# AdrienC21/CCSD

Hardware: AMD Instinct MI355X
Metric: sampled complexes/sec at 1000 PC steps, QM9_CC batch=1024, 1/2/4/8 GPU (higher is better)
Workload: dtype f32; 1 GPU; qm9_CC N=9 F=4 E=36 K=466, B=1024 per GPU, VE x3, Reverse+Langevin snr=0.2 scale_eps=0.7 n_steps=1, 1000 scales; global_batch=1024, parallelism=batch-sharded x1, per-shard Langevin norms, all-gather at end, finite=True

## Files before the change

### ccsd_amd/_lib.py

```python
from __future__ import annotations

import ctypes as C
import os
from typing import Optional

HERE = os.path.dirname(os.path.abspath(__file__))
HIP_LIB_PATH = os.path.join(HERE, "libccsd_hip.so")

ABI_VERSION = 5
OK, ERR_INVALID, ERR_UNSUPPORTED, ERR_WEIGHTS, ERR_RUNTIME, ERR_WORKSPACE, ERR_CALLBACK = range(7)
SDE_VP, SDE_VE, SDE_SUBVP = 0, 1, 2
PRED_EULER, PRED_REVERSE, PRED_S4 = 0, 1, 2
CORR_NONE, CORR_LANGEVIN = 0, 1
TARGET_X, TARGET_ADJ, TARGET_RANK2 = 0, 1, 2

EXPORTS = [
    "ccsd_plan_create", "ccsd_plan_destroy", "ccsd_weight_count", "ccsd_rank2_dims", "ccsd_workspace_bytes",
    "ccsd_last_error", "ccsd_score", "ccsd_init_state", "ccsd_corrector_norms", "ccsd_corrector_apply",
    "ccsd_predictor", "ccsd_s4_apply", "ccsd_sampler_run", "ccsd_quantize", "ccsd_rank2_cells", "ccsd_profile_kernel", "ccsd_profile_stride", "ccsd_profile_read", "ccsd_profile_launches", "ccsd_debug_stamps",
    "ccsd_noise_draws", "ccsd_noise_draws_at", "ccsd_plan_query", "ccsd_sampler_run_ex", "ccsd_finish",
    "ccsd_cluster_hist", "ccsd_orbit_counts", "ccsd_mmd_workspace_bytes", "ccsd_mmd",
    "ccsd_eig_workspace_bytes", "ccsd_eigvalsh", "ccsd_spectral_workspace_bytes", "ccsd_spectral_hist",
    "ccsd_hodge_workspace_bytes", "ccsd_hodge_spectrum",
    "ccsd_nspdk_row_capacity", "ccsd_nspdk_workspace_bytes", "ccsd_nspdk_features", "ccsd_nspdk_mmd_workspace_bytes", "ccsd_nspdk_mmd",
]
QUERIES = {"fused_r2": 0, "xa_variant": 1, "r2_lds_bytes": 2, "xa_lds_bytes": 3, "fused_loop": 4, "merged_r2": 5, "ew1": 6, "large_graph": 7,
           "r2_family": 8, "r2_instance": 9, "loop_form": 10, "h_full": 11, "hp_full": 12, "p0_narrow": 13, "tiled_fuse": 14, "ew1_fuse": 15,
           "h_general": 16, "geo_ek": 17, "h_wide": 18, "mlp_forms": 19}
KERNEL_IDS = {"k_xa": 0, "k_gemm_p": 1, "k_hf_score": 2, "k_gemm_h": 3, "k_langevin_apply": 4, "k_r2": 5, "k_s4_apply": 6, "k_ew1": 7}


class StepCoef(C.Structure):
    _fields_ = [(n, C.c_float) for n in ("sscale", "alpha", "pa", "pb", "pc", "m1", "s1", "d", "m2", "s2")]


class Config(C.Structure):
    _fields_ = (
        [(n, C.c_int32) for n in (
            "abi_version", "N", "F", "is_cc", "d_min", "d_max",
            "x_depth", "x_nhid",
            "a_num_layers", "a_num_linears", "a_c_init", "a_c_hid", "a_c_final", "a_nhid", "a_adim", "a_num_heads",
            "a_is_cc_net", "h_num_layers", "h_num_linears", "h_nhid", "h_adim", "h_c_hid", "h_c_final", "h_num_heads",
            "f_num_layers", "f_num_linears", "f_nhid", "f_c_hid", "f_c_final", "f_cnum", "f_num_layers_mlp",
            "f_use_hodge_mask",
            "predictor", "corrector", "n_corr_steps", "probability_flow", "denoise")]
        + [("snr", C.c_float), ("scale_eps", C.c_float), ("diff_steps", C.c_int32), ("batch_hint", C.c_int32)]
        + [(n, C.c_int32) for n in ("x_gmh", "x_num_linears", "x_c_init", "x_c_hid", "x_c_final", "x_adim", "x_num_heads",
                                    "a_conv_mlp", "x_conv_mlp")]
    )


class State(C.Structure):
    _fields_ = [("x", C.c_void_p), ("adj", C.c_void_p), ("rank2", C.c_void_p)]


class Noise(C.Structure):
    _fields_ = [("zx", C.c_void_p), ("zadj", C.c_void_p), ("zrank2", C.c_void_p)]


FINISH_ADJ_QUANTIZE, FINISH_ADJ_MOL = 0, 1
MMD_EMD, MMD_TV, MMD_L2 = 0, 1, 2
MMD_INT32, MMD_FP64 = 0, 1
MMD_IS_HIST, MMD_DEGREE, MMD_F32_PMF = 1, 2, 4
CLUSTER_MAX_BINS, MMD_MAX_ROWS, MMD_MAX_BINS = 1024, 1 << 20, 1 << 16
ORBITS = 15
NSPDK_MAX_NODES, NSPDK_FEATURES = 64, 65537
EIG_MAXN, EIG_MAX_SWEEPS = 512, 30


class FinishDims(C.Structure):
    _fields_ = [("B", C.c_int32), ("N", C.c_int32), ("F", C.c_int32), ("E", C.c_int32), ("K", C.c_int64),
                ("d_min", C.c_int32), ("d_max", C.c_int32), ("adj_mode", C.c_int32), ("thr", C.c_float)]


FINISH_OUTPUTS = ("adj_int", "degree", "degree_hist", "edge_hist", "n_nodes", "x_hist", "rank2_u8", "rank2_cell_bits",
                  "rank2_cell_count", "rank2_cell_hist", "rank2_nnz")


class FinishOut(C.Structure):
    _fields_ = [(n, C.c_void_p) for n in FINISH_OUTPUTS]


REDUCE_FN = C.CFUNCTYPE(C.c_int, C.c_void_p, C.c_int32, C.c_void_p, C.c_void_p)


class RunOptions(C.Structure):
    _fields_ = [("reduce", REDUCE_FN), ("user", C.c_void_p)]


class CcsdError(RuntimeError):
    pass


def raise_status(lib, status: int):
    if status == OK:
        return
    msg = lib.ccsd_last_error().decode("utf-8", "replace")
    if status == ERR_UNSUPPORTED:
        raise NotImplementedError(msg)
    if status in (ERR_INVALID, ERR_WEIGHTS, ERR_WORKSPACE):
        raise ValueError(msg)
    raise CcsdError(msg)


class Library:

    def __init__(self, path: str, is_hip: bool):
        if not os.path.exists(path):
            raise FileNotFoundError(path)
        self.path = path
        self.is_hip = is_hip
        L = self.c = C.CDLL(path)
        vp, i32, i64, u64, f32, sz = C.c_void_p, C.c_int32, C.c_int64, C.c_uint64, C.c_float, C.c_size_t
        P = C.POINTER
        L.ccsd_plan_create.argtypes = [P(Config), P(C.c_float), sz, P(StepCoef), P(vp)]
        L.ccsd_plan_create.restype = C.c_int
        L.ccsd_plan_destroy.argtypes = [vp]
        L.ccsd_plan_destroy.restype = None
        L.ccsd_weight_count.argtypes = [P(Config)]
        L.ccsd_weight_count.restype = sz
        L.ccsd_rank2_dims.argtypes = [P(Config), P(i32), P(i64)]
        L.ccsd_rank2_dims.restype = None
        L.ccsd_workspace_bytes.argtypes = [vp, i32]
        L.ccsd_workspace_bytes.restype = sz
        L.ccsd_last_error.argtypes = []
        L.ccsd_last_error.restype = C.c_char_p
        L.ccsd_score.argtypes = [vp, i32, i32, P(State), vp, f32, vp, vp, sz, vp]
        L.ccsd_score.restype = C.c_int
        L.ccsd_init_state.argtypes = [vp, i32, vp, P(Noise), u64, i64, P(State), vp]
        L.ccsd_init_state.restype = C.c_int
        L.ccsd_corrector_norms.argtypes = [vp, i32, i32, i32, P(State), P(State), vp, P(Noise), u64, i64, vp, vp, sz, vp]
        L.ccsd_corrector_norms.restype = C.c_int
        L.ccsd_corrector_apply.argtypes = [vp, i32, i32, i32, P(State), vp, P(Noise), u64, i64, vp, P(State), vp, sz, vp]
        L.ccsd_corrector_apply.restype = C.c_int
        L.ccsd_predictor.argtypes = [vp, i32, i32, P(State), vp, P(Noise), u64, i64, P(State), P(State), vp, sz, vp]
        L.ccsd_predictor.restype = C.c_int
        L.ccsd_s4_apply.argtypes = [vp, i32, i32, P(State), vp, P(Noise), P(Noise), P(Noise), u64, i64, vp, P(State), P(State), vp, sz, vp]
        L.ccsd_s4_apply.restype = C.c_int
        L.ccsd_sampler_run.argtypes = [vp, i32, vp, u64, i64, i32, i32, P(State), P(State), P(State), vp, vp, sz, vp]
        L.ccsd_sampler_run.restype = C.c_int
        L.ccsd_sampler_run_ex.argtypes = L.ccsd_sampler_run.argtypes + [P(RunOptions)]
        L.ccsd_sampler_run_ex.restype = C.c_int
        L.ccsd_quantize.argtypes = [vp, i64, f32, vp, vp]
        L.ccsd_quantize.restype = C.c_int
        L.ccsd_rank2_cells.argtypes = [vp, i32, i32, i64, f32, vp, vp, vp]
        L.ccsd_rank2_cells.restype = C.c_int
        L.ccsd_profile_kernel.argtypes = [vp, i32]
        L.ccsd_profile_kernel.restype = C.c_int
        L.ccsd_profile_stride.argtypes = [vp, i32]
        L.ccsd_profile_stride.restype = C.c_int
        L.ccsd_profile_read.argtypes = [vp, i32, P(i64), P(C.c_double)]
        L.ccsd_profile_read.restype = C.c_int
        L.ccsd_profile_launches.argtypes = [vp, i32, P(i64)]
        L.ccsd_profile_launches.restype = C.c_int
        L.ccsd_debug_stamps.argtypes = [vp, vp]
        L.ccsd_debug_stamps.restype = C.c_int
        L.ccsd_noise_draws.argtypes = [vp, i32, vp, u64, i64, i32, i32, P(State), vp]
        L.ccsd_noise_draws.restype = C.c_int
        L.ccsd_noise_draws_at.argtypes = [vp, i32, vp, u64, i64, C.c_uint32, i32, P(State), vp]
        L.ccsd_noise_draws_at.restype = C.c_int
        L.ccsd_plan_query.argtypes = [vp, i32, P(i64)]
        L.ccsd_plan_query.restype = C.c_int
        L.ccsd_finish.argtypes = [P(FinishDims), P(State), vp, P(FinishOut), vp]
        L.ccsd_finish.restype = C.c_int
        L.ccsd_cluster_hist.argtypes = [vp, i32, i32, i32, f32, vp, i32, vp, vp, vp]
        L.ccsd_cluster_hist.restype = C.c_int
        L.ccsd_orbit_counts.argtypes = [vp, i32, i32, i32, f32, vp, vp, vp, vp]
        L.ccsd_orbit_counts.restype = C.c_int
        L.ccsd_mmd_workspace_bytes.argtypes = [i32, i32, i32]
        L.ccsd_mmd_workspace_bytes.restype = sz
        L.ccsd_mmd.argtypes = [vp, i32, vp, vp, i32, vp, i32, i32, i32, i32, C.c_double, C.c_double, vp, sz, vp, vp]
        L.ccsd_mmd.restype = C.c_int
        L.ccsd_eig_workspace_bytes.argtypes = [i32, i32]
        L.ccsd_eig_workspace_bytes.restype = sz
        L.ccsd_eigvalsh.argtypes = [vp, i32, i32, vp, vp, vp, sz, vp]
        L.ccsd_eigvalsh.restype = C.c_int
        L.ccsd_spectral_workspace_bytes.argtypes = [i32, i32]
        L.ccsd_spectral_workspace_bytes.restype = sz
        L.ccsd_spectral_hist.argtypes = [vp, i32, i32, i32, f32, vp, i32, vp, vp, vp, vp, sz, vp]
        L.ccsd_spectral_hist.restype = C.c_int
        L.ccsd_hodge_workspace_bytes.argtypes = [i32, i32]
        L.ccsd_hodge_workspace_bytes.restype = sz
        L.ccsd_hodge_spectrum.argtypes = [vp, vp, i32, i32, i32, i32, i32, f32, vp, vp, vp, sz, vp]
        L.ccsd_hodge_spectrum.restype = C.c_int
        L.ccsd_nspdk_row_capacity.argtypes = [i32]
        L.ccsd_nspdk_row_capacity.restype = i32
        L.ccsd_nspdk_workspace_bytes.argtypes = [i32, i32]
        L.ccsd_nspdk_workspace_bytes.restype = sz
        L.ccsd_nspdk_features.argtypes = [vp, vp, i32, i32, i32, f32, vp, vp, vp, vp, sz, vp]
        L.ccsd_nspdk_features.restype = C.c_int
        L.ccsd_nspdk_mmd_workspace_bytes.argtypes = [i32, i32]
        L.ccsd_nspdk_mmd_workspace_bytes.restype = sz
        L.ccsd_nspdk_mmd.argtypes = [vp, vp, vp, i32, vp, vp, vp, i32, vp, sz, vp, vp]
        L.ccsd_nspdk_mmd.restype = C.c_int

    def __getattr__(self, name):
        return getattr(self.c, name)

    def check(self, status: int):
        raise_status(self.c, status)


_hip: Optional[Library] = None


def get_library() -> Library:
    global _hip
    if _hip is None:
        import torch

        path = os.environ.get("CCSD_LIB_PATH") or HIP_LIB_PATH
        if not os.path.exists(path):
            raise CcsdError(
                f"{path} is missing: build it with `python -c 'import __graft_entry__ as g; g.build()'` "
                "(hipcc --offload-arch=gfx950).  ccsd_amd has no CPU fallback."
            )
        _hip = Library(path, is_hip=True)
    return _hip
```

### ccsd_amd/csrc/ccsd_api.h

```cpp
#pragma once
#include "ccsd_kernels.h"
#define CCSD_INST_TABLES
#include "ccsd_instances.h"
#include <stdio.h>
#include <stdlib.h>
#include <memory>
#include <string>
#include <vector>

static thread_local std::string g_last_error;
static int set_err(int st, const std::string& m) { g_last_error = m; return st; }

static inline int fnet_width(const PlanD& p) {
    int fw = p.f_fdim > p.f_cnum ? p.f_fdim : p.f_cnum;
    for (int l = 0; l < p.f_L; ++l) {
        const MlpD& m = p.fl[l];
        const int wd = m.n > 1 && m.hid > m.in ? (m.hid > m.out ? m.hid : m.out) : (m.in > m.out ? m.in : m.out);
        if (wd > fw) fw = wd;
    }
    if (p.f_fin.n > 1 && p.f_fin.hid > fw) fw = p.f_fin.hid;
    return fw;
}

struct Knobs {
    int no_fused_r2 = 0, hodge_general = 0, geo_off = 0, no_fused_apply = 0, no_h_full = 0, no_hp_full = 0, hp_full_norms = 0, split_bf16 = 0;
    int xa_threads = 0, xa_prio = 0, lg_force = 0, xa_pass = -1, xa_gch = 0, no_mlp_wt = 0, verbose = 0;
    const char *dump_plan = nullptr, *dump_plan_name = nullptr;
};
static Knobs read_knobs() {
    Knobs k;
    auto on = [](const char* name) { return getenv(name) != nullptr; };
    k.no_fused_r2 = on("CCSD_NO_FUSED_R2"); k.hodge_general = on("CCSD_HODGE_GENERAL");
    k.geo_off = on("CCSD_NO_GEO") ? 1 : on("CCSD_NO_BAKE") ? 2 : 0;
    k.no_fused_apply = on("CCSD_NO_FUSED_APPLY"); k.no_h_full = on("CCSD_NO_H_FULL"); k.no_hp_full = on("CCSD_NO_HP_FULL");
    k.hp_full_norms = on("CCSD_HP_FULL_NORMS");
    if (const char* v = getenv("CCSD_SPLIT_BF16")) k.split_bf16 = atoi(v) == 3 ? 3 : 0;
    if (const char* v = getenv("CCSD_XA_THREADS")) { const int t = atoi(v); if (t >= 64 && t <= 1024 && t % 64 == 0) k.xa_threads = t; }
    if (const char* v = getenv("CCSD_XA_PRIO")) k.xa_prio = atoi(v);
    if (const char* v = getenv("CCSD_LARGE_GRAPH")) { const int f = atoi(v); k.lg_force = (f == 1 || f == 2) ? f : 0; }
    if (const char* v = getenv("CCSD_XA_PASS")) k.xa_pass = atoi(v);
    k.xa_gch = on("CCSD_XA_GCH"); k.no_mlp_wt = on("CCSD_NO_MLP_WT"); k.verbose = on("CCSD_VERBOSE");
    k.dump_plan = getenv("CCSD_DUMP_PLAN"); k.dump_plan_name = getenv("CCSD_DUMP_PLAN_NAME");
    return k;
}

enum { R2_NONE = 0, R2_FUSED = 1, R2_EW1 = 2, R2_TILED = 3 };
enum { LOOP_PRED_ONLY = 0, LOOP_LANGEVIN = 1, LOOP_LANGEVIN_FUSED = 2, LOOP_S4 = 3, LOOP_LANGEVIN_MULTI = 4 };
struct Route {
    int lg = 0;
    int xa_variant = 0;
    const XaEntry* xa = nullptr;
    const XaEntry* xa_twin = nullptr;
    int xa_threads = 0;
    int r2_family = R2_NONE;
    const R2Entry* r2 = nullptr;
    int r2_ldk = 0, r2_ldh = 0;
    size_t r2_lds = 0;
    int h_general = 0;
    int h_wide = 0;
    int geo = 0;
    int p0 = -1;
    int h_full = 0;
    unsigned hp_full_modes = 0;
    int loop = LOOP_PRED_ONLY;
    int merged = 0;
    int tiled_fuse = 0;
    int ew1_fuse = 0;
    int corrector_flat = 0, predictor_flat = 0;
};

struct ccsd_plan {
    ccsd_config_t cfg;
    PlanD h;
    HodgeBaseD hbx[CCSD_LG_MAXHB];
    MlpD hdm[CCSD_MAXHL + CCSD_MAXHLX];
    MlpD afin_lg;
    PlanD* d = nullptr;
    float* w = nullptr;
    float* wp = nullptr;
    unsigned char* hpairs = nullptr;
    size_t npacked = 0;
    unsigned char* edges = nullptr;
    unsigned long long* cells = nullptr;
    std::vector<ccsd_step_coef_t> coef;
    size_t nweights = 0;
    long long* dbg = nullptr;
    unsigned long long* init_off = nullptr;
    size_t init_off_cap = 0;
    Knobs knobs;
    Route rt;
    mutable unsigned prof_mask = 0;
    mutable size_t prof_used[8] = {0, 0, 0, 0, 0, 0, 0, 0};
    mutable int prof_stride = 1;
    mutable size_t prof_calls[8] = {0, 0, 0, 0, 0, 0, 0, 0};
#ifndef CCSD_EMU
    mutable std::vector<hipEvent_t> prof_ev[8];
#endif
};

enum { KID_XA = 0, KID_GEMM_P = 1, KID_HF = 2, KID_GEMM_H = 3, KID_LANGEVIN = 4, KID_R2 = 5, KID_S4 = 6, KID_EW1 = 7 };
static void prof_mark(const ccsd_plan* pl, int kid, void* stream) {
#ifndef CCSD_EMU
    if (!(pl->prof_mask & (1u << kid))) return;
    const size_t call = pl->prof_calls[kid]++;
    if (pl->prof_stride > 1 && (call >> 1) % (size_t)pl->prof_stride != 0) return;
    std::vector<hipEvent_t>& ev = pl->prof_ev[kid];
    if (pl->prof_used[kid] == ev.size()) {
        hipEvent_t e;
        if (hipEventCreate(&e) != hipSuccess) return;
        ev.push_back(e);
    }
    (void)hipEventRecord(ev[pl->prof_used[kid]++], (hipStream_t)stream);
#else
    (void)pl; (void)kid; (void)stream;
#endif
}
#define RT_CHECK(expr)                                                                    \
    do {                                                                                  \
        rtError_t _e = (expr);                                                            \
        if (_e != RT_OK) return set_err(CCSD_ERR_RUNTIME, std::string(#expr) + ": " + rt_error_string(_e)); \
    } while (0)
#define LAUNCH_CHECK()                                                                    \
    do {                                                                                  \
        rtError_t _e = rt_last_error();                                                   \
        if (_e != RT_OK) return set_err(CCSD_ERR_RUNTIME, std::string("kernel launch: ") + rt_error_string(_e)); \
    } while (0)

static int resolve_route(ccsd_plan* pl) {
    const PlanD& p = pl->h;
    const ccsd_config_t& c = pl->cfg;
    const Knobs& k = pl->knobs;
    Route& r = pl->rt;
    const int E = p.E, K = p.K;
    const bool s4 = c.predictor == CCSD_PRED_S4, langevin = c.corrector == CCSD_CORR_LANGEVIN;
    unsigned char arch[sizeof(PlanD)];
    ccsd_plan_arch_bytes(p, arch);
    auto baked = [&](const unsigned char* plan, size_t size) { return size == sizeof(PlanD) && p.geo_off == 0 && memcmp(arch, plan, size) == 0; };

    bool conv_mlp = false;
    for (int l = 0; l < p.a_L; ++l) conv_mlp = conv_mlp || p.al[l].conv_mlp;
    if (p.x_gmh) for (int l = 0; l < p.x_depth; ++l) conv_mlp = conv_mlp || p.gl[l].conv_mlp;
    int v = p.hb_L ? XA_HB : p.x_gmh ? XA_GMH : XA_PLAIN;
    if (conv_mlp || (p.hb_L && p.x_gmh) || p.h_L > 2 || (!p.chan_global && !p.hb_L && p.a_fin.chain >= 5)) v = XA_GEN;
    if (v == XA_PLAIN && !p.chan_global && baked(CCSD_BAKED_QM9_PLAN, CCSD_BAKED_QM9_SIZE)) v = XA_BAKED9;
    else if (v == XA_PLAIN && p.chan_global && baked(CCSD_BAKED_CS_PLAN, CCSD_BAKED_CS_SIZE)) v = XA_BAKED20;
    else if (v == XA_PLAIN && p.chan_global && baked(CCSD_BAKED_Z_PLAN, CCSD_BAKED_Z_SIZE)) v = XA_BAKED38;
    else if (v == XA_GEN && !p.chan_global && baked(CCSD_BAKED_ENZ_PLAN, CCSD_BAKED_ENZ_SIZE)) v = XA_BAKEDENZ;
    else if (v == XA_PLAIN && p.geo_off != 1)
        for (const auto& g : XA_GEO_TABLE)
            if ((p.chan_global != 0) == (g.gch != 0) && p.N == g.N && (!g.F || p.F == g.F) && E == g.E && p.ldn == g.ldn) v = g.var;
    r.xa_variant = v;
    r.xa_threads = k.xa_threads;
    for (const XaEntry& e : XA_TABLE) {
        if ((e.gch != 0) != (p.chan_global != 0)) continue;
        if (e.var == v) r.xa = &e;
        if (e.var == XA_PLAIN) r.xa_twin = &e;
    }
    if (!r.xa || !r.xa_twin) return set_err(CCSD_ERR_RUNTIME, "k_xa variant " + std::to_string(v) + " has no instance in CCSD_XA_LIST");
    if (!r.xa->fixed256) r.xa_twin = nullptr;

    const bool aff = p.f_affine != 0, gen1 = p.h_L > 1 && p.hl[0].mval.n > 1;
    const int mt = (E + 15) / 16, rem = E & 15, rs = (!aff || rem == 0 || rem > 12) ? 0 : (rem + 3) / 4;
    auto r2_find = [&](int qm9) -> const R2Entry* {
        for (const R2Entry& e : R2_TABLE)
            if (e.mt == mt && e.rs == rs && (e.affine != 0) == aff && (e.gen1 != 0) == gen1 && e.qm9 == qm9) return &e;
        return nullptr;
    };
    bool fused = false;
    if (c.is_cc && E <= 64 && !k.no_fused_r2 && !r.h_wide) {
        const int Kp4 = (K + 31) & ~31, Ep4 = (E + 3) & ~3;
        int ldk = Kp4; while ((ldk & 31) != 8 && (ldk & 31) != 24) ldk += 4;
        const int ldh = Ep4;
        const size_t fl = (size_t)E * ldk + (size_t)E * ldh + 64 * 2 + (size_t)p.a_cinit * E + 3 * c.N * c.N + 64 + (Kp4 + 3) / 4 + 4;
        if (fl * 4 + 64 <= 160 * 1024 && fnet_width(p) <= CCSD_FW && r2_find(0) && p.f_cnum <= 2) {
            fused = true; r.r2_ldk = ldk; r.r2_ldh = ldh; r.r2_lds = fl * 4;
            const bool qm9 = p.geo_off != 1 && !gen1 && E == CCSD_R2_QM9_E && K == CCSD_R2_QM9_K && p.N == CCSD_R2_QM9_N &&
                             ldk == CCSD_R2_QM9_LDK && ldh == CCSD_R2_QM9_LDH;
            r.r2 = r2_find(!qm9 ? 0 : aff && baked(CCSD_BAKED_QM9_PLAN, CCSD_BAKED_QM9_SIZE) ? 2 : 1);
            if (!r.r2) return set_err(CCSD_ERR_RUNTIME, "k_r2: the qm9-geometry instance is missing from CCSD_R2_LIST_*");
        }
    }
    if (p.h_L > 2) {
        bool affine_values = true;
        for (int l = 0; l + 1 < p.h_L; ++l) affine_values = affine_values && ccsd_hl(p, l).mval.n == 1;
        if (!affine_values || !fused || p.h_L > 4 || k.hodge_general || r.lg) { r.h_general = 1; fused = false; r.r2 = nullptr; }
    }
    const bool ew1 = c.is_cc && !fused && aff && p.f_cnum == 1 && !s4 && !r.h_wide;
    r.r2_family = !c.is_cc ? R2_NONE : fused ? R2_FUSED : ew1 ? R2_EW1 : R2_TILED;
    if (p.geo_off != 1) for (const GeoEntry& g : GEO_TABLE) if (E == g.E && K == g.K) r.geo = g.idx;
    if (p.h_L >= 1) {
        auto p0_find = [&](int kc) {
            for (int i = 0; i < (int)(sizeof(P0_TABLE) / sizeof(P0_TABLE[0])); ++i)
                if (P0_TABLE[i].nt == (p.hl[0].wc + 15) / 16 && P0_TABLE[i].kc == kc) return i;
            return -1;
        };
        if (p.geo_off != 1) r.p0 = p0_find(K);
        if (r.p0 < 0) r.p0 = p0_find(0);
    }
    r.tiled_fuse = !r.lg && r.r2_family == R2_TILED && p.h_L == 1 && (K & 3) == 0 && !s4 && langevin;
    r.ew1_fuse = !r.lg && ew1 && p.h_L == 1 && (K & 3) == 0 && langevin;
    const bool full_geo = c.is_cc && E == CCSD_FULL_E && K == CCSD_FULL_K && p.geo_off != 1 && !k.no_h_full;
    r.h_full = full_geo && r.r2_family == R2_TILED && p.f_cnum >= 2;

    const bool fused_apply = !r.lg && (fused || (ew1 && p.h_L <= 1) || r.tiled_fuse) && !k.no_fused_apply;
    r.loop = s4 ? LOOP_S4 : !langevin ? LOOP_PRED_ONLY : c.n_corr_steps != 1 ? LOOP_LANGEVIN_MULTI : fused_apply ? LOOP_LANGEVIN_FUSED : LOOP_LANGEVIN;
    if (full_geo && r.tiled_fuse && p.hl[0].wc <= 16 && p.f_cnum == 2 && !k.no_hp_full)
        r.hp_full_modes = (r.loop == LOOP_LANGEVIN_FUSED ? 1u << 2 : 0u) | (k.hp_full_norms ? 1u << 1 : 0u);
    r.merged = r.loop == LOOP_LANGEVIN_FUSED && fused && mt == 3 && rs == 1 && aff && !gen1 && (K & 1) == 0 && ((E * K) & 3) == 0;
    r.corrector_flat = !s4;
    r.predictor_flat = ew1;
    return CCSD_OK;
}
static inline bool use_h_full(const Route& r, int B) { return r.h_full && B >= 256; }
static inline bool use_hp_full(const Route& r, int B, int mode) { return B >= 256 && ((r.hp_full_modes >> mode) & 1u); }
#define HP_FULL_LDS ((size_t)(2 * 192 * H_LD + 2 * 16 * H_LD) * 4)
static inline int hodge_value_cw(int E) { return E > 128 ? 32 : 64; }
static inline size_t hodge_value_lds(int E) { return (size_t)E * hodge_value_cw(E) * 4; }
static inline const XaEntry* xa_launch(const Route& r, int B, int* threads) {
    const XaEntry* e = r.xa;
    int t = r.xa_threads;
    if (t == 0) t = e->max_threads == 256 ? 256 : B <= 256 ? 1024 : B <= 512 ? 512 : 256;
    if (e->fixed256 && t != 256) e = r.xa_twin;
    *threads = t > e->max_threads ? e->max_threads : t;
    return e;
}
static inline int normsum_threads(int B) { return B > 512 ? 1024 : B > 256 ? 512 : 256; }

extern "C" const char* ccsd_last_error(void) { return g_last_error.c_str(); }

extern "C" void ccsd_rank2_dims(const ccsd_config_t* cfg, int32_t* E, int64_t* K) {
    int e = 0; int64_t k = 0;
    if (cfg) ccsd_dims(cfg, &e, &k);
    if (E) *E = e;
    if (K) *K = k;
}

extern "C" size_t ccsd_weight_count(const ccsd_config_t* cfg) {
    PlanD p; PlanBuilder pb;
    size_t n = ccsd_build_plan(cfg, &p, pb);
    if (pb.status != CCSD_OK) { set_err(pb.status, pb.err); return 0; }
    return n;
}

extern "C" int ccsd_debug_stamps(ccsd_plan_t* plan, void* dev_buffer) {
    if (!plan) return set_err(CCSD_ERR_INVALID, "NULL plan");
    plan->dbg = (long long*)dev_buffer;
    return CCSD_OK;
}
extern "C" int ccsd_profile_kernel(ccsd_plan_t* plan, int32_t kernel_id) {
    if (!plan) return set_err(CCSD_ERR_INVALID, "NULL plan");
    if (kernel_id < 0) plan->prof_mask = 0;
    else if (kernel_id < 8) plan->prof_mask |= 1u << kernel_id;
    for (int k = 0; k < 8; ++k) { plan->prof_used[k] = 0; plan->prof_calls[k] = 0; }
    return CCSD_OK;
}
extern "C" int ccsd_profile_stride(ccsd_plan_t* plan, int32_t stride) {
    if (!plan || stride < 1) return set_err(CCSD_ERR_INVALID, "bad argument");
    plan->prof_stride = stride;
    for (int k = 0; k < 8; ++k) plan->prof_calls[k] = 0;
    return CCSD_OK;
}
extern "C" int ccsd_profile_launches(ccsd_plan_t* plan, int32_t kernel_id, int64_t* launches) {
    if (!plan || !launches || kernel_id < 0 || kernel_id >= 8) return set_err(CCSD_ERR_INVALID, "bad argument");
    *launches = (int64_t)(plan->prof_calls[kernel_id] >> 1);
    return CCSD_OK;
}
extern "C" int ccsd_profile_read(ccsd_plan_t* plan, int32_t kernel_id, int64_t* launches, double* total_ms) {
    if (!plan || !launches || !total_ms || kernel_id < 0 || kernel_id >= 8) return set_err(CCSD_ERR_INVALID, "bad argument");
    *launches = 0; *total_ms = 0.0;
#ifndef CCSD_EMU
    for (size_t i = 0; i + 1 < plan->prof_used[kernel_id]; i += 2) {
        float ms = 0.f;
        RT_CHECK(hipEventSynchronize(plan->prof_ev[kernel_id][i + 1]));
        RT_CHECK(hipEventElapsedTime(&ms, plan->prof_ev[kernel_id][i], plan->prof_ev[kernel_id][i + 1]));
        *total_ms += ms; *launches += 1;
    }
#endif
    plan->prof_used[kernel_id] = 0;
    return CCSD_OK;
}

extern "C" void ccsd_plan_destroy(ccsd_plan_t* plan) {
    if (!plan) return;
#ifndef CCSD_EMU
    for (int k = 0; k < 8; ++k) for (hipEvent_t e : plan->prof_ev[k]) (void)hipEventDestroy(e);
#endif
    if (plan->d) (void)rt_free(plan->d);
    if (plan->w) (void)rt_free(plan->w);
    if (plan->wp) (void)rt_free(plan->wp);
    if (plan->hpairs) (void)rt_free(plan->hpairs);
    if (plan->edges) (void)rt_free(plan->edges);
    if (plan->cells) (void)rt_free(plan->cells);
    if (plan->init_off) (void)rt_free(plan->init_off);
    delete plan;
}

extern "C" int ccsd_plan_create(const ccsd_config_t* cfg, const float* weights, size_t n_weights,
                                const ccsd_step_coef_t* step_coef, ccsd_plan_t** out) {
    if (!cfg || !weights || !step_coef || !out) return set_err(CCSD_ERR_INVALID, "NULL argument");
    *out = nullptr;
    std::unique_ptr<ccsd_plan, void (*)(ccsd_plan_t*)> guard(new ccsd_plan(), ccsd_plan_destroy);
    ccsd_plan* pl = guard.get();
    pl->cfg = *cfg;
    const Knobs& k = pl->knobs = read_knobs();
    PlanBuilder pb;
    pb.lg_force = k.lg_force; pb.xa_pass = k.xa_pass; pb.xa_gch = k.xa_gch; pb.no_mlp_wt = k.no_mlp_wt; pb.verbose = k.verbose;
    pl->nweights = ccsd_build_plan(cfg, &pl->h, pb);
    if (pb.status != CCSD_OK) return set_err(pb.status, pb.err);
    pl->rt.lg = pb.lg; pl->rt.h_wide = pb.h_wide;
    memcpy(pl->hbx, pb.hbx, sizeof(pl->hbx));
    memcpy(pl->hdm, pb.hdm, sizeof(pl->hdm));
    pl->afin_lg = pb.afin_lg;
    pl->h.geo_off = k.geo_off;
    pl->npacked = (size_t)pb.pcur;
    if (pl->nweights != n_weights)
        return set_err(CCSD_ERR_WEIGHTS, "weight blob has " + std::to_string(n_weights) + " floats, config needs " +
                                             std::to_string(pl->nweights));
    if (cfg->predictor != CCSD_PRED_EULER && cfg->predictor != CCSD_PRED_REVERSE && cfg->predictor != CCSD_PRED_S4) return set_err(CCSD_ERR_UNSUPPORTED, "unknown predictor");
    if (cfg->corrector != CCSD_CORR_NONE && cfg->corrector != CCSD_CORR_LANGEVIN) return set_err(CCSD_ERR_UNSUPPORTED, "unknown corrector");
    if (cfg->diff_steps < 1 || cfg->n_corr_steps < 0) return set_err(CCSD_ERR_INVALID, "bad step counts");
    ccsd_fold_fnet(&pl->h, weights);
    pl->coef.assign(step_coef, step_coef + (size_t)cfg->diff_steps * 3);
    const int N = cfg->N, E = pl->h.E, K = pl->h.K;
    std::vector<unsigned char> edges((size_t)2 * E + 2);
    {
        int e = 0;
        for (int i = 0; i < N; ++i)
            for (int j = i + 1; j < N; ++j) { edges[2 * e] = (unsigned char)i; edges[2 * e + 1] = (unsigned char)j; ++e; }
    }
    std::vector<unsigned long long> cells((size_t)K + 1);
    if (cfg->is_cc) {
        size_t c = 0;
        std::vector<int> idx;
        for (int k = cfg->d_min; k <= cfg->d_max; ++k) {
            idx.resize(k);
            for (int i = 0; i < k; ++i) idx[i] = i;
            while (true) {
                unsigned long long m = 0;
                for (int i = 0; i < k; ++i) m |= 1ull << idx[i];
                cells[c++] = m;
                int i = k - 1;
                while (i >= 0 && idx[i] == N - k + i) --i;
                if (i < 0) break;
                ++idx[i];
                for (int j = i + 1; j < k; ++j) idx[j] = idx[j - 1] + 1;
            }
        }
        if ((int)c != K) return set_err(CCSD_ERR_INVALID, "cell enumeration mismatch");
    }
    RT_CHECK(rt_malloc((void**)&pl->d, sizeof(PlanD)));
    RT_CHECK(rt_h2d(pl->d, &pl->h, sizeof(PlanD)));
    {
        const size_t wtotal = pl->h.f_blk >= 0 ? (size_t)pl->h.f_blk + CCSD_FBLK_FLOATS : n_weights;
        RT_CHECK(rt_malloc((void**)&pl->w, wtotal * sizeof(float)));
        RT_CHECK(rt_h2d(pl->w, weights, n_weights * sizeof(float)));
        if (pl->h.f_blk >= 0) {
            std::vector<float> blk(CCSD_FBLK_FLOATS);
            ccsd_pack_fnet_blocks(&pl->h, weights, blk.data());
            RT_CHECK(rt_h2d(pl->w + pl->h.f_blk, blk.data(), blk.size() * sizeof(float)));
        }
    }
    {
        std::vector<float> packed(pl->npacked + 4, 0.f);
        ccsd_pack_mlp(pl->h.x_fin, weights, packed.data());
        for (int l = 0; l < pl->h.a_L; ++l) {
            ccsd_pack_mlp(pl->h.al[l].mlp, weights, packed.data()); ccsd_pack_mlp(pl->h.al[l].mc, weights, packed.data());
            ccsd_pack_qkv(pl->h.al[l], weights, packed.data()); ccsd_pack_mc(pl->h.al[l], weights, packed.data());
        }
        if (pl->h.x_gmh) for (int l = 0; l < pl->h.x_depth; ++l) {
            ccsd_pack_mlp(pl->h.gl[l].mlp, weights, packed.data()); ccsd_pack_mlp(pl->h.gl[l].mc, weights, packed.data());
            ccsd_pack_qkv(pl->h.gl[l], weights, packed.data()); ccsd_pack_mc(pl->h.gl[l], weights, packed.data());
        }
        for (int l = 0; l < pl->h.hb_L; ++l) {
            const HodgeBaseD& h = pl->hbx[l];
            ccsd_pack_mlp(h.mh, weights, packed.data());
            for (int c = 0; c < h.cin; ++c) {
                const float* blk = weights + h.blk_base + (size_t)c * h.blk_stride;
                const float* w2 = blk + h.hid * E + h.hid;
                for (int e = 0; e < E; ++e)
                    for (int hh = 0; hh < h.hid; ++hh) {
                        packed[(size_t)h.w2t + ((size_t)c * h.hid + hh) * E + e] = w2[e * h.hid + hh];
                        packed[(size_t)h.w1t + ((size_t)c * E + e) * h.hid + hh] = blk[hh * E + e];
                    }
            }
        }
        ccsd_pack_mlp(pl->h.a_fin, weights, packed.data());
        if (pl->rt.lg) {
            for (int l = 0; l < pl->h.h_L; ++l) ccsd_pack_mlp(pl->hdm[l], weights, packed.data());
            if (pl->afin_lg.chain) ccsd_pack_mlp(pl->afin_lg, weights, packed.data());
        }
        for (int l = 0; l < pl->h.h_L; ++l) {
            const HodgeLayerD& h = ccsd_hl(pl->h, l);
            const int Kp = (K + 31) & ~31;
            for (int k = 0; k < K; ++k)
                for (int n = 0; n < h.wc; ++n) packed[(size_t)h.wcatT + (size_t)n * Kp + k] = weights[(size_t)h.wcat + (size_t)k * h.wc + n];
        }
        RT_CHECK(rt_malloc((void**)&pl->wp, packed.size() * sizeof(float)));
        RT_CHECK(rt_h2d(pl->wp, packed.data(), packed.size() * sizeof(float)));
    }
    if (pl->h.h_L > 1 && !pl->rt.lg) {
        if (E > 255) return set_err(CCSD_ERR_UNSUPPORTED, "dense hodge layer needs E <= 255");
        std::vector<unsigned char> hp;
        for (int e = 0; e < E; ++e)
            for (int e2 = e; e2 < E; ++e2) { hp.push_back((unsigned char)e); hp.push_back((unsigned char)e2); }
        RT_CHECK(rt_malloc((void**)&pl->hpairs, hp.size()));
        RT_CHECK(rt_h2d(pl->hpairs, hp.data(), hp.size()));
    }
    RT_CHECK(rt_malloc((void**)&pl->edges, edges.size()));
    RT_CHECK(rt_h2d(pl->edges, edges.data(), edges.size()));
    RT_CHECK(rt_malloc((void**)&pl->cells, cells.size() * sizeof(unsigned long long)));
    RT_CHECK(rt_h2d(pl->cells, cells.data(), cells.size() * sizeof(unsigned long long)));
    if (int st = resolve_route(pl)) return st;
    {
        const Route& r = pl->rt;
        const size_t xlds = (size_t)pl->h.xa_lds_floats * 4;
        if (xlds > 64 * 1024) {
            RT_CHECK(rt_set_max_dyn_smem((const void*)r.xa->fn, xlds));
            if (r.xa_twin) RT_CHECK(rt_set_max_dyn_smem((const void*)r.xa_twin->fn, xlds));
        }
        if (r.r2 && r.r2_lds > 64 * 1024) RT_CHECK(rt_set_max_dyn_smem((const void*)r.r2->fn, r.r2_lds));
        if (r.lg && lg_nmlp_lds(pl->h) > 64 * 1024) RT_CHECK(rt_set_max_dyn_smem((const void*)k_lg_nmlp, lg_nmlp_lds(pl->h)));
        if (r.lg && pl->h.hb_L > 1) {
            size_t v = 0;
            for (int l = 0; l + 1 < pl->h.hb_L; ++l) if (lg_hb_dense_lds(pl->hbx[l]) > v) v = lg_hb_dense_lds(pl->hbx[l]);
            if (v > 64 * 1024) RT_CHECK(rt_set_max_dyn_smem((const void*)k_lg_hb_dense, v));
        }
        if (r.lg && r.h_general && hodge_value_lds(E) > 64 * 1024)
            RT_CHECK(rt_set_max_dyn_smem(r.h_wide ? (const void*)k_hodge_value_w : (const void*)k_hodge_value, hodge_value_lds(E)));
#ifndef CCSD_EMU
        if (r.hp_full_modes) {
            RT_CHECK(rt_set_max_dyn_smem((const void*)k_hp_full<CCSD_FULL_E, CCSD_FULL_K, 1>, HP_FULL_LDS));
            RT_CHECK(rt_set_max_dyn_smem((const void*)k_hp_full<CCSD_FULL_E, CCSD_FULL_K, 2>, HP_FULL_LDS));
        }
#endif
    }
    if (const char* path = k.dump_plan) {
        const char* nm = k.dump_plan_name ? k.dump_plan_name : "QM9";
        std::vector<unsigned char> bytes(sizeof(PlanD));
        ccsd_plan_arch_bytes(pl->h, bytes.data());
        if (FILE* f = fopen(path, "w")) {
            fprintf(f, "// GENERATED by tools/bake_plan.py (do not edit): the PlanD of a shipped configuration at its bench batch as a compile-time\n"
                       "// constant (architecture bytes: ccsd_plan_arch_bytes, the weight-derived affine fold zeroed).  The baked kernel instances read\n"
                       "// their plan from it instead of from memory; the host selects them only for plans whose architecture bytes are equal.\n"
                       "#pragma once\n#define CCSD_BAKED_%s_SIZE %zu\n#define CCSD_BAKED_%s_A_L %d      /* AttentionLayers of ScoreNetworkA: unroll count */\n"
                       "alignas(16) static constexpr unsigned char CCSD_BAKED_%s_PLAN[CCSD_BAKED_%s_SIZE] = {", nm, sizeof(PlanD), nm, pl->h.a_L, nm, nm);
            for (size_t i = 0; i < bytes.size(); ++i) fprintf(f, "%s%u,", (i % 40) ? "" : "\n    ", (unsigned)bytes[i]);
            fprintf(f, "\n};\n");
            fclose(f);
        }
    }
    *out = guard.release();
    return CCSD_OK;
}

#define CCSD_P_SPLITS 8

struct Workspace {
    unsigned long long* offbits;
    unsigned char *mfr, *mfl;
    int Kp, Ep;
    float *H, *P0, *P1, *U1, *acoef, *net_x, *net_adj, *net_r, *norm2, *part, *sums, *chan, *zpart, *part2;
    float* psplit; size_t psplit_floats;
    float *P0b, *P1b, *U1b;
    int ntiles, nchunk;
    float *hgH, *hgR[2], *hgP[CCSD_MAXHL + CCSD_MAXHLX - 1];
    size_t hg_hstride;
    float *lg_S, *lg_att, *lg_dis, *lg_Y, *lg_QKV, *lg_x[2], *lg_xcat, *lg_xY, *lg_xnet, *lg_part;
    int lg_tiles;
    float *lg_hbg, *lg_hbH;
    size_t lg_hbg_stride, lg_hbH_stride;
    float *lg_hdq, *lg_hdd, *lg_hdpc, *lg_hdH;
    size_t lg_hdq_stride, lg_hdH_stride;
    ccsd_state_t third;
    size_t bytes;
    MaskTab masks() const { return MaskTab{mfr, mfl, Kp, Ep}; }
};
struct Pass {
    const float* h_src = nullptr;
    int p1_raw = 0;
};
static inline int r2_p1_raw(const PlanD& p) { return p.h_L > 1 && p.hl[0].mval.n == 1; }
static Workspace carve_ws(const ccsd_plan* pl, int B, void* base) {
    const PlanD& p = pl->h;
    Workspace w{};
    size_t o = 0;
    auto take = [&](size_t nbytes) { size_t r = o; o += (nbytes + 255) / 256 * 256; return base ? (char*)base + r : (char*)nullptr; };
    w.offbits = (unsigned long long*)take((size_t)B * 8);
    const size_t E = p.E, K = p.K;
    w.Kp = p.is_cc ? (p.K + 3) & ~3 : 0; w.Ep = p.is_cc ? (p.E + 3) & ~3 : 0;
    w.mfr = (unsigned char*)take((size_t)B * w.Kp);
    w.mfl = (unsigned char*)take((size_t)B * w.Ep);
    w.H = (float*)take(p.is_cc ? (size_t)B * E * h_ld((int)E) * 4 * (p.f_cnum > 2 ? p.f_cnum - 1 : 1) : 0);
    w.P0 = (float*)take(p.h_L > 0 ? (size_t)B * E * p.hl[0].wc * 4 : 0);
    w.P1 = (float*)take(p.h_L > 1 ? (size_t)B * E * p.h_pw * 4 : 0);
    w.U1 = (float*)take(p.h_L > 1 ? (size_t)B * p.h_pw * 4 : 0);
    w.psplit_floats = p.h_L > 1 ? (size_t)CCSD_P_SPLITS * B * E * p.h_pw : 0;
    w.psplit = (float*)take(w.psplit_floats * 4);
    const bool two = pl->rt.r2_family == R2_FUSED;
    w.P0b = (float*)take(two && p.h_L > 0 ? (size_t)B * E * p.hl[0].wc * 4 : 0);
    w.P1b = (float*)take(two && p.h_L > 1 ? (size_t)B * E * p.h_pw * 4 : 0);
    w.U1b = (float*)take(two && p.h_L > 1 ? (size_t)B * p.h_pw * 4 : 0);
    w.acoef = (float*)take(p.h_L > 1 ? (size_t)B * p.a_cinit * E * 4 : 0);
    if (pl->rt.h_general) {
        int cmax = 1;
        for (int l = 0; l + 1 < p.h_L; ++l) cmax = ccsd_hl(p, l).cout > cmax ? ccsd_hl(p, l).cout : cmax;
        w.hg_hstride = (size_t)cmax * E * E;
        w.hgH = (float*)take((size_t)B * w.hg_hstride * 4);
        w.hgR[0] = (float*)take((size_t)B * E * K * 4);
        w.hgR[1] = (float*)take((size_t)B * E * K * 4);
        for (int l = 1; l < p.h_L; ++l) w.hgP[l - 1] = (float*)take((size_t)B * E * ccsd_hl(p, l).wc * 4);
    }
    w.net_x = (float*)take((size_t)B * p.N * p.F * 4);
    w.net_adj = (float*)take((size_t)B * p.N * p.N * 4);
    w.net_r = (float*)take(p.is_cc ? (size_t)B * E * K * 4 : 0);
    w.norm2 = (float*)take((size_t)B * 4 * 4);
    w.ntiles = p.is_cc ? ((p.K + T_BN - 1) / T_BN) * ((p.E + T_BM - 1) / T_BM) : 0;
    w.nchunk = p.is_cc ? (int)((((size_t)p.E * p.K + 3) / 4 + CCSD_NN_CH - 1) / CCSD_NN_CH) : 0;
    { int np = w.ntiles > w.nchunk ? w.ntiles : w.nchunk; if ((int)E > np) np = (int)E;
      w.part = (float*)take((size_t)B * (np ? np : 1) * 2 * 4); }
    w.zpart = (float*)take((size_t)B * ((size_t)w.nchunk > E ? (size_t)w.nchunk : E ? E : 1) * 4);
    w.part2 = (float*)take((size_t)B * 2 * 4);
    w.sums = (float*)take(64);
    w.chan = (float*)take(p.chan_global ? (size_t)B * p.chan_rows * p.N * p.N * 4 : 0);
    if (pl->rt.lg) {
        const size_t N = p.N, NN = N * N;
        int cin = 1, cp = 1, fx = p.F > p.x_nhid ? p.F : p.x_nhid;
        for (int l = 0; l < p.a_L; ++l) {
            if (p.al[l].cin > cin) cin = p.al[l].cin;
            if (p.al[l].cp > cp) cp = p.al[l].cp;
            if (p.al[l].fout > fx) fx = p.al[l].fout;
        }
        w.lg_tiles = (int)((NN + CCSD_LG_FIN_ROWS - 1) / CCSD_LG_FIN_ROWS);
        w.lg_S = (float*)take((size_t)B * p.a_fdim * NN * 4);
        w.lg_att = (float*)take((size_t)B * cin * NN * 4);
        w.lg_dis = (float*)take((size_t)B * cin * N * 4);
        w.lg_Y = (float*)take((size_t)B * cin * N * cp * 4);
        w.lg_QKV = (float*)take((size_t)B * cin * N * cp * 4);
        w.lg_x[0] = (float*)take((size_t)B * N * fx * 4);
        w.lg_x[1] = (float*)take((size_t)B * N * fx * 4);
        w.lg_xcat = (float*)take((size_t)B * N * p.x_fdim * 4);
        w.lg_xY = (float*)take((size_t)B * N * p.x_nhid * 4);
        w.lg_xnet = (float*)take((size_t)B * N * p.F * 4);
        w.lg_part = (float*)take((size_t)B * w.lg_tiles * 2 * 4);
        if (p.hb_L) {
            size_t g = 0, hd = 0;
            for (int l = 0; l < p.hb_L; ++l) {
                const HodgeBaseD& h = pl->hbx[l];
                if ((size_t)h.cin * E * h.hid > g) g = (size_t)h.cin * E * h.hid;
                if (l + 1 < p.hb_L && (size_t)h.cout * E * E > hd) hd = (size_t)h.cout * E * E;
            }
            w.lg_hbg_stride = g; w.lg_hbH_stride = hd;
            w.lg_hbg = (float*)take((size_t)B * g * 4);
            w.lg_hbH = (float*)take((size_t)B * hd * 4);
        }
        if (p.h_L > 1) {
            size_t q = 0, d = 0, hd = 0;
            for (int l = 0; l < p.h_L; ++l) {
                const HodgeLayerD& h = ccsd_hl(p, l);
                if ((size_t)h.cin * E * 2 * h.adim > q) q = (size_t)h.cin * E * 2 * h.adim;
                if (l > 0 && (size_t)h.cin * E > d) d = (size_t)h.cin * E;
                if (l + 1 < p.h_L && (size_t)h.cout * E * E > hd) hd = (size_t)h.cout * E * E;
            }
            w.lg_hdq_stride = q;
            w.lg_hdq = (float*)take((size_t)B * q * 4);
            w.lg_hdd = (float*)take((size_t)B * d * 4);
            w.lg_hdpc = (float*)take((size_t)B * 2 * E * 4);
            if (pl->rt.h_general) { w.lg_hdH = w.hgH; w.lg_hdH_stride = w.hg_hstride; }
            else { w.lg_hdH_stride = hd; w.lg_hdH = (float*)take((size_t)B * hd * 4); }
        }
    }
    if (pl->rt.loop == LOOP_LANGEVIN_MULTI && pl->cfg.n_corr_steps > 1) {
        w.third.x = (float*)take((size_t)B * p.N * p.F * 4);
        w.third.adj = (float*)take((size_t)B * p.N * p.N * 4);
        w.third.rank2 = p.is_cc ? (float*)take((size_t)B * E * K * 4) : nullptr;
    }
    w.bytes = o;
    return w;
}
extern "C" size_t ccsd_workspace_bytes(const ccsd_plan_t* plan, int32_t B) {
    if (!plan || B < 1) return 0;
    return carve_ws(plan, B, nullptr).bytes;
}

static int grid_for(long long n, int block) {
    long long g = (n + block - 1) / block;
    if (g > 2048) g = 2048;
    if (g < 1) g = 1;
    return (int)g;
}

static int check_common(const ccsd_plan* pl, int B, const void* flags, void* ws, size_t ws_bytes, Workspace& w) {
    if (!pl) return set_err(CCSD_ERR_INVALID, "NULL plan");
    if (B < 1) return set_err(CCSD_ERR_INVALID, "B must be >= 1");
    if (!flags) return set_err(CCSD_ERR_INVALID, "NULL flags");
    if (ws) w = carve_ws(pl, B, ws);
    if (!ws || ws_bytes < w.bytes) return set_err(CCSD_ERR_WORKSPACE, "workspace too small");
    return CCSD_OK;
}
static int check_state(const ccsd_plan* pl, const ccsd_state_t* s, const char* what) {
    if (!s || !s->x || !s->adj || (pl->h.is_cc && !s->rank2)) return set_err(CCSD_ERR_INVALID, std::string("NULL tensor in ") + what);
    return CCSD_OK;
}

static int launch_flagbits(const ccsd_plan* pl, int B, const float* flags, Workspace& w, void* stream) {
    if (pl->rt.lg && !pl->h.is_cc) return CCSD_OK;
    CCSD_LAUNCH(k_flagbits, dim3(grid_for(B, 256)), dim3(CCSD_NTHREADS), 0, stream, flags, w.offbits, B, pl->h.N);
    LAUNCH_CHECK();
    if (pl->h.is_cc) {
        CCSD_LAUNCH(k_masktab, dim3(grid_for((long long)B * (w.Kp + w.Ep), 256)), dim3(CCSD_NTHREADS), 0, stream,
                    (const unsigned long long*)w.offbits, (const unsigned char*)pl->edges, (const unsigned long long*)pl->cells, w.mfr, w.mfl,
                    B, pl->h.E, pl->h.K, w.Kp, w.Ep);
        LAUNCH_CHECK();
    }
    return CCSD_OK;
}

static int launch_h(const ccsd_plan* pl, int B, const float* rank2, Pass& ps, Workspace& w, void* stream) {
    const PlanD& p = pl->h;
    if (!p.is_cc || p.f_cnum < 2) return CCSD_OK;
    if (ps.h_src == rank2) return CCSD_OK;
    const bool full = use_h_full(pl->rt, B);
    const int nth_ = (p.E + T_BM - 1) / T_BM;
    dim3 g(xcd_grid(B, nth_ * (nth_ + 1) / 2));
    prof_mark(pl, KID_GEMM_H, stream);
#ifndef CCSD_EMU
    if (full && pl->knobs.split_bf16 == 3) hipLaunchKernelGGL((k_gemm_h_full<CCSD_FULL_E, CCSD_FULL_K, 2>), dim3(B), dim3(256), 0, (hipStream_t)stream, rank2, w.H, p.f_hmask);
    else if (full) hipLaunchKernelGGL((k_gemm_h_full<CCSD_FULL_E, CCSD_FULL_K>), dim3(B), dim3(256), 0, (hipStream_t)stream, rank2, w.H, p.f_hmask);
    else
#endif
    {
        (void)full;
#define H_GO(EC_, KC_) CCSD_LAUNCH((k_gemm_h<EC_, KC_>), g, dim3(CCSD_NTHREADS), 0, stream, rank2, w.H, p.E, p.K, p.f_hmask, B)
        GEO_EK(pl->rt.geo, H_GO);
#undef H_GO
    }
    prof_mark(pl, KID_GEMM_H, stream);
    LAUNCH_CHECK();
    for (int j = 2; j < p.f_cnum; ++j) {
        const size_t slab = (size_t)B * p.E * h_ld(p.E);
        const int nt = (p.E + 15) / 16, per = CCSD_NTHREADS >= 64 ? CCSD_NTHREADS / 64 : 1;
        CCSD_LAUNCH(k_gemm_pow, dim3((nt * nt + per - 1) / per, 1, B), dim3(CCSD_NTHREADS), 0, stream,
                    (const float*)(w.H + (size_t)(j - 2) * slab), (const float*)w.H, w.H + (size_t)(j - 1) * slab, p.E);
        LAUNCH_CHECK();
    }
    return CCSD_OK;
}
static void launch_gemm_p_whole(const ccsd_plan* pl, int B, const float* R, const HodgeLayerD& h, float* out, const Workspace& w, void* stream) {
    const PlanD& p = pl->h;
    const int rows = B * p.E;
    CCSD_LAUNCH(k_gemm_p, dim3((h.wc + T_BN - 1) / T_BN, (rows + T_BM - 1) / T_BM, 1), dim3(CCSD_NTHREADS), 0, stream, R, (const float*)pl->w, out,
                rows, p.E, p.K, h.wc, h.wcat, 0, h.mval, h.cin, (const float*)nullptr, (const unsigned long long*)w.offbits,
                (const unsigned char*)pl->edges, (const unsigned long long*)pl->cells, p.K);
}
static void launch_hodge_value(const ccsd_plan* pl, int B, const float* Rin, const float* H, size_t h_stride, const float* acoef,
                              const HodgeLayerD& h, float* Rout, const Workspace& w, void* stream) {
    const PlanD& p = pl->h;
    const int cw = hodge_value_cw(p.E);
    CCSD_LAUNCH(pl->rt.h_wide ? k_hodge_value_w : k_hodge_value, dim3((p.K + cw - 1) / cw, B), dim3(CCSD_NTHREADS), hodge_value_lds(p.E), stream, Rin, H,
                (int)h_stride, acoef, (const float*)pl->w, h.mval, h.cin, Rout, p.E, p.K, cw,
                (const unsigned long long*)w.offbits, (const unsigned char*)pl->edges, (const unsigned long long*)pl->cells);
}
static int hodge_stack_layer(const ccsd_plan* pl, int B, int l, Workspace& w, void* stream) {
    float* Rl = w.hgR[(l - 1) & 1];
    launch_hodge_value(pl, B, w.hgR[(l - 2) & 1], w.hgH, w.hg_hstride, nullptr, ccsd_hl(pl->h, l - 1), Rl, w, stream);
    LAUNCH_CHECK();
    launch_gemm_p_whole(pl, B, Rl, ccsd_hl(pl->h, l), w.hgP[l - 1], w, stream);
    LAUNCH_CHECK();
    return CCSD_OK;
}
static int launch_r2(const ccsd_plan* pl, int B, const float* rank2, const float* adj, const float* flags, int want_p,
                     RankEpi& ep, NoiseArgs& na, Pass& ps, Workspace& w, void* stream, const CorrFuse* cf, int merge_draw);
static int launch_p(const ccsd_plan* pl, int B, const float* adj, const float* rank2, Pass& ps, Workspace& w, void* stream, const P0Fuse* fuse = nullptr) {
    const PlanD& p = pl->h;
    const Route& rt = pl->rt;
    if (p.h_L < 1) return CCSD_OK;
    if (p.h_L > 2 && !rt.h_general) {
        RankEpi ep{};
        ep.mode = MODE_SCORE; ep.sscale = 0.f; ep.out = w.net_r;
        NoiseArgs na0{};
        return launch_r2(pl, B, rank2, adj, nullptr, 1, ep, na0, ps, w, stream, nullptr, -1);
    }
    ps.p1_raw = 0;
    const int rows = B * p.E;
    const bool hp_full = fuse && use_hp_full(rt, B, fuse->mode);
#ifndef CCSD_EMU
    if (hp_full) {
        const HodgeLayerD& h = p.hl[0];
        const float* WT = (const float*)pl->wp + h.wcatT;
        prof_mark(pl, KID_GEMM_H, stream);
        if (fuse->mode == 1)
            hipLaunchKernelGGL((k_hp_full<CCSD_FULL_E, CCSD_FULL_K, 1>), dim3(B), dim3(512), HP_FULL_LDS, (hipStream_t)stream, rank2, WT, w.H, w.P0, h.wc, p.f_hmask, *fuse);
        else
            hipLaunchKernelGGL((k_hp_full<CCSD_FULL_E, CCSD_FULL_K, 2>), dim3(B), dim3(512), HP_FULL_LDS, (hipStream_t)stream, rank2, WT, w.H, w.P0, h.wc, p.f_hmask, *fuse);
        prof_mark(pl, KID_GEMM_H, stream);
        LAUNCH_CHECK();
        ps.h_src = fuse->mode == 2 ? fuse->f1 : rank2;
        return CCSD_OK;
    }
#endif
    (void)hp_full;
    {
        const HodgeLayerD& h = p.hl[0];
        prof_mark(pl, KID_GEMM_P, stream);
        P0Fuse pf{};
        if (fuse) pf = *fuse;
#ifndef CCSD_EMU
        if (rt.p0 >= 0)
            hipLaunchKernelGGL(P0_TABLE[rt.p0].fn[pf.mode], dim3((rows + T_BM - 1) / T_BM), dim3(256), 0, (hipStream_t)stream, rank2,
                               (const float*)pl->wp + h.wcatT, w.P0, rows, p.K, (p.K + 31) & ~31, h.wc, pf);
        else
#endif
        {
            const float* src = rank2;
            if (pf.mode) {
                CCSD_LAUNCH(k_p0_fuse_ew, dim3(grid_for(rows, 256)), dim3(CCSD_NTHREADS), 0, stream, rank2, pf, rows, p.K);
                LAUNCH_CHECK();
                if (pf.mode == 2 || pf.mode == 4) src = pf.f1;
            }
            launch_gemm_p_whole(pl, B, src, h, w.P0, w, stream);
        }
        prof_mark(pl, KID_GEMM_P, stream);
        LAUNCH_CHECK();
    }
    if (p.h_L > 1) {
        CCSD_LAUNCH(k_edgecoef, dim3(B), dim3(CCSD_NTHREADS), (size_t)3 * p.N * p.N * 4, stream, adj, w.acoef, p.N, p.E,
                    p.a_cinit, (const unsigned char*)pl->edges);
        LAUNCH_CHECK();
        const HodgeLayerD& h0 = p.hl[0];
        const HodgeLayerD& h = p.hl[1];
        dim3 g((h.wc + T_BN - 1) / T_BN, (rows + T_BM - 1) / T_BM, 1);
        const int nslab = (p.K + T_BK - 1) / T_BK;
        int S = CCSD_P_SPLITS < nslab ? CCSD_P_SPLITS : nslab;
        if ((size_t)S * rows * h.wc > w.psplit_floats) S = 1;
        const int kchunk = ((nslab + S - 1) / S) * T_BK;
        S = (p.K + kchunk - 1) / kchunk;
        g.z = S;
        float* P1 = rt.h_general ? w.hgP[0] : w.P1;
        CCSD_LAUNCH(rt.h_wide ? k_gemm_p_w : k_gemm_p, g, dim3(CCSD_NTHREADS), 0, stream, rank2, (const float*)pl->w, S > 1 ? w.psplit : P1, rows, p.E, p.K, h.wc,
                    h.wcat, 1, h0.mval, h0.cin, (const float*)w.acoef, (const unsigned long long*)w.offbits,
                    (const unsigned char*)pl->edges, (const unsigned long long*)pl->cells, kchunk);
        LAUNCH_CHECK();
        if (S > 1) {
            const long long n = (long long)rows * h.wc;
            CCSD_LAUNCH(k_sum_splits, dim3(grid_for(n, 256)), dim3(CCSD_NTHREADS), 0, stream, (const float*)w.psplit, P1, n, S);
            LAUNCH_CHECK();
        }
        if (rt.h_general) {
            launch_hodge_value(pl, B, rank2, nullptr, 0, w.acoef, h0, w.hgR[0], w, stream);
            LAUNCH_CHECK();
        }
    }
    return CCSD_OK;
}
static int launch_lg(const ccsd_plan* pl, int B, XaArgs& xa, NoiseArgs& na, Workspace& w, void* stream);
static int launch_xa(const ccsd_plan* pl, int B, XaArgs& xa, NoiseArgs& na, const Pass& ps, Workspace& w, void* stream, bool set_b = false) {
    const Route& rt = pl->rt;
    xa.P0 = set_b ? w.P0b : w.P0;
    xa.P1 = set_b ? w.P1b : w.P1; xa.U1 = set_b ? w.U1b : w.U1; xa.p1_raw = ps.p1_raw;
    if (rt.lg) return launch_lg(pl, B, xa, na, w, stream);
    xa.chan_ws = w.chan;
    xa.dbg = pl->dbg ? pl->dbg + 32 : nullptr;
    int xa_threads;
    const XaEntry* inst = xa_launch(rt, B, &xa_threads);
    prof_mark(pl, KID_XA, stream);
    xa.wp = pl->wp; xa.hpairs = pl->hpairs;
    xa.prio_mode = pl->knobs.xa_prio;
    const dim3 xblk(CCSD_NTHREADS == 1 ? 1 : xa_threads);
    const size_t xlds = (size_t)pl->h.xa_lds_floats * 4;
#define XA_LAUNCH(XA_) CCSD_LAUNCH(inst->fn, dim3(B), xblk, xlds, stream, (const PlanD*)pl->d, (const float*)pl->w, (const unsigned char*)pl->edges, XA_, na)
    if (rt.h_general) {
        const PlanD& p = pl->h;
        if (rt.xa_variant != XA_GEN) return set_err(CCSD_ERR_RUNTIME, "general hodge stack needs k_xa<., XA_GEN>");
        xa.pdirect = 1;
        for (int l = 1; l < p.h_L; ++l) xa.Pd[l - 1] = w.hgP[l - 1];
        for (int l = 2; l < p.h_L; ++l) {
            XaArgs pre = xa;
            pre.hdump_layer = l - 1; pre.hdump = w.hgH; pre.hdump_stride = (int)w.hg_hstride;
            XA_LAUNCH(pre);
            LAUNCH_CHECK();
            if (int st = hodge_stack_layer(pl, B, l, w, stream)) return st;
        }
    }
    XA_LAUNCH(xa);
#undef XA_LAUNCH
    prof_mark(pl, KID_XA, stream);
    LAUNCH_CHECK();
    return CCSD_OK;
}
static int launch_lg(const ccsd_plan* pl, int B, XaArgs& xa, NoiseArgs& na, Workspace& w, void* stream) {
    const PlanD& p = pl->h;
    if (xa.cf.on) return set_err(CCSD_ERR_RUNTIME, "tiled graph-network route: no fused corrector apply");
    const int N = p.N, F = p.F, NN = N * N, H = p.x_nhid, XF = p.x_fdim;
    const int rt = (N + 15) / 16, gt = (N + CCSD_LG_GT - 1) / CCSD_LG_GT, at = (N + CCSD_LG_AT - 1) / CCSD_LG_AT;
    const dim3 blk(CCSD_NTHREADS);
    auto cdiv = [](int a, int b_) { return (a + b_ - 1) / b_; };
    prof_mark(pl, KID_XA, stream);
    if (xa.do_x) {
        CCSD_LAUNCH(k_lg_dis, dim3(grid_for(N, 256), B), blk, 0, stream, xa.adjX, (long long)NN, 0, 1, N, w.lg_dis);
        CCSD_LAUNCH(k_lg_put, dim3(grid_for((long long)B * N * F, 256)), blk, 0, stream, xa.xX, F, w.lg_xcat, XF, B * N);
        for (int l = 0; l < p.x_depth; ++l) {
            const int fin = l ? H : F;
            const float* src = l ? w.lg_xcat + F + (l - 1) * H : xa.xX;
            CCSD_LAUNCH(k_lg_xw, dim3(grid_for((long long)N * H, 256), B), blk, 0, stream, src, (long long)N * (l ? XF : F), l ? XF : F, fin,
                        (const float*)pl->w + p.x_gw[l], 0, H, 1, N, (const float*)w.lg_dis, w.lg_xY);
            CCSD_LAUNCH(k_lg_gcn, dim3(gt * cdiv(H, CCSD_LG_GT), 1, B), blk, 0, stream, xa.adjX, (long long)NN, 0, (const float*)w.lg_xY,
                        (const float*)w.lg_dis, (const float*)pl->w + p.x_gb[l], 0, H, H, 1, N, w.lg_xcat, (long long)N * XF, 0, XF, F + l * H, 1);
        }
        CCSD_LAUNCH(k_lg_nmlp, dim3(rt, B), blk, lg_nmlp_lds_of(p.x_fin), stream, p.x_fin, (const float*)pl->w,
                    (LgGather{w.lg_xcat, (long long)N * XF, 0, XF, 0, XF}), N, xa.flags, 0, w.lg_xnet);
        LAUNCH_CHECK();
    }
    if (xa.do_a) {
        const long long ss = (long long)p.a_fdim * NN;
        for (int c = 0; c < p.a_cinit; ++c)
            CCSD_LAUNCH(k_lg_pow, dim3(grid_for(NN, 256), B), blk, 0, stream, xa.adjA, w.lg_S, ss, N, c);
        if (p.h_L == 1) {
            if (!xa.P0) return set_err(CCSD_ERR_RUNTIME, "tiled graph-network route: no hodge projections");
            if (pl->rt.h_wide) {
                CCSD_LAUNCH(k_lg_hodge1_w, dim3(grid_for(p.E, 256), B), blk, 0, stream, p.hl[0], pl->hdm[0], 1.0f / (float)sqrt((double)p.K), (const float*)pl->w,
                            (const float*)pl->wp, (const unsigned char*)pl->edges, xa.P0, w.lg_S, ss, p.a_nch_graph, N, p.E, xa.flags);
            } else {
                CCSD_LAUNCH(k_lg_hodge1, dim3(grid_for(p.E + N, 256), B), blk, 0, stream, p.hl[0], 1.0f / (float)sqrt((double)p.K), (const float*)pl->w,
                            (const unsigned char*)pl->edges, xa.P0, w.lg_S, ss, p.a_nch_graph, N, p.E, xa.flags);
            }
        }
        if (p.h_L > 1) {
            const Route& rtp = pl->rt;
            if (!xa.P0 || (!rtp.h_general && !xa.P1)) return set_err(CCSD_ERR_RUNTIME, "tiled graph-network route: no hodge projections");
            if (p.h_L > 2 && !rtp.h_general) return set_err(CCSD_ERR_RUNTIME, "tiled graph-network route: more than two hodge layers need the general hodge stack");
            const int E = p.E, et = (E + 15) / 16;
            const unsigned char* edges = (const unsigned char*)pl->edges;
            const float* wts = (const float*)pl->w;
            const float rks = 1.0f / (float)sqrt((double)p.K);
            const long long qs = (long long)w.lg_hdq_stride, hs = (long long)w.lg_hdH_stride;
            int ch = p.a_nch_graph + p.a_cinit;
            CCSD_LAUNCH(k_lg_hd_qk0, dim3(grid_for(E + N, 256), B), blk, 0, stream, p.hl[0], p.a_nch_hodge, wts, edges, xa.P0, w.lg_S, ss, p.a_nch_graph, N, E,
                        w.lg_hdq, qs);
            for (int j = 1; j < p.h_L; ++j) {
                const HodgeLayerD& hp = ccsd_hl(p, j - 1);
                const HodgeLayerD& h = ccsd_hl(p, j);
                CCSD_LAUNCH(k_lg_hd_dense, dim3(et * (et + 1) / 2, B), blk, lg_hd_dense_lds(hp), stream, hp, pl->hdm[j - 1], rks, (const float*)pl->wp, edges,
                            (const float*)w.lg_hdq, qs, w.lg_hdH, hs, w.lg_S, ss, ch, N, E, xa.flags);
                ch += hp.cout;
                LAUNCH_CHECK();
                if (rtp.h_general && j + 1 < p.h_L)
                    if (int st = hodge_stack_layer(pl, B, j + 1, w, stream)) return st;
                const bool raw = j == 1 && !rtp.h_general && xa.p1_raw;
                LgHdRaw rw{};
                if (raw) {
                    if (!xa.U1) return set_err(CCSD_ERR_RUNTIME, "tiled graph-network route: raw hodge projections without their u_1");
                    rw = LgHdRaw{wts, (const float*)w.lg_S, xa.flags, edges, w.lg_hdpc, ss, N, p.hl[0].cin, p.hl[0].mval.w[0], p.hl[0].mval.b[0]};
                }
                const float* Pj = rtp.h_general ? (const float*)w.hgP[j - 1] : xa.P1;
                CCSD_LAUNCH(k_lg_hd_dis, dim3(grid_for((long long)h.cin * E, 256), B), blk, 0, stream, (const float*)w.lg_hdH, hs, h.cin, E, w.lg_hdd, rw);
                CCSD_LAUNCH(k_lg_hd_conv, dim3((et + 3) / 4, h.cin, B), blk, 0, stream, h, wts, (const float*)w.lg_hdH, hs, (const float*)w.lg_hdd, Pj, h.wc,
                            raw ? (const float*)w.lg_hdpc : (const float*)nullptr, raw ? xa.U1 : (const float*)nullptr, E, w.lg_hdq, qs);
                LAUNCH_CHECK();
            }
            if (rtp.h_wide) {
                CCSD_LAUNCH(k_lg_hd_diag_w, dim3(grid_for(E, 256), B), blk, 0, stream, ccsd_hl(p, p.h_L - 1), pl->hdm[p.h_L - 1], rks, (const float*)pl->wp, edges,
                            (const float*)w.lg_hdq, qs, w.lg_S, ss, ch, N, E, xa.flags);
            } else {
                CCSD_LAUNCH(k_lg_hd_diag, dim3(grid_for(E, 256), B), blk, 0, stream, ccsd_hl(p, p.h_L - 1), rks, wts, edges, (const float*)w.lg_hdq, qs, w.lg_S, ss,
                            ch, N, E, xa.flags);
            }
            LAUNCH_CHECK();
        }
        if (p.hb_L) {
            const int E = p.E, et = (E + 15) / 16;
            const unsigned char* edges = (const unsigned char*)pl->edges;
            const float* wts = (const float*)pl->w;
            const float* wpk = (const float*)pl->wp;
            int ch = p.a_nch_graph + p.a_cinit;
            CCSD_LAUNCH(k_lg_hb_in, dim3(grid_for(E + N, 256), B), blk, 0, stream, pl->hbx[0], p.a_nch_hodge, wts, edges, w.lg_S, ss, p.a_nch_graph, N, E,
                        w.lg_hbg, (long long)w.lg_hbg_stride);
            for (int l = 0; l + 1 < p.hb_L; ++l) {
                const HodgeBaseD& h = pl->hbx[l];
                const HodgeBaseD& hn = pl->hbx[l + 1];
                float* Hl = w.lg_hbH;
                CCSD_LAUNCH(k_lg_hb_dense, dim3(et * (et + 1) / 2, B), blk, lg_hb_dense_lds(h), stream, h, wts, wpk, edges, (const float*)w.lg_hbg,
                            (long long)w.lg_hbg_stride, Hl, (long long)w.lg_hbH_stride, w.lg_S, ss, ch, N, E, xa.flags);
                CCSD_LAUNCH(k_lg_hb_hid, dim3((et + 3) / 4, hn.cin, B), blk, 0, stream, hn, wts, wpk, (const float*)Hl, (long long)w.lg_hbH_stride, E,
                            w.lg_hbg, (long long)w.lg_hbg_stride);
                ch += h.cout;
            }
            CCSD_LAUNCH(k_lg_hb_diag, dim3(grid_for(E, 256), B), blk, 0, stream, pl->hbx[p.hb_L - 1], wts, edges, (const float*)w.lg_hbg,
                        (long long)w.lg_hbg_stride, w.lg_S, ss, ch, N, E, xa.flags);
            LAUNCH_CHECK();
        }
        for (int l = 0; l < p.a_L; ++l) {
            const AttnLayerD& L = p.al[l];
            const float* xin = l ? w.lg_x[(l - 1) & 1] : xa.xA;
            const float* wq = pl->wp + L.qkvp;
            const int wcs = L.fin * L.cp + L.cp;
            CCSD_LAUNCH(k_lg_dis, dim3(grid_for((long long)L.cin * N, 256), B), blk, 0, stream, (const float*)w.lg_S, ss, L.ci0, L.cin, N, w.lg_dis);
            CCSD_LAUNCH(k_lg_xw, dim3(grid_for((long long)L.cin * N * L.cp, 256), B), blk, 0, stream, xin, (long long)N * L.fin, L.fin, L.fin,
                        wq, wcs, L.cp, L.cin, N, (const float*)w.lg_dis, w.lg_Y);
            CCSD_LAUNCH(k_lg_gcn, dim3(gt * cdiv(L.cp, CCSD_LG_GT), L.cin, B), blk, 0, stream, (const float*)w.lg_S, ss, L.ci0, (const float*)w.lg_Y,
                        (const float*)w.lg_dis, wq + L.fin * L.cp, wcs, L.cp, L.cp, L.cin, N, w.lg_QKV, (long long)L.cin * N * L.cp, N * L.cp, L.cp, 0, 0);
            CCSD_LAUNCH(k_lg_nmlp, dim3(rt, B), blk, lg_nmlp_lds_of(L.mc), stream, L.mc, (const float*)pl->w,
                        (LgGather{w.lg_QKV, (long long)L.cin * N * L.cp, N * L.cp, L.cp, 2 * L.adim, L.fout}), N, xa.flags, 1, w.lg_x[l & 1]);
            const float inv_scale = (float)sqrt((double)L.fout);
            CCSD_LAUNCH(k_lg_att, dim3(at * at, L.cin, B), blk, 0, stream, (const float*)w.lg_QKV, L.cp, L.adim, L.nchunk, L.dsplit, 1.0f / inv_scale,
                        0.5f / (float)L.nchunk, L.cin, N, w.lg_att);
            CCSD_LAUNCH(k_lg_edge, dim3(w.lg_tiles, B), blk, 0, stream, L.mlp, (const float*)pl->wp, (const float*)w.lg_att, w.lg_S, ss, L.ci0, L.co0,
                        L.cin, N);
            CCSD_LAUNCH(k_lg_sym, dim3(grid_for((long long)L.cout * NN, 256), B), blk, 0, stream, w.lg_S, ss, L.co0, L.cout, N, xa.flags);
            LAUNCH_CHECK();
        }
        if (pl->afin_lg.chain) {
            CCSD_LAUNCH(k_lg_fin_w, dim3(w.lg_tiles, B), blk, 0, stream, pl->afin_lg, (const float*)pl->wp, (const float*)w.lg_S, ss, N, xa.flags, xa.adjA,
                        xa, na, w.lg_part);
        } else {
            CCSD_LAUNCH(k_lg_fin, dim3(w.lg_tiles, B), blk, 0, stream, p.a_fin, (const float*)pl->wp, (const float*)w.lg_S, ss, N, xa.flags, xa.adjA,
                        xa, na, w.lg_part);
        }
        LAUNCH_CHECK();
    }
    CCSD_LAUNCH(k_lg_epi, dim3(B), blk, 0, stream, (const float*)w.lg_xnet, xa.xX, xa.flags, xa, na, (const float*)w.lg_part, w.lg_tiles, N, F);
    prof_mark(pl, KID_XA, stream);
    LAUNCH_CHECK();
    return CCSD_OK;
}

static int launch_hf(const ccsd_plan* pl, int B, const float* rank2, RankEpi& ep, NoiseArgs& na, Workspace& w, void* stream) {
    const PlanD& p = pl->h;
    dim3 g(xcd_grid(B, ((p.K + T_BN - 1) / T_BN) * ((p.E + T_BM - 1) / T_BM)));
    prof_mark(pl, KID_HF, stream);
#define HF_ARGS (const PlanD*)pl->d, (const float*)pl->w, rank2, (const float*)w.H, (const unsigned long long*)w.offbits, \
                (const unsigned char*)pl->edges, (const unsigned long long*)pl->cells, ep, na, B, w.masks()
    const int fw = fnet_width(p);
#define HF_AFF1(EC_, KC_) CCSD_LAUNCH((k_hf_score<true, 8, 1, EC_, KC_>), g, dim3(CCSD_NTHREADS), 0, stream, HF_ARGS)
#define HF_GEN1(EC_, KC_) CCSD_LAUNCH((k_hf_score<false, 8, 1, EC_, KC_>), g, dim3(CCSD_NTHREADS), 0, stream, HF_ARGS)
#define HF_GO(NP_) \
    do { \
        if (p.f_affine && NP_ == 1) GEO_EK(pl->rt.geo, HF_AFF1); \
        else if (p.f_affine) CCSD_LAUNCH((k_hf_score<true, 8, NP_>), g, dim3(CCSD_NTHREADS), 0, stream, HF_ARGS); \
        else if (fw <= 8 && NP_ == 1) GEO_EK(pl->rt.geo, HF_GEN1); \
        else if (fw <= 8) CCSD_LAUNCH((k_hf_score<false, 8, NP_>), g, dim3(CCSD_NTHREADS), 0, stream, HF_ARGS); \
        else if (fw <= CCSD_FW) CCSD_LAUNCH((k_hf_score<false, CCSD_FW, NP_>), g, dim3(CCSD_NTHREADS), 0, stream, HF_ARGS); \
        else CCSD_LAUNCH((k_hf_score<false, CCSD_FWMAX, NP_>), g, dim3(CCSD_NTHREADS), 0, stream, HF_ARGS); \
    } while (0)
    if (p.f_cnum <= 2) HF_GO(1); else HF_GO(CCSD_MAXCN - 1);
#undef HF_GO
#undef HF_AFF1
#undef HF_GEN1
#undef HF_ARGS
    prof_mark(pl, KID_HF, stream);
    LAUNCH_CHECK();
    return CCSD_OK;
}

static int launch_ew1(const ccsd_plan* pl, int B, const float* rank2, RankEpi& ep, NoiseArgs& na, Workspace& w, void* stream,
                      float* net_out = nullptr, const CorrFuse* cf = nullptr, float* f1 = nullptr) {
    const PlanD& p = pl->h;
    Ew1Args a{};
    a.r = rank2; a.out = ep.out; a.mean = ep.mean; a.f1 = f1; a.net_out = net_out; a.part = ep.part;
    a.mode = ep.mode; a.apply = (cf && cf->on) ? 1 : 0;
    a.sscale = ep.sscale; a.pa = ep.pa; a.pb = ep.pb; a.pc = ep.pc; a.alpha = p.f_alpha; a.gamma = p.f_gamma;
    if (a.apply) {
        const LangCoef& lc = cf->lc;
        a.sums = lc.sums; a.ss = lc.ss[2]; a.sde_alpha = lc.alpha[2]; a.snr = lc.snr; a.seps = lc.seps; a.draw_corr = cf->draw_r;
    }
    a.E = p.E; a.K = p.K; a.mt = w.masks();
    prof_mark(pl, KID_EW1, stream);
#define EW1_GO(EC_, KC_) CCSD_LAUNCH((k_ew1<EC_, KC_>), dim3(w.nchunk, B), dim3(CCSD_NTHREADS), 0, stream, a, na)
    GEO_EK(pl->rt.geo, EW1_GO);
#undef EW1_GO
    prof_mark(pl, KID_EW1, stream);
    LAUNCH_CHECK();
    return CCSD_OK;
}

static int launch_r2(const ccsd_plan* pl, int B, const float* rank2, const float* adj, const float* flags, int want_p,
                     RankEpi& ep, NoiseArgs& na, Pass& ps, Workspace& w, void* stream, const CorrFuse* cf = nullptr, int merge_draw = -1) {
    const Route& rt = pl->rt;
    R2Args ra{};
    if (cf) ra.cf = *cf;
    ra.masked = (cf && cf->on) ? 1 : 0;
    if (merge_draw >= 0) {
        ra.merge = 1; ra.draw_r2 = (unsigned)merge_draw;
        ra.P0b = w.P0b; ra.P1b = w.P1b; ra.U1b = w.U1b; ra.net2 = w.net_r; ra.part2 = w.part;
    }
    ra.rank2 = rank2; ra.adj = adj; ra.flags = flags; ra.offbits = w.offbits; ra.P0 = w.P0; ra.P1 = w.P1; ra.U1 = w.U1; ra.want_p = want_p;
    ra.ldk = rt.r2_ldk; ra.ldh = rt.r2_ldh; ra.dbg = pl->dbg; ra.wp = pl->wp;
    if (want_p && pl->h.h_L > 1) ps.p1_raw = r2_p1_raw(pl->h);
    prof_mark(pl, KID_R2, stream);
    CCSD_LAUNCH(rt.r2->fn, dim3(B), dim3(CCSD_NTHREADS == 1 ? 1 : 512), rt.r2_lds, stream, (const PlanD*)pl->d, (const float*)pl->w,
                (const unsigned char*)pl->edges, (const unsigned long long*)pl->cells, ra, ep, na);
    prof_mark(pl, KID_R2, stream);
    LAUNCH_CHECK();
    return CCSD_OK;
}

static inline int draws_per_step(const ccsd_config_t& cfg) { return cfg.predictor == CCSD_PRED_S4 ? 3 : cfg.n_corr_steps + 1; }
static unsigned int draw_base(const ccsd_plan* pl, int step, int phase) { return 3u + (unsigned)((step * draws_per_step(pl->cfg) + phase) * 3); }
static inline long long state_items(const PlanD& p, int B, int flat_r) {
    const long long r4 = flat_r ? ((long long)p.E * p.K + 3) / 4 : (long long)((p.E + 3) / 4) * p.K;
    return (long long)B * (p.N * p.F + p.N * p.N) + (p.is_cc ? (long long)B * r4 : 0);
}
static NoiseArgs make_noise(const ccsd_noise_t* n, uint64_t seed, int64_t off, unsigned int base, int flat_r = 0) {
    NoiseArgs na{};
    if (n) { na.zx = n->zx; na.zadj = n->zadj; na.zr = n->zrank2; }
    na.seed = seed; na.b_off = off;
    na.draw_x = base; na.draw_adj = base + 1; na.draw_r = base + 2;
    na.flat_r = flat_r;
    return na;
}

static LangCoef lang_coef(const ccsd_plan* pl, int step, const float* sums) {
    LangCoef lc{};
    lc.sums = sums;
    for (int t = 0; t < 3; ++t) {
        const ccsd_step_coef_t& c = pl->coef[(size_t)step * 3 + t];
        lc.ss[t] = c.sscale; lc.alpha[t] = c.alpha;
    }
    lc.snr = pl->h.snr; lc.seps = pl->h.seps;
    return lc;
}
static LangArgs lang_args(const ccsd_plan* pl, int B, int step, const ccsd_state_t* cur, const float* flags, const float* sums,
                          ccsd_state_t* out, const Workspace& w) {
    const PlanD& p = pl->h;
    LangArgs a{};
    a.x = cur->x; a.adj = cur->adj; a.r = cur->rank2;
    a.nx = w.net_x; a.nadj = w.net_adj; a.nr = w.net_r;
    a.ox = out->x; a.oadj = out->adj; a.orr = out->rank2;
    a.flags = flags; a.lc = lang_coef(pl, step, sums);
    a.B = B; a.N = p.N; a.F = p.F; a.E = p.E; a.K = p.K; a.is_cc = p.is_cc;
    return a;
}
static P0Fuse p0_fuse(const ccsd_plan* pl, int mode, const NoiseArgs& na, unsigned int draw, const Workspace& w) {
    P0Fuse pf{};
    pf.mode = mode; pf.seed = na.seed; pf.b_off = na.b_off; pf.draw = draw;
    pf.mt = w.masks(); pf.E = pl->h.E;
    return pf;
}
static RankEpi pred_epi(const ccsd_plan* pl, int step, ccsd_state_t* out, ccsd_state_t* mean) {
    const ccsd_step_coef_t& c = pl->coef[(size_t)step * 3 + 2];
    RankEpi ep{};
    ep.mode = MODE_PRED; ep.pa = c.pa; ep.pb = c.pb; ep.pc = c.pc;
    ep.out = out->rank2; ep.mean = mean ? mean->rank2 : nullptr;
    return ep;
}
static RankEpi norms_epi(const Workspace& w) {
    RankEpi ep{};
    ep.mode = MODE_NORMS; ep.out = w.net_r; ep.part = w.part;
    return ep;
}
static int copy_state(const ccsd_state_t& dst, const ccsd_state_t& src, const PlanD& p, size_t n, void* stream) {
    RT_CHECK(rt_d2d_async(dst.x, src.x, n * p.N * p.F * 4, stream));
    RT_CHECK(rt_d2d_async(dst.adj, src.adj, n * p.N * p.N * 4, stream));
    if (p.is_cc && p.E && p.K) RT_CHECK(rt_d2d_async(dst.rank2, src.rank2, n * p.E * p.K * 4, stream));
    return CCSD_OK;
}

extern "C" int ccsd_score(ccsd_plan_t* pl, int32_t target, int32_t B, const ccsd_state_t* in, const float* flags,
                          float sscale, float* out, void* workspace, size_t ws_bytes, void* stream) {
    Workspace w{};
    int st = check_common(pl, B, flags, workspace, ws_bytes, w);
    if (st) return st;
    if ((st = check_state(pl, in, "in"))) return st;
    if (!out) return set_err(CCSD_ERR_INVALID, "NULL out");
    if ((st = launch_flagbits(pl, B, flags, w, stream))) return st;
    NoiseArgs na{};
    Pass ps;
    if (target == CCSD_TARGET_X || target == CCSD_TARGET_ADJ) {
        XaArgs xa{};
        xa.xX = xa.xA = in->x; xa.adjX = xa.adjA = in->adj; xa.flags = flags;
        xa.do_x = target == CCSD_TARGET_X; xa.do_a = !xa.do_x; xa.mode = MODE_SCORE;
        xa.ss_x = xa.ss_a = sscale; xa.out_x = xa.out_a = out;
        if (xa.do_a && (st = launch_p(pl, B, in->adj, in->rank2, ps, w, stream))) return st;
        return launch_xa(pl, B, xa, na, ps, w, stream);
    }
    if (target == CCSD_TARGET_RANK2) {
        if (!pl->h.is_cc) return set_err(CCSD_ERR_INVALID, "rank2 score requested from a graph-only plan");
        RankEpi ep{};
        ep.mode = MODE_SCORE; ep.sscale = sscale; ep.out = out;
        if (pl->rt.r2_family == R2_FUSED) return launch_r2(pl, B, in->rank2, in->adj, flags, 0, ep, na, ps, w, stream);
        if (pl->rt.r2_family == R2_EW1) return launch_ew1(pl, B, in->rank2, ep, na, w, stream);
        if ((st = launch_h(pl, B, in->rank2, ps, w, stream))) return st;
        return launch_hf(pl, B, in->rank2, ep, na, w, stream);
    }
    return set_err(CCSD_ERR_UNSUPPORTED, "Object not yet supported. Select from [x, adj, rank2].");
}

static int draws_to_state(ccsd_plan* pl, int32_t B, const float* flags, const ccsd_noise_t* raw, uint64_t seed, int64_t sample_offset,
                          unsigned int base, ccsd_state_t* state, void* stream, int flat_r = 0) {
    if (!pl || B < 1 || !flags) return set_err(CCSD_ERR_INVALID, "bad argument");
    int st = check_state(pl, state, "state");
    if (st) return st;
    const PlanD& p = pl->h;
    if (pl->init_off_cap < (size_t)B) {
        if (pl->init_off) {
#ifndef CCSD_EMU
            (void)hipDeviceSynchronize();
#endif
            (void)rt_free(pl->init_off);
            pl->init_off = nullptr; pl->init_off_cap = 0;
        }
        RT_CHECK(rt_malloc((void**)&pl->init_off, (size_t)B * 8));
        pl->init_off_cap = (size_t)B;
    }
    unsigned long long* offbits = pl->init_off;
    if (!pl->rt.lg || p.is_cc) CCSD_LAUNCH(k_flagbits, dim3(grid_for(B, 256)), dim3(CCSD_NTHREADS), 0, stream, flags, offbits, B, p.N);
    NoiseArgs na = make_noise(raw, seed, sample_offset, base, flat_r);
    CCSD_LAUNCH(k_init_state, dim3(grid_for(state_items(p, B, flat_r), 256)), dim3(CCSD_NTHREADS), 0, stream, state->x, state->adj, state->rank2,
                flags, na, (const unsigned long long*)offbits, (const unsigned char*)pl->edges,
                (const unsigned long long*)pl->cells, B, p.N, p.F, p.E, p.K, p.is_cc);
    LAUNCH_CHECK();
    return CCSD_OK;
}

extern "C" int ccsd_init_state(ccsd_plan_t* pl, int32_t B, const float* flags, const ccsd_noise_t* prior, uint64_t seed,
                               int64_t sample_offset, ccsd_state_t* state, void* stream) {
    return draws_to_state(pl, B, flags, prior, seed, sample_offset, 0, state, stream);
}

extern "C" int ccsd_noise_draws(ccsd_plan_t* pl, int32_t B, const float* flags, uint64_t seed, int64_t sample_offset, int32_t step,
                                int32_t phase, ccsd_state_t* out, void* stream) {
    if (!pl) return set_err(CCSD_ERR_INVALID, "NULL plan");
    if (step < 0 || step >= pl->cfg.diff_steps || phase < 0 || phase >= draws_per_step(pl->cfg)) return set_err(CCSD_ERR_INVALID, "step / phase out of range");
    const bool corr = pl->cfg.predictor != CCSD_PRED_S4 && phase < pl->cfg.n_corr_steps && pl->cfg.corrector == CCSD_CORR_LANGEVIN;
    return draws_to_state(pl, B, flags, nullptr, seed, sample_offset, draw_base(pl, step, phase), out, stream,
                          corr ? pl->rt.corrector_flat : pl->rt.predictor_flat);
}

extern "C" int ccsd_noise_draws_at(ccsd_plan_t* pl, int32_t B, const float* flags, uint64_t seed, int64_t sample_offset, uint32_t draw,
                                   int32_t flat_rank2, ccsd_state_t* out, void* stream) {
    if (!pl) return set_err(CCSD_ERR_INVALID, "NULL plan");
    return draws_to_state(pl, B, flags, nullptr, seed, sample_offset, draw, out, stream, flat_rank2 ? 1 : 0);
}

extern "C" int ccsd_plan_query(const ccsd_plan_t* pl, int32_t what, int64_t* value) {
    if (!pl || !value) return set_err(CCSD_ERR_INVALID, "NULL argument");
    const Route& r = pl->rt;
    const int hint = pl->cfg.batch_hint;
    switch (what) {
        case CCSD_QUERY_FUSED_R2: *value = r.r2_family == R2_FUSED; break;
        case CCSD_QUERY_XA_VARIANT: *value = r.xa_variant; break;
        case CCSD_QUERY_R2_LDS_BYTES: *value = (int64_t)r.r2_lds; break;
        case CCSD_QUERY_XA_LDS_BYTES: *value = (int64_t)pl->h.xa_lds_floats * 4; break;
        case CCSD_QUERY_FUSED_LOOP: *value = r.loop == LOOP_LANGEVIN_FUSED; break;
        case CCSD_QUERY_MERGED_R2: *value = r.merged; break;
        case CCSD_QUERY_EW1: *value = r.r2_family == R2_EW1; break;
        case CCSD_QUERY_LARGE_GRAPH: *value = r.lg; break;
        case CCSD_QUERY_R2_FAMILY: *value = r.r2_family; break;
        case CCSD_QUERY_R2_INSTANCE: *value = r.r2 ? ((((int64_t)r.r2->mt * 10 + r.r2->rs) * 10 + r.r2->affine) * 10 + r.r2->gen1) * 10 + r.r2->qm9 : -1; break;
        case CCSD_QUERY_LOOP_FORM: *value = r.loop; break;
        case CCSD_QUERY_H_FULL: *value = use_h_full(r, hint); break;
        case CCSD_QUERY_HP_FULL: *value = (use_hp_full(r, hint, 2) ? 1 : 0) | (use_hp_full(r, hint, 1) ? 2 : 0); break;
        case CCSD_QUERY_P0_NARROW: *value = r.p0 >= 0 ? (int64_t)P0_TABLE[r.p0].nt * 100000 + P0_TABLE[r.p0].kc : 0; break;
        case CCSD_QUERY_TILED_FUSE: *value = r.tiled_fuse; break;
        case CCSD_QUERY_EW1_FUSE: *value = r.ew1_fuse; break;
        case CCSD_QUERY_H_GENERAL: *value = r.h_general; break;
        case CCSD_QUERY_GEO_EK: *value = r.geo; break;
        case CCSD_QUERY_H_WIDE: *value = r.h_wide; break;
        case CCSD_QUERY_MLP_FORMS: {
            int64_t edge = 0;
            for (int l = 0; l < pl->h.a_L; ++l) edge |= (int64_t)(pl->h.al[l].mlp.chain != 0) << l;
            const int afin = r.lg && pl->afin_lg.chain ? pl->afin_lg.chain : pl->h.a_fin.chain;
            *value = pl->h.x_fin.chain + 16 * afin + 256 * edge;
            break;
        }
        default: return set_err(CCSD_ERR_INVALID, "unknown query");
    }
    return CCSD_OK;
}

static int corrector_norms(ccsd_plan* pl, int B, int step, int it, const ccsd_state_t* base, const ccsd_state_t* cur,
                           const float* flags, const ccsd_noise_t* noise, uint64_t seed, int64_t off, float* sums,
                           Workspace& w, void* stream, bool keep_net = true, bool r2_done = false) {
    const PlanD& p = pl->h;
    int st = CCSD_OK;
    NoiseArgs na = make_noise(noise, seed, off, draw_base(pl, step, it), pl->rt.corrector_flat);
    const Route& rt = pl->rt;
    Pass ps;
    enum { NR_NONE, NR_R2, NR_EW1_RIDE, NR_EW1, NR_TILED };
    const bool same_r2 = cur->rank2 == base->rank2, own_draw = na.flat_r && !na.zr;
    const int form = !p.is_cc ? NR_NONE : rt.r2_family == R2_FUSED && same_r2 ? NR_R2 : rt.r2_family != R2_EW1 ? NR_TILED
                   : rt.ew1_fuse && own_draw && same_r2 ? NR_EW1_RIDE : NR_EW1;
    const bool z_rides = form == NR_TILED && rt.tiled_fuse && own_draw;
    RankEpi ep = norms_epi(w);
    P0Fuse pf{};
    int ntiles = w.ntiles;
    switch (form) {
    case NR_R2:
        if (r2_done) ps.p1_raw = r2_p1_raw(p);
        else if ((st = launch_r2(pl, B, cur->rank2, cur->adj, flags, 1, ep, na, ps, w, stream))) return st;
        ntiles = 1;
        break;
    case NR_EW1_RIDE:
        pf = p0_fuse(pl, 3, na, na.draw_r, w);
        pf.zrow = w.part; pf.alpha = p.f_alpha; pf.gamma = p.f_gamma;
        pf.net_out = keep_net ? w.net_r : nullptr;
        ntiles = p.E;
        break;
    case NR_TILED:
        if (z_rides) { pf = p0_fuse(pl, 1, na, na.draw_r, w); pf.zrow = w.zpart; }
        break;
    }
    if (form != NR_R2) st = launch_p(pl, B, cur->adj, base->rank2, ps, w, stream, pf.mode ? &pf : nullptr);
    if (st) return st;
    XaArgs xa{};
    xa.xX = cur->x; xa.adjX = base->adj;
    xa.xA = base->x; xa.adjA = cur->adj;
    xa.flags = flags; xa.do_x = xa.do_a = 1; xa.mode = MODE_NORMS;
    xa.out_x = w.net_x; xa.out_a = w.net_adj; xa.norm2 = w.norm2;
    if ((st = launch_xa(pl, B, xa, na, ps, w, stream, form == NR_R2 && r2_done))) return st;
    if (form == NR_EW1) {
        if ((st = launch_ew1(pl, B, cur->rank2, ep, na, w, stream, keep_net ? w.net_r : nullptr))) return st;
        ntiles = w.nchunk;
    } else if (form == NR_TILED) {
        if ((st = launch_h(pl, B, cur->rank2, ps, w, stream))) return st;
        if ((st = launch_hf(pl, B, cur->rank2, ep, na, w, stream))) return st;
    }
    const float* part = w.part;
    if (form != NR_NONE && form != NR_R2) {
        const bool zk = form == NR_TILED && own_draw;
        if (zk && !z_rides) {
#define NN_GO(EC_, KC_) CCSD_LAUNCH((k_noise_norm<EC_, KC_>), dim3(w.nchunk, B), dim3(CCSD_NTHREADS), 0, stream, na, w.masks(), p.E, p.K, w.zpart)
            GEO_EK(pl->rt.geo, NN_GO);
#undef NN_GO
            LAUNCH_CHECK();
        }
        if (zk || ntiles > 8) {
            CCSD_LAUNCH(k_normpart, dim3(B), dim3(CCSD_NTHREADS), 0, stream, (const float*)w.part, ntiles, zk ? (const float*)w.zpart : (const float*)nullptr,
                        z_rides ? p.E : w.nchunk, w.part2);
            LAUNCH_CHECK();
            part = w.part2; ntiles = 1;
        }
    }
    CCSD_LAUNCH(k_normsum, dim3(1), dim3(CCSD_NTHREADS == 1 ? 1 : normsum_threads(B)), 0, stream, (const float*)w.norm2, part, B, ntiles,
                p.is_cc, sums);
    LAUNCH_CHECK();
    return CCSD_OK;
}
static int corrector_apply(ccsd_plan* pl, int B, int step, int it, const ccsd_state_t* cur, const float* flags,
                           const ccsd_noise_t* noise, uint64_t seed, int64_t off, const float* sums, ccsd_state_t* out,
                           Workspace& w, void* stream) {
    const PlanD& p = pl->h;
    NoiseArgs na = make_noise(noise, seed, off, draw_base(pl, step, it), pl->rt.corrector_flat);
    LangArgs a = lang_args(pl, B, step, cur, flags, sums, out, w);
    const long long total = state_items(p, B, 1);
    prof_mark(pl, KID_LANGEVIN, stream);
#define LA_GO(EC_, KC_) CCSD_LAUNCH((k_langevin_apply<EC_, KC_>), dim3(grid_for(total, 256)), dim3(CCSD_NTHREADS), 0, stream, a, na, w.masks())
    GEO_EK(pl->rt.geo, LA_GO);
#undef LA_GO
    prof_mark(pl, KID_LANGEVIN, stream);
    LAUNCH_CHECK();
    return CCSD_OK;
}
static int predictor(ccsd_plan* pl, int B, int step, const ccsd_state_t* in, const float* flags, const ccsd_noise_t* noise,
                     uint64_t seed, int64_t off, ccsd_state_t* out, ccsd_state_t* mean, Workspace& w, void* stream,
                     const float* fuse_sums = nullptr, bool merge_next = false) {
    const PlanD& p = pl->h;
    int st = CCSD_OK;
    NoiseArgs na = make_noise(noise, seed, off, draw_base(pl, step, pl->cfg.n_corr_steps), pl->rt.predictor_flat);
    const ccsd_step_coef_t* c = &pl->coef[(size_t)step * 3];
    const Route& rt = pl->rt;
    Pass ps;
    enum { PR_NONE, PR_R2, PR_EW1_ONEPASS, PR_EW1, PR_TILED_APPLY, PR_TILED };
    const int form = !p.is_cc ? PR_NONE : rt.r2_family == R2_FUSED ? PR_R2
                   : rt.r2_family == R2_EW1 ? (fuse_sums && rt.ew1_fuse && !na.zr ? PR_EW1_ONEPASS : PR_EW1)
                   : fuse_sums && rt.tiled_fuse ? PR_TILED_APPLY : PR_TILED;
    CorrFuse cf{};
    if (fuse_sums) {
        cf.on = 1; cf.net_x = w.net_x; cf.net_adj = w.net_adj; cf.net_r = w.net_r; cf.lc = lang_coef(pl, step, fuse_sums);
        const unsigned int cb = draw_base(pl, step, 0);
        cf.draw_x = cb; cf.draw_adj = cb + 1; cf.draw_r = cb + 2;
    }
    RankEpi ep = pred_epi(pl, step, out, mean);
    P0Fuse pf{};
    const float* p_in = in->rank2;
    const float* r2_in = in->rank2;
    const int md = merge_next ? (int)draw_base(pl, step + 1, 0) + 2 : -1;
    switch (form) {
    case PR_R2:
        if ((st = launch_r2(pl, B, in->rank2, in->adj, flags, 1, ep, na, ps, w, stream, &cf, md))) return st;
        break;
    case PR_EW1_ONEPASS:
        pf = p0_fuse(pl, 4, na, cf.draw_r, w);
        pf.draw_pred = na.draw_r; pf.cf = cf;
        pf.alpha = p.f_alpha; pf.gamma = p.f_gamma; pf.pa = c[2].pa; pf.pb = c[2].pb; pf.pc = c[2].pc;
        pf.out = out->rank2; pf.mean = mean ? mean->rank2 : nullptr;
        pf.f1 = w.net_r;
        break;
    case PR_EW1:
        if ((st = launch_ew1(pl, B, in->rank2, ep, na, w, stream, nullptr, &cf, w.net_r))) return st;
        if (cf.on) p_in = w.net_r;
        break;
    case PR_TILED_APPLY:
        pf = p0_fuse(pl, 2, na, cf.draw_r, w);
        pf.net = w.net_r; pf.f1 = w.net_r; pf.cf = cf;
        r2_in = w.net_r;
        break;
    }
    if (form != PR_R2) st = launch_p(pl, B, in->adj, p_in, ps, w, stream, pf.mode ? &pf : nullptr);
    if (st) return st;
    XaArgs xa{};
    xa.xX = xa.xA = in->x; xa.adjX = xa.adjA = in->adj; xa.flags = flags;
    xa.do_x = xa.do_a = 1; xa.mode = MODE_PRED;
    xa.pa_x = c[0].pa; xa.pb_x = c[0].pb; xa.pc_x = c[0].pc;
    xa.pa_a = c[1].pa; xa.pb_a = c[1].pb; xa.pc_a = c[1].pc;
    xa.out_x = out->x; xa.out_a = out->adj;
    xa.mean_x = mean ? mean->x : nullptr; xa.mean_a = mean ? mean->adj : nullptr;
    xa.cf = cf;
    if ((st = launch_xa(pl, B, xa, na, ps, w, stream))) return st;
    if (form == PR_TILED_APPLY || form == PR_TILED) {
        if ((st = launch_h(pl, B, r2_in, ps, w, stream))) return st;
        if ((st = launch_hf(pl, B, r2_in, ep, na, w, stream))) return st;
    }
    return CCSD_OK;
}

static int s4_apply(ccsd_plan* pl, int B, int step, const ccsd_state_t* cur, const float* flags, const ccsd_noise_t* n1,
                    const ccsd_noise_t* n2, const ccsd_noise_t* n3, uint64_t seed, int64_t off, const float* sums,
                    ccsd_state_t* out, ccsd_state_t* mean, Workspace& w, void* stream) {
    const PlanD& p = pl->h;
    S4Args q{};
    q.a = lang_args(pl, B, step, cur, flags, sums, out, w);
    for (int t = 0; t < 3; ++t) {
        const ccsd_step_coef_t& c = pl->coef[(size_t)step * 3 + t];
        q.m1[t] = c.m1; q.s1[t] = c.s1; q.d[t] = c.d; q.m2[t] = c.m2; q.s2[t] = c.s2;
    }
    q.mx = mean ? mean->x : nullptr; q.madj = mean ? mean->adj : nullptr; q.mr = mean ? mean->rank2 : nullptr;
    NoiseArgs na1 = make_noise(n1, seed, off, draw_base(pl, step, 0));
    NoiseArgs na2 = make_noise(n2, seed, off, draw_base(pl, step, 1));
    NoiseArgs na3 = make_noise(n3, seed, off, draw_base(pl, step, 2));
    prof_mark(pl, KID_S4, stream);
    CCSD_LAUNCH(k_s4_apply, dim3(grid_for(state_items(p, B, 0), 256)), dim3(CCSD_NTHREADS), 0, stream, q, na1, na2, na3,
                (const unsigned long long*)w.offbits, (const unsigned char*)pl->edges, (const unsigned long long*)pl->cells);
    prof_mark(pl, KID_S4, stream);
    LAUNCH_CHECK();
    return CCSD_OK;
}

static int check_step(const ccsd_plan* pl, int step) {
    if (step < 0 || step >= pl->cfg.diff_steps) return set_err(CCSD_ERR_INVALID, "step out of range");
    return CCSD_OK;
}

extern "C" int ccsd_corrector_norms(ccsd_plan_t* pl, int32_t B, int32_t step, int32_t corr_iter, const ccsd_state_t* base,
                                    const ccsd_state_t* cur, const float* flags, const ccsd_noise_t* noise, uint64_t seed,
                                    int64_t sample_offset, float* norm_sums, void* workspace, size_t ws_bytes, void* stream) {
    Workspace w{};
    int st = check_common(pl, B, flags, workspace, ws_bytes, w);
    if (st || (st = check_step(pl, step)) || (st = check_state(pl, base, "base")) || (st = check_state(pl, cur, "cur"))) return st;
    if (!norm_sums) return set_err(CCSD_ERR_INVALID, "NULL norm_sums");
    if ((st = launch_flagbits(pl, B, flags, w, stream))) return st;
    return corrector_norms(pl, B, step, corr_iter, base, cur, flags, noise, seed, sample_offset, norm_sums, w, stream);
}
extern "C" int ccsd_corrector_apply(ccsd_plan_t* pl, int32_t B, int32_t step, int32_t corr_iter, const ccsd_state_t* cur,
                                    const float* flags, const ccsd_noise_t* noise, uint64_t seed, int64_t sample_offset,
                                    const float* norm_sums, ccsd_state_t* out, void* workspace, size_t ws_bytes, void* stream) {
    Workspace w{};
    int st = check_common(pl, B, flags, workspace, ws_bytes, w);
    if (st || (st = check_step(pl, step)) || (st = check_state(pl, cur, "cur")) || (st = check_state(pl, out, "out"))) return st;
    if (!norm_sums) return set_err(CCSD_ERR_INVALID, "NULL norm_sums");
    if ((st = launch_flagbits(pl, B, flags, w, stream))) return st;
    return corrector_apply(pl, B, step, corr_iter, cur, flags, noise, seed, sample_offset, norm_sums, out, w, stream);
}
extern "C" int ccsd_predictor(ccsd_plan_t* pl, int32_t B, int32_t step, const ccsd_state_t* in, const float* flags,
                              const ccsd_noise_t* noise, uint64_t seed, int64_t sample_offset, ccsd_state_t* out,
                              ccsd_state_t* mean, void* workspace, size_t ws_bytes, void* stream) {
    Workspace w{};
    int st = check_common(pl, B, flags, workspace, ws_bytes, w);
    if (!st && pl->cfg.predictor == CCSD_PRED_S4) return set_err(CCSD_ERR_INVALID, "S4 plans step with ccsd_corrector_norms + ccsd_s4_apply");
    if (st || (st = check_step(pl, step)) || (st = check_state(pl, in, "in")) || (st = check_state(pl, out, "out"))) return st;
    if (mean && (st = check_state(pl, mean, "mean"))) return st;
    if (in->x == out->x || in->adj == out->adj || (pl->h.is_cc && in->rank2 == out->rank2))
        return set_err(CCSD_ERR_INVALID, "predictor cannot run in place");
    if ((st = launch_flagbits(pl, B, flags, w, stream))) return st;
    return predictor(pl, B, step, in, flags, noise, seed, sample_offset, out, mean, w, stream);
}

extern "C" int ccsd_s4_apply(ccsd_plan_t* pl, int32_t B, int32_t step, const ccsd_state_t* cur, const float* flags,
                             const ccsd_noise_t* noise1, const ccsd_noise_t* noise2, const ccsd_noise_t* noise3, uint64_t seed,
                             int64_t sample_offset, const float* norm_sums, ccsd_state_t* out, ccsd_state_t* mean,
                             void* workspace, size_t ws_bytes, void* stream) {
    Workspace w{};
    int st = check_common(pl, B, flags, workspace, ws_bytes, w);
    if (st || (st = check_step(pl, step)) || (st = check_state(pl, cur, "cur")) || (st = check_state(pl, out, "out"))) return st;
    if (mean && (st = check_state(pl, mean, "mean"))) return st;
    if (pl->cfg.predictor != CCSD_PRED_S4) return set_err(CCSD_ERR_INVALID, "ccsd_s4_apply needs a plan created with CCSD_PRED_S4");
    if (!norm_sums) return set_err(CCSD_ERR_INVALID, "NULL norm_sums");
    if ((st = launch_flagbits(pl, B, flags, w, stream))) return st;
    return s4_apply(pl, B, step, cur, flags, noise1, noise2, noise3, seed, sample_offset, norm_sums, out, mean, w, stream);
}

extern "C" int ccsd_sampler_run_ex(ccsd_plan_t* pl, int32_t B, const float* flags, uint64_t seed, int64_t sample_offset,
                                   int32_t first_step, int32_t last_step, ccsd_state_t* state, ccsd_state_t* scratch,
                                   ccsd_state_t* result, float* traj, void* workspace, size_t ws_bytes, void* stream,
                                   const ccsd_run_options_t* options) {
    Workspace w{};
    int st = check_common(pl, B, flags, workspace, ws_bytes, w);
    if (st || (st = check_state(pl, state, "state")) || (st = check_state(pl, scratch, "scratch")) ||
        (st = check_state(pl, result, "result"))) return st;
    if (first_step < 0 || last_step > pl->cfg.diff_steps || first_step >= last_step) return set_err(CCSD_ERR_INVALID, "bad step range");
    const Route& rt = pl->rt;
    const PlanD& p = pl->h;
    if ((st = launch_flagbits(pl, B, flags, w, stream))) return st;
    const size_t nx = (size_t)p.N * p.F, na = (size_t)p.N * p.N, nr = p.is_cc ? (size_t)p.E * p.K : 0;
    ccsd_state_t a = *state, b = *scratch;
#define REDUCE_SUMS() do { if (options && options->reduce && options->reduce(w.sums, 6, stream, options->user)) \
                               return set_err(CCSD_ERR_CALLBACK, "the reduce hook of ccsd_sampler_run_ex failed"); } while (0)
    for (int step = first_step; step < last_step; ++step) {
        const bool lastone = step == last_step - 1;
        const bool want_mean = pl->cfg.denoise && (lastone || traj);
        if (rt.loop == LOOP_S4) {
            if ((st = corrector_norms(pl, B, step, 0, &a, &a, flags, nullptr, seed, sample_offset, w.sums, w, stream))) return st;
            REDUCE_SUMS();
            if ((st = s4_apply(pl, B, step, &a, flags, nullptr, nullptr, nullptr, seed, sample_offset, w.sums, &b,
                               want_mean ? result : nullptr, w, stream))) return st;
            ccsd_state_t t = a; a = b; b = t;
        } else if (rt.loop == LOOP_LANGEVIN_FUSED) {
            const bool r2_done = rt.merged && step > first_step;
            const bool merge_next = rt.merged && !lastone;
            if ((st = corrector_norms(pl, B, step, 0, &a, &a, flags, nullptr, seed, sample_offset, w.sums, w, stream, rt.r2_family == R2_FUSED, r2_done))) return st;
            REDUCE_SUMS();
            if (rt.merged && !r2_done && r2_p1_raw(p))
                RT_CHECK(rt_d2d_async(w.U1b, w.U1, (size_t)B * p.h_pw * 4, stream));
            if ((st = predictor(pl, B, step, &a, flags, nullptr, seed, sample_offset, &b, want_mean ? result : nullptr, w, stream, w.sums, merge_next))) return st;
            ccsd_state_t t = a; a = b; b = t;
        } else if (rt.loop == LOOP_LANGEVIN || (rt.loop == LOOP_LANGEVIN_MULTI && pl->cfg.n_corr_steps > 0)) {
            const ccsd_state_t* cur = &a;
            for (int it = 0; it < pl->cfg.n_corr_steps; ++it) {
                ccsd_state_t* out = (it & 1) ? &w.third : &b;
                if ((st = corrector_norms(pl, B, step, it, &a, cur, flags, nullptr, seed, sample_offset, w.sums, w, stream))) return st;
                REDUCE_SUMS();
                if ((st = corrector_apply(pl, B, step, it, cur, flags, nullptr, seed, sample_offset, w.sums, out, w, stream))) return st;
                cur = out;
            }
            if ((st = predictor(pl, B, step, cur, flags, nullptr, seed, sample_offset, &a, want_mean ? result : nullptr, w, stream))) return st;
        } else {
            if ((st = predictor(pl, B, step, &a, flags, nullptr, seed, sample_offset, &b, want_mean ? result : nullptr, w, stream))) return st;
            ccsd_state_t t = a; a = b; b = t;
        }
        if (traj) {
            const ccsd_state_t* src = pl->cfg.denoise ? result : &a;
            float* slot = traj + (size_t)step * (nx + na + nr);
            if ((st = copy_state(ccsd_state_t{slot, slot + nx, slot + nx + na}, *src, p, 1, stream))) return st;
        }
    }
#undef REDUCE_SUMS
    if (a.x != state->x) st = copy_state(*state, a, p, B, stream);
    if (!st && !pl->cfg.denoise) st = copy_state(*result, a, p, B, stream);
    return st;
}
extern "C" int ccsd_sampler_run(ccsd_plan_t* pl, int32_t B, const float* flags, uint64_t seed, int64_t sample_offset,
                                int32_t first_step, int32_t last_step, ccsd_state_t* state, ccsd_state_t* scratch,
                                ccsd_state_t* result, float* traj, void* workspace, size_t ws_bytes, void* stream) {
    return ccsd_sampler_run_ex(pl, B, flags, seed, sample_offset, first_step, last_step, state, scratch, result, traj, workspace, ws_bytes, stream, nullptr);
}

#include "ccsd_api_samples.h"
```

### ccsd_amd/csrc/ccsd_k_r2.h

```cpp
#pragma once
#include "ccsd_baked_qm9.h"
#include "ccsd_rank2_common.h"

#ifndef CCSD_R2_LB
#define CCSD_R2_LB 4
#endif
struct R2Args {
    const float* rank2; const float* adj; const float* flags;
    const unsigned long long* offbits;
    float* P0; float* P1;
    float* U1;
    int want_p;
    int masked;
    int merge;
    unsigned int draw_r2;
    float* P0b; float* P1b; float* U1b;
    float* net2; float* part2;
    int ldk, ldh;
    long long* dbg;
    const float* wp;
    CorrFuse cf;
};

template <int MT, int RS, bool AFFINE, bool GEN1, int QM9 = 0>
__global__ __launch_bounds__(512, 4) void k_r2(const PlanD* __restrict__ plan, const float* __restrict__ w,
                                            const unsigned char* __restrict__ edges,
                                            const unsigned long long* __restrict__ cells, R2Args ra, RankEpi ep,
                                            NoiseArgs na) {
    CCSD_DYN_SMEM(sm);
    constexpr bool BAKED = QM9 == 2 && CCSD_BAKED_QM9_SIZE == sizeof(PlanD);
    const PlanD& pw = *plan;
    const PlanD& p = BAKED ? *reinterpret_cast<const PlanD*>(CCSD_BAKED_QM9_PLAN) : *plan;
    const int E = QM9 ? 36 : p.E, K = QM9 ? 466 : p.K, N = QM9 ? 9 : p.N, NN = N * N, ldk = QM9 ? 488 : ra.ldk, ldh = QM9 ? 36 : ra.ldh;
    const int b = blockIdx.x, tid = threadIdx.x, nth = blockDim.x;
    const int Kp4 = (K + 31) & ~31, Ep4 = (E + 3) & ~3;
    float* sF = sm;
    float* sH = sF + E * ldk;
    float* sFl = sH + E * ldh;
    float* sRow = sFl + 64;
    float* sAco = sRow + 64;
    float* sAdj = sAco + p.a_cinit * E;
    float* sRed = sAdj + 3 * NN;
    unsigned char* sFrb = reinterpret_cast<unsigned char*>(sRed + 64);
#ifndef CCSD_EMU
    __shared__ int s_hdone;
#endif
    const float* Fg = ra.rank2 + (size_t)b * E * K;
    const FastDiv dK(K);
    constexpr bool ST = AFFINE && !GEN1 && MT == 3 && RS == 1;
    constexpr int MTF = ST ? MT - 1 : MT;
    constexpr int E0 = 16 * MTF;

    stamp(ra.dbg, 0);
#ifndef CCSD_EMU
    if (tid == 0) s_hdone = 0;
#endif
    const unsigned long long off = ra.offbits[b];
    const int hodge2 = (p.h_L > 1) && ra.want_p;
    const bool adjpow = hodge2 && p.hl[0].mval.n > 1;
    auto build_tables = [&](auto&& between) {
        unsigned long long cw[2];
        unsigned int ew = 0;
#pragma unroll
        for (int u = 0; u < 2; ++u) { const int k = tid + u * nth; cw[u] = cells[k < K ? k : K - 1]; }
        if (tid < 64) ew = *reinterpret_cast<const unsigned short*>(edges + 2 * (tid < E ? tid : E - 1));
        between();
#pragma unroll
        for (int u = 0; u < 2; ++u) { const int k = tid + u * nth; if (k < Kp4) sFrb[k] = (k < K && !(cw[u] & off)) ? 1 : 0; }
        for (int k = tid + 2 * nth; k < Kp4; k += nth) sFrb[k] = (k < K && !(cells[k] & off)) ? 1 : 0;
        if (tid < 64) sFl[tid] = (tid < E && !(((off >> (ew & 0xffu)) | (off >> (ew >> 8))) & 1ull)) ? 1.f : 0.f;
        for (int e = tid + nth; e < 64; e += nth) sFl[e] = e < E ? edge_on(off, edges, e) : 0.f;
        for (int t = tid; t < E * (Kp4 - K); t += nth) { const int e = t / (Kp4 - K), k = K + t % (Kp4 - K); sF[e * ldk + k] = 0.f; }
        if (adjpow) {
            float c1a = 0.f, c2a = 0.f;
            if (ra.cf.on) langevin_coef(ra.cf.lc, 1, &c1a, &c2a);
            for (int i = tid; i < NN; i += nth) {
                float v = ra.adj[(size_t)b * NN + i];
                if (ra.cf.on) {
                    NoiseArgs nc = na;
                    nc.zadj = nullptr; nc.draw_adj = ra.cf.draw_adj;
                    const int ii = i / N, jj = i % N;
                    const float z = raw_noise_adj(nc, b, ii, jj, N) * ra.flags[(size_t)b * N + ii] * ra.flags[(size_t)b * N + jj];
                    v = corr_apply(c1a, c2a, ra.cf.net_adj[(size_t)b * NN + i], v, z);
                }
                sAdj[i] = v; sAdj[NN + i] = v;
            }
        }
        __syncthreads();
        stamp(ra.dbg, 8);
    };
    float s_net = 0.f, s_z = 0.f;
    {
        float c1f = 0.f, c2f = 0.f;
        if (ra.cf.on) langevin_coef(ra.cf.lc, 2, &c1f, &c2f);
        NoiseArgs nc = na;
        if (ra.cf.on) { nc.zr = nullptr; nc.draw_r = ra.cf.draw_r; }
        const bool znorm = ep.mode == MODE_NORMS && na.flat_r, zuse = znorm || ra.cf.on;
        const float* Ng = ra.cf.on ? ra.cf.net_r + (size_t)b * E * K : Fg;
        const int EK = E * K;
        if ((EK & 3) == 0 && (K & 1) == 0) {
            const float4* F4 = reinterpret_cast<const float4*>(Fg);
            const float4* N4 = reinterpret_cast<const float4*>(Ng);
            const float4* Z4 = reinterpret_cast<const float4*>(nc.zr ? nc.zr + (size_t)b * EK : Fg);
            const int n4 = EK >> 2;
            const FastDiv dK2(K >> 1);
            auto phase0 = [&](auto LB_, auto CF_, auto ZN_) {
                constexpr int LB = decltype(LB_)::value;
                constexpr bool CF = decltype(CF_)::value;
                constexpr bool ZN = decltype(ZN_)::value;
                constexpr int LN = CF ? LB : 1;
                float4 va[LB], vb[LB], qa[LN], qb[LN];
                auto issue = [&](float4* v, float4* q, int base) {
#pragma unroll
                    for (int u = 0; u < LB; ++u) { const int i4 = base + u * nth; v[u] = F4[i4 < n4 ? i4 : n4 - 1]; }
                    if (CF) {
#pragma unroll
                        for (int u = 0; u < LB; ++u) { const int i4 = base + u * nth; q[CF ? u : 0] = N4[i4 < n4 ? i4 : n4 - 1]; }
                    }
                };
                auto consume = [&](const float4* v, const float4* q, int base) {
#pragma unroll
                    for (int u = 0; u < LB; ++u) {
                        const int i4 = base + u * nth;
                        if (i4 < n4) {
                            int e, kp;
                            dK2.divmod(2 * i4, e, kp);
                            const int k = 2 * kp;
                            const bool wrap = k + 2 == K;
                            const int e1 = wrap ? e + 1 : e, k1 = wrap ? 0 : k + 2;
                            float vv[4] = {v[u].x, v[u].y, v[u].z, v[u].w};
                            if (CF || ZN) {
                                float z[4];
                                if (nc.zr) { const float4 z4 = Z4[i4]; z[0] = z4.x; z[1] = z4.y; z[2] = z4.z; z[3] = z4.w; }
                                else philox_normal4(nc.seed, nc.draw_r, nc.b_off + b, (unsigned)i4, z);
                                const unsigned f0 = *reinterpret_cast<const unsigned short*>(sFrb + k), f1 = *reinterpret_cast<const unsigned short*>(sFrb + k1);
                                const float fl0 = sFl[e], fl1 = sFl[e1];
                                const float m[4] = {fl0 * (float)(f0 & 0xffu), fl0 * (float)(f0 >> 8), fl1 * (float)(f1 & 0xffu), fl1 * (float)(f1 >> 8)};
                                const float4 n4v = q[CF ? u : 0];
                                const float nn[4] = {n4v.x, n4v.y, n4v.z, n4v.w};
#pragma unroll
                                for (int j = 0; j < 4; ++j) {
                                    const float zz = z[j] * m[j];
                                    if (ZN && !CF) s_z = fmaf(zz, zz, s_z);
                                    if (CF) vv[j] = corr_apply(c1f, c2f, nn[j], vv[j], zz);
                                }
                                if (CF && ZN) {
                                    float z2[4];
                                    philox_normal4(na.seed, ra.draw_r2, na.b_off + b, (unsigned)i4, z2);
#pragma unroll
                                    for (int j = 0; j < 4; ++j) { const float zz = z2[j] * m[j]; s_z = fmaf(zz, zz, s_z); }
                                }
                            }
                            *reinterpret_cast<float2*>(sF + e * ldk + k) = make_float2(vv[0], vv[1]);
                            *reinterpret_cast<float2*>(sF + e1 * ldk + k1) = make_float2(vv[2], vv[3]);
                        }
                    }
                };
                const int step = LB * nth;
                int base = tid;
                build_tables([&]() { issue(va, qa, base); });
                while (true) {
                    const bool more_b = base - tid + step < n4;
                    if (more_b) issue(vb, qb, base + step);
                    consume(va, qa, base);
                    if (!more_b) break;
                    base += step;
                    const bool more_a = base - tid + step < n4;
                    if (more_a) issue(va, qa, base + step);
                    consume(vb, qb, base);
                    if (!more_a) break;
                    base += step;
                }
            };
            typedef std::integral_constant<bool, true> T_;
            typedef std::integral_constant<bool, false> F_;
            if (ra.cf.on && ra.merge) phase0(std::integral_constant<int, 3>{}, T_{}, T_{});
            else if (ra.cf.on) phase0(std::integral_constant<int, 3>{}, T_{}, F_{});
            else if (znorm) phase0(std::integral_constant<int, 3>{}, F_{}, T_{});
            else phase0(std::integral_constant<int, 3>{}, F_{}, F_{});
        } else {
            build_tables([]() {});
            for (int t = tid; t < EK; t += nth) {
                int e, k;
                dK.divmod(t, e, k);
                float v = Fg[t];
                if (zuse) {
                    const float z = nc.zr ? nc.zr[(size_t)b * EK + t] : philox_normal1(nc.seed, nc.draw_r, nc.b_off + b, (unsigned)t);
                    const float zz = z * sFl[e] * (float)sFrb[k];
                    if (znorm) s_z = fmaf(zz, zz, s_z);
                    if (ra.cf.on) v = corr_apply(c1f, c2f, Ng[t], v, zz);
                }
                sF[e * ldk + k] = v;
            }
        }
    }
    stamp(ra.dbg, 9);
    if (adjpow) {
        float* A = sAdj; float* P0_ = sAdj + NN; float* P1_ = sAdj + 2 * NN;
        for (int c = 0; c < p.a_cinit; ++c) {
            for (int e = tid; e < E; e += nth) sAco[c * E + e] = P0_[edges[2 * e] * N + edges[2 * e + 1]];
            if (c + 1 < p.a_cinit) {
                for (int i = tid; i < NN; i += nth) {
                    const int r = i / N, cc = i % N;
                    float acc = 0.f;
                    for (int kk = 0; kk < N; ++kk) acc = fmaf(P0_[r * N + kk], A[kk * N + cc], acc);
                    P1_[i] = acc;
                }
                __syncthreads();
                float* t2 = P0_; P0_ = P1_; P1_ = t2;
            }
            __syncthreads();
        }
    }
    __syncthreads();
    const int npass = ra.merge ? 2 : 1;
    for (int pass = 0; pass < npass; ++pass) {
    const bool wb = ra.merge && pass == 0;
    if (pass == 1) {
        __syncthreads();
        ep.mode = MODE_NORMS; ep.out = ra.net2; ep.mean = nullptr; ep.part = ra.part2;
        na.zr = nullptr; na.draw_r = ra.draw_r2; na.flat_r = 1;
        ra.P0 = ra.P0b; ra.P1 = ra.P1b; ra.U1 = ra.U1b;
#ifndef CCSD_EMU
        if (tid == 0) s_hdone = 0;
#endif
        __syncthreads();
    }
    stamp(ra.dbg, 1);
#ifdef CCSD_STOP_DIAG
    const int diag = ra.dbg ? (int)ra.dbg[((size_t)gridDim.x + 254) * 64 + 62] : 0;
#else
    constexpr int diag = 0;
#endif
    const HodgeLayerD& h0 = p.hl[0];
    const HodgeLayerD& h1 = p.hl[1];
    const bool doP0 = ra.want_p && p.h_L > 0, doP1 = hodge2;
    const bool lin1 = doP1 && h0.mval.n == 1;
    const bool pm = !GEN1 && lin1 && ra.masked;
    const int wc0 = doP0 ? h0.wc : 0, wc1 = doP1 ? p.h_pw : 0;

    stamp(ra.dbg, 2);
    const int ks = Kp4 >> 2;
    int nHtasks = 0;
    const int nHf = p.f_cnum == 2 ? MTF * (MTF + 1) / 2 : 0, nHs = (ST && p.f_cnum == 2) ? MT : 0;
    const int nH = nHf + nHs;
    const int nt0 = doP0 ? (wc0 + 15) >> 4 : 0, nt1 = doP1 ? (wc1 + 15) >> 4 : 0;
    const int nPf = MTF * (nt0 + nt1);
    const int ntask = nH + nPf + (ST ? nt0 + nt1 : 0);
#ifdef CCSD_EMU
    (void)ks; (void)ntask;
    for (int m = 0; m < E; ++m) {
        for (int n = 0; n < E; ++n) {
            float acc = 0.f;
            if (p.f_cnum == 2) for (int kk = 0; kk < K; ++kk) acc = fmaf(sF[m * ldk + kk], sF[n * ldk + kk], acc);
            sH[m * ldh + n] = (p.f_hmask && m == n) ? 0.f : acc;
        }
        for (int n = 0; n < wc0; ++n) {
            float acc = 0.f;
            for (int kk = 0; kk < K; ++kk) acc = fmaf(sF[m * ldk + kk], w[h0.wcat + (size_t)kk * wc0 + n], acc);
            ra.P0[((size_t)b * E + m) * wc0 + n] = acc;
        }
        for (int n = 0; n < wc1; ++n) {
            float acc = 0.f, un = 0.f;
            int ll = 1;
            while (ll + 1 < p.h_L && n >= p.h_poff[ll + 1]) ++ll;
            const HodgeLayerD& hn = ccsd_hl(p, ll);
            const int nl = n - p.h_poff[ll];
            for (int kk = 0; kk < K; ++kk) {
                const float frk = (float)sFrb[kk], wv = nl < hn.wc ? w[hn.wcat + (size_t)kk * hn.wc + nl] : 0.f;
                float a;
                if (lin1) a = sF[m * ldk + kk] * frk;
                else {
                    float in[CCSD_SMALLW], out[CCSD_SMALLW];
                    for (int c = 0; c < CCSD_SMALLW; ++c) in[c] = c < h0.cin ? sAco[c * E + m] * sF[m * ldk + kk] : 0.f;
                    small_mlp<CCSD_SMALLW>(h0.mval, w, in, out);
                    a = sFl[m] * out[0] * frk;
                }
                acc = fmaf(a, wv, acc);
                un = fmaf(frk, wv, un);
            }
            ra.P1[((size_t)b * E + m) * wc1 + n] = acc;
            if (lin1 && m == 0 && !pm) ra.U1[(size_t)b * wc1 + n] = un;
        }
    }
#endif
#ifndef CCSD_EMU
    typedef float r2_f32x4 __attribute__((ext_vector_type(4)));
    const int nblk = Kp4 >> 4;
    const float* WT0 = ra.wp + h0.wcatT;
    const float* WT1 = ra.wp + h1.wcatT;
    const bool hmask = p.f_hmask != 0;
    auto run_tile = [&](int t) {
        const int lane = tid & 63, l15 = lane & 15, kq = lane >> 4;
        int type, i, c;
        bool strip = false;
        if (t < nHf) {
            type = 0; i = 0;
            int rem = t;
            while (rem >= MTF - i) { rem -= MTF - i; ++i; }
            c = i + rem;
        } else if (t < nH) {
            type = 0; i = MTF; c = t - nHf; strip = true;
        } else if (t < nH + MTF * nt0) {
            type = 1; i = (t - nH) / nt0; c = (t - nH) % nt0;
        } else if (t < nH + nPf) {
            type = 2; i = (t - nH - MTF * nt0) / nt1; c = (t - nH - MTF * nt0) % nt1;
        } else if (t < nH + nPf + nt0) {
            type = 1; i = MTF; c = t - nH - nPf; strip = true;
        } else {
            type = 2; i = MTF; c = t - nH - nPf - nt0; strip = true;
        }
        const int ra_ = strip ? E0 + (l15 & 3) : 16 * i + l15;
        const int arow = ra_ < E ? ra_ : E - 1;
        const float* pa = sF + arow * ldk + 4 * kq;
        int offB = 0;
        const float* wtp = WT0;
        if (type == 0) {
            const int rb_ = 16 * c + l15;
            offB = (rb_ < E ? rb_ : E - 1) * ldk + 4 * kq;
        } else {
            const int wcn = type == 1 ? wc0 : wc1, n = 16 * c + l15;
            wtp = (type == 1 ? WT0 : WT1) + (size_t)(n < wcn ? n : wcn - 1) * Kp4 + 4 * kq;
        }
        r2_f32x4 acc0 = {0.f, 0.f, 0.f, 0.f}, acc1 = {0.f, 0.f, 0.f, 0.f};
        float upart = 0.f;
        auto kloop = [&](auto LB, auto K1, auto SR) {
            constexpr bool lb = decltype(LB)::v, k1 = decltype(K1)::v, sr = decltype(SR)::v;
            auto ldB = [&](int blk) -> float4 {
                if (lb) return *reinterpret_cast<const float4*>(sF + offB + 16 * blk);
                return *reinterpret_cast<const float4*>(wtp + 16 * blk);
            };
            constexpr int D = 4;
            float4 ab[D], bb[D];
            unsigned int fb[D];
#pragma unroll
            for (int u = 0; u < D; ++u) {
                const int bl = u < nblk ? u : nblk - 1;
                ab[u] = *reinterpret_cast<const float4*>(pa + 16 * bl);
                bb[u] = ldB(bl);
                fb[u] = k1 ? *reinterpret_cast<const unsigned int*>(sFrb + 16 * bl + 4 * kq) : 0u;
            }
            auto block = [&](int u, int blk, bool refill) {
                float4 a4 = ab[u];
                const float4 b4 = bb[u];
                if (k1) {
                    const unsigned int f4 = fb[u];
                    const float fr0 = (float)(f4 & 0xffu), fr1 = (float)((f4 >> 8) & 0xffu), fr2 = (float)((f4 >> 16) & 0xffu),
                                fr3 = (float)(f4 >> 24);
                    if (GEN1) {
                        const int e = arow;
                        float fv[4] = {a4.x, a4.y, a4.z, a4.w};
                        const float frv[4] = {fr0, fr1, fr2, fr3};
#pragma unroll
                        for (int j = 0; j < 4; ++j) {
                            float iin[CCSD_SMALLW], out[CCSD_SMALLW];
#pragma unroll
                            for (int cc = 0; cc < CCSD_SMALLW; ++cc) iin[cc] = cc < h0.cin ? sAco[cc * E + e] * fv[j] : 0.f;
                            small_mlp<CCSD_SMALLW>(h0.mval, w, iin, out);
                            fv[j] = sFl[e] * out[0] * frv[j];
                        }
                        a4 = make_float4(fv[0], fv[1], fv[2], fv[3]);
                    } else {
                        a4.x *= fr0; a4.y *= fr1; a4.z *= fr2; a4.w *= fr3;
                        if (!sr) upart = fmaf(fr0, b4.x, fmaf(fr1, b4.y, fmaf(fr2, b4.z, fmaf(fr3, b4.w, upart))));
                    }
                }
                r2_f32x4& acc = (u & 1) ? acc1 : acc0;
                if (sr) {
                    acc = __builtin_amdgcn_mfma_f32_4x4x1f32(a4.x, b4.x, acc, 0, 0, 0);
                    acc = __builtin_amdgcn_mfma_f32_4x4x1f32(a4.y, b4.y, acc, 0, 0, 0);
                    acc = __builtin_amdgcn_mfma_f32_4x4x1f32(a4.z, b4.z, acc, 0, 0, 0);
                    acc = __builtin_amdgcn_mfma_f32_4x4x1f32(a4.w, b4.w, acc, 0, 0, 0);
                } else {
                    acc = __builtin_amdgcn_mfma_f32_16x16x4f32(a4.x, b4.x, acc, 0, 0, 0);
                    acc = __builtin_amdgcn_mfma_f32_16x16x4f32(a4.y, b4.y, acc, 0, 0, 0);
                    acc = __builtin_amdgcn_mfma_f32_16x16x4f32(a4.z, b4.z, acc, 0, 0, 0);
                    acc = __builtin_amdgcn_mfma_f32_16x16x4f32(a4.w, b4.w, acc, 0, 0, 0);
                }
                if (refill) {
                    __builtin_amdgcn_sched_barrier(0);
                    const int bl = blk + D < nblk ? blk + D : nblk - 1;
                    ab[u] = *reinterpret_cast<const float4*>(pa + 16 * bl);
                    bb[u] = ldB(bl);
                    if (k1) fb[u] = *reinterpret_cast<const unsigned int*>(sFrb + 16 * bl + 4 * kq);
                    __builtin_amdgcn_sched_barrier(0);
                }
            };
            int blk0 = 0;
            for (; blk0 + D <= nblk; blk0 += D) {
#pragma unroll
                for (int u = 0; u < D; ++u) block(u, blk0 + u, true);
            }
#pragma unroll
            for (int u = 0; u < D - 1; ++u)
                if (blk0 + u < nblk) block(u, blk0 + u, false);
        };
        if ((diag & 1) && type != 0) { (void)0; }
        else if ((diag & 2) && type == 0) { (void)0; }
        else
        if (ST && strip) {
            if (type == 2 && !pm) kloop(BoolTag<false>{}, BoolTag<true>{}, BoolTag<true>{});
            else if (type == 0) kloop(BoolTag<true>{}, BoolTag<false>{}, BoolTag<true>{});
            else kloop(BoolTag<false>{}, BoolTag<false>{}, BoolTag<true>{});
        } else {
            if (type == 2 && !pm) kloop(BoolTag<false>{}, BoolTag<true>{}, BoolTag<false>{});
            else if (type == 0) kloop(BoolTag<true>{}, BoolTag<false>{}, BoolTag<false>{});
            else kloop(BoolTag<false>{}, BoolTag<false>{}, BoolTag<false>{});
        }
        r2_f32x4 acc = acc0 + acc1;
        const int n = 16 * c + l15;
        if (ST && strip) {
            float v = 0.f;
#pragma unroll
            for (int r = 0; r < 4; ++r) {
                const float tot = rows_allsum(acc[r]);
                v = kq == r ? tot : v;
            }
            const int m = E0 + kq;
            if (type == 0) {
                if (n < E && m < E) {
                    const float hv = (hmask && m == n) ? 0.f : v;
                    sH[m * ldh + n] = hv;
                    sH[n * ldh + m] = hv;
                }
                __builtin_amdgcn_fence(__ATOMIC_RELEASE, "workgroup");
                if (lane == 0) atomicAdd(&s_hdone, 1);
            } else {
                const int wcn = type == 1 ? wc0 : wc1;
                float* const dstp = type == 1 ? ra.P0 : ra.P1;
                if (n < wcn && m < E) dstp[((size_t)b * E + m) * wcn + n] = v;
            }
            return;
        }
        const int mb = 16 * i + 4 * kq;
        if (type == 0) {
            if (n < E) {
#pragma unroll
                for (int r = 0; r < 4; ++r) {
                    const int m = mb + r;
                    if (m < E) {
                        const float hv = (hmask && m == n) ? 0.f : acc[r];
                        sH[m * ldh + n] = hv;
                        sH[n * ldh + m] = hv;
                    }
                }
            }
            __builtin_amdgcn_fence(__ATOMIC_RELEASE, "workgroup");
            if (lane == 0) atomicAdd(&s_hdone, 1);
        } else if (type == 1) {
            if (n < wc0) {
                float* dst = ra.P0 + ((size_t)b * E + mb) * wc0 + n;
#pragma unroll
                for (int r = 0; r < 4; ++r)
                    if (mb + r < E) dst[(size_t)r * wc0] = acc[r];
            }
        } else {
            float un = upart;
            un += __shfl_xor(un, 16, 64);
            un += __shfl_xor(un, 32, 64);
            if (n < wc1) {
                float* dst = ra.P1 + ((size_t)b * E + mb) * wc1 + n;
#pragma unroll
                for (int r = 0; r < 4; ++r)
                    if (mb + r < E) dst[(size_t)r * wc1] = acc[r];
                if (!GEN1 && i == 0 && kq == 0 && !pm) ra.U1[(size_t)b * wc1 + n] = un;
            }
        }
    };
    nHtasks = nH;
    const int nw1 = nth >> 6, wave1 = wave_index();
    int n1 = ntask;
    if (AFFINE && !wb) {
        n1 = ((nH + nw1 - 1) / nw1) * nw1;
        if (n1 > ntask) n1 = ntask;
    }
    for (int t = wave1; t < n1; t += nw1) {
        run_tile(t);
        if (t == 0) stamp(ra.dbg, 6);
    }

    stamp(ra.dbg, 7);
    if (wb) __syncthreads();
    else if (nHtasks > 0) {
        unsigned spins = 0;
        while (__hip_atomic_load(&s_hdone, __ATOMIC_ACQUIRE, __HIP_MEMORY_SCOPE_WORKGROUP) < nHtasks) {
            __builtin_amdgcn_s_sleep(8);
            if (++spins == (1u << 27)) __builtin_trap();
        }
    }
#endif

    stamp(ra.dbg, 3);
    const bool eznorm = !na.flat_r;
    const int ntn = (K + 15) >> 4, ksE = Ep4 >> 2;
    auto epi4 = [&](int e0, int k, const float* hf) {
        if (e0 >= E || k >= K) return;
        float z[4] = {0.f, 0.f, 0.f, 0.f};
        if (ep.mode == MODE_PRED || (ep.mode == MODE_NORMS && eznorm)) raw_noise_r4(na, b, e0 >> 2, k, E, K, z);
        const float fr = (float)sFrb[k];
#pragma unroll
        for (int r = 0; r < 4; ++r) {
            const int e = e0 + r;
            if (e >= E) continue;
            const float f = sF[e * ldk + k];
            const float m = sFl[e] * fr;
            const float hf1[CCSD_MAXCN - 1] = {hf[r], 0.f, 0.f};
            const float net = fnet_element<AFFINE>(pw, w, f, hf1, m);
            const size_t gi = ((size_t)b * E + e) * K + k;
            if (ep.mode == MODE_SCORE) {
                ep.out[gi] = ep.sscale * net;
            } else {
                const float zz = z[r] * m;
                if (ep.mode == MODE_NORMS) {
                    ep.out[gi] = net;
                    s_net = fmaf(net, net, s_net);
                    if (eznorm) s_z = fmaf(zz, zz, s_z);
                } else {
// ... 445 lines not shown
```

### ccsd_amd/csrc/ccsd_k_update.h

```cpp
#pragma once
#include "ccsd_rank2_common.h"

__global__ void k_normsum(const float* __restrict__ norm2, const float* __restrict__ part, int B, int ntiles,
                          int is_cc, float* __restrict__ sums) {
    __shared__ float red[16 * 6];
    float acc[6] = {0.f, 0.f, 0.f, 0.f, 0.f, 0.f};
    for (int b = threadIdx.x; b < B; b += blockDim.x) {
        const float4 n4 = *reinterpret_cast<const float4*>(norm2 + (size_t)b * 4);
        acc[0] += sqrtf(n4.x);
        acc[1] += sqrtf(n4.y);
        acc[3] += sqrtf(n4.z);
        acc[4] += sqrtf(n4.w);
        if (is_cc) {
            float sn = 0.f, sz = 0.f;
            for (int t = 0; t < ntiles; ++t) {
                const float* p2 = part + ((size_t)b * ntiles + t) * 2;
                sn += p2[0];
                sz += p2[1];
            }
            acc[2] += sqrtf(sn);
            acc[5] += sqrtf(sz);
        }
    }
#ifdef CCSD_EMU
    for (int i = 0; i < 6; ++i) sums[i] = acc[i];
#else
    const int wave = wave_index(), lane = threadIdx.x & 63, nw = (blockDim.x + 63) >> 6;
#pragma unroll
    for (int i = 0; i < 6; ++i) {
        float v = acc[i];
#pragma unroll
        for (int o = 32; o > 0; o >>= 1) v += __shfl_xor(v, o, 64);
        if (lane == 0) red[wave * 6 + i] = v;
    }
    __syncthreads();
    if (threadIdx.x < 6) {
        float t = 0.f;
        for (int w = 0; w < nw; ++w) t += red[w * 6 + threadIdx.x];
        sums[threadIdx.x] = t;
    }
#endif
}

__global__ void k_normpart(const float* __restrict__ part, int ntiles, const float* __restrict__ zpart, int nchunk,
                           float* __restrict__ out) {
    __shared__ float red[64];
    const int b = blockIdx.x;
    float sn = 0.f, sz = 0.f;
    for (int t = threadIdx.x; t < ntiles; t += blockDim.x) {
        const float* p2 = part + ((size_t)b * ntiles + t) * 2;
        sn += p2[0];
        sz += p2[1];
    }
    if (zpart)
        for (int c = threadIdx.x; c < nchunk; c += blockDim.x) sz += zpart[(size_t)b * nchunk + c];
    const float tn = block_sum(sn, red);
    const float tz = block_sum(sz, red);
    if (threadIdx.x == 0) { out[(size_t)b * 2 + 0] = tn; out[(size_t)b * 2 + 1] = tz; }
}

#define CCSD_NN_CH 4096
template <int EC = 0, int KC = 0>
__global__ void k_noise_norm(NoiseArgs na, MaskTab mt, int E_, int K_, float* __restrict__ zpart) {
    __shared__ float red[64];
    const int E = EC ? EC : E_, K = KC ? KC : K_;
    const int b = blockIdx.y, EK = E * K, ng = (EK + 3) >> 2;
    const int g0 = blockIdx.x * CCSD_NN_CH, g1 = g0 + CCSD_NN_CH < ng ? g0 + CCSD_NN_CH : ng;
    float acc = 0.f;
    for (int g = g0 + threadIdx.x; g < g1; g += blockDim.x) {
        float z[4];
        raw_noise_rflat4(na, b, g, EK, z);
        int e, k;
        flat_split(4 * g, K, e, k);
        float m[4];
        group_masks(mt, b, E, K, e, k, m);
#pragma unroll
        for (int s = 0; s < 4; ++s) {
            if (4 * g + s < EK) {
                const float zz = z[s] * m[s];
                acc = fmaf(zz, zz, acc);
            }
        }
    }
    const float t = block_sum(acc, red);
    if (threadIdx.x == 0) zpart[(size_t)b * gridDim.x + blockIdx.x] = t;
}

struct LangArgs {
    const float* x; const float* adj; const float* r;
    const float* nx; const float* nadj; const float* nr;
    float* ox; float* oadj; float* orr;
    const float* flags;
    LangCoef lc;
    int B, N, F, E, K, is_cc;
};
template <int EC = 0, int KC = 0>
__global__ void k_langevin_apply(LangArgs a, NoiseArgs na, MaskTab mt) {
    if (EC) { a.E = EC; a.K = KC; }
    const long long nxe = (long long)a.B * a.N * a.F, nae = (long long)a.B * a.N * a.N;
    const int EK = a.E * a.K, ng = (EK + 3) >> 2;
    const long long nre = a.is_cc ? (long long)a.B * ng : 0;
    const long long total = nxe + nae + nre;
    const bool vec = (EK & 3) == 0;
    float c1x, c2x, c1a, c2a, c1r = 0.f, c2r = 0.f;
    langevin_coef(a.lc, 0, &c1x, &c2x);
    langevin_coef(a.lc, 1, &c1a, &c2a);
    if (a.is_cc) langevin_coef(a.lc, 2, &c1r, &c2r);
    for (long long t = (long long)blockIdx.x * blockDim.x + threadIdx.x; t < total; t += (long long)gridDim.x * blockDim.x) {
        if (t < nre) {
            const int b = (int)(t / ng), g = (int)(t - (long long)b * ng);
            const size_t base = (size_t)b * EK + 4 * (size_t)g;
            float v[4], nv[4], z[4];
            if (vec) {
                const float4 v4 = *reinterpret_cast<const float4*>(a.r + base), n4 = *reinterpret_cast<const float4*>(a.nr + base);
                v[0] = v4.x; v[1] = v4.y; v[2] = v4.z; v[3] = v4.w;
                nv[0] = n4.x; nv[1] = n4.y; nv[2] = n4.z; nv[3] = n4.w;
            } else {
#pragma unroll
                for (int s = 0; s < 4; ++s) {
                    const bool in = 4 * g + s < EK;
                    v[s] = in ? a.r[base + s] : 0.f;
                    nv[s] = in ? a.nr[base + s] : 0.f;
                }
            }
            raw_noise_rflat4(na, b, g, EK, z);
            int e, k;
            flat_split(4 * g, a.K, e, k);
            float o[4], m[4];
            group_masks(mt, b, a.E, a.K, e, k, m);
#pragma unroll
            for (int s = 0; s < 4; ++s)
                o[s] = corr_apply(c1r, c2r, nv[s], v[s], z[s] * m[s]);
            if (vec) *reinterpret_cast<float4*>(a.orr + base) = make_float4(o[0], o[1], o[2], o[3]);
            else {
#pragma unroll
                for (int s = 0; s < 4; ++s)
                    if (4 * g + s < EK) a.orr[base + s] = o[s];
            }
        } else if (t < nre + nxe) {
            const long long u = t - nre;
            const int per = a.N * a.F, b = (int)(u / per), idx = (int)(u % per), i = idx / a.F;
            const float z = raw_noise_x(na, b, idx, per) * a.flags[(size_t)b * a.N + i];
            a.ox[u] = corr_apply(c1x, c2x, a.nx[u], a.x[u], z);
        } else {
            const long long u = t - nre - nxe;
            const int per = a.N * a.N, b = (int)(u / per), ij = (int)(u % per), i = ij / a.N, j = ij % a.N;
            const float z = raw_noise_adj(na, b, i, j, a.N) * a.flags[(size_t)b * a.N + i] * a.flags[(size_t)b * a.N + j];
            a.oadj[u] = corr_apply(c1a, c2a, a.nadj[u], a.adj[u], z);
        }
    }
}

struct Ew1Args {
    const float* r; float* out; float* mean; float* f1; float* net_out; float* part;
    int mode, apply;
    float sscale, pa, pb, pc, alpha, gamma;
    const float* sums; float ss, sde_alpha, snr, seps; unsigned int draw_corr;
    int E, K;
    MaskTab mt;
};
template <int EC = 0, int KC = 0>
__global__ void k_ew1(Ew1Args a, NoiseArgs na) {
    __shared__ float red[64];
    if (EC) { a.E = EC; a.K = KC; }
    const int b = blockIdx.y, EK = a.E * a.K, ng = (EK + 3) >> 2;
    const int g0 = blockIdx.x * CCSD_NN_CH, g1 = g0 + CCSD_NN_CH < ng ? g0 + CCSD_NN_CH : ng;
    const bool vec = (EK & 3) == 0;
    float c1 = 0.f, c2 = 0.f;
    if (a.mode == MODE_PRED && a.apply) langevin_coef(LangCoef{a.sums, {0.f, 0.f, a.ss}, {0.f, 0.f, a.sde_alpha}, a.snr, a.seps}, 2, &c1, &c2);
    NoiseArgs nc = na;
    if (a.mode == MODE_PRED) { nc.zr = nullptr; nc.draw_r = a.draw_corr; }
    float s_net = 0.f, s_z = 0.f;
    for (int g = g0 + threadIdx.x; g < g1; g += blockDim.x) {
        const size_t base = (size_t)b * EK + 4 * (size_t)g;
        float v[4];
        if (vec) { const float4 v4 = *reinterpret_cast<const float4*>(a.r + base); v[0] = v4.x; v[1] = v4.y; v[2] = v4.z; v[3] = v4.w; }
        else {
#pragma unroll
            for (int s = 0; s < 4; ++s) v[s] = 4 * g + s < EK ? a.r[base + s] : 0.f;
        }
        int e, k;
        flat_split(4 * g, a.K, e, k);
        float m[4];
        group_masks(a.mt, b, a.E, a.K, e, k, m);
        float o[4], mu[4], w1[4], nt[4];
        float zc[4] = {0.f, 0.f, 0.f, 0.f}, zp[4] = {0.f, 0.f, 0.f, 0.f};
        if (a.mode == MODE_NORMS || (a.mode == MODE_PRED && a.apply)) raw_noise_rflat4(nc, b, g, EK, zc);
        if (a.mode == MODE_PRED) raw_noise_rflat4(na, b, g, EK, zp);
#pragma unroll
        for (int s = 0; s < 4; ++s) {
            float f = v[s];
            float net = ew1_net(a.alpha, a.gamma, m[s], f);
            if (a.mode == MODE_SCORE) {
                o[s] = a.sscale * net;
            } else if (a.mode == MODE_NORMS) {
                const float zz = zc[s] * m[s];
                nt[s] = net;
                s_net = fmaf(net, net, s_net);
                s_z = fmaf(zz, zz, s_z);
            } else {
                if (a.apply) {
                    f = corr_apply(c1, c2, net, f, zc[s] * m[s]);
                    w1[s] = f;
                    net = ew1_net(a.alpha, a.gamma, m[s], f);
                }
                const float mean = fmaf(a.pa, f, a.pb * net);
                mu[s] = mean;
                o[s] = fmaf(a.pc, zp[s] * m[s], mean);
            }
        }
        auto st4 = [&](float* dst, const float* val) {
            if (vec) *reinterpret_cast<float4*>(dst + base) = make_float4(val[0], val[1], val[2], val[3]);
            else {
#pragma unroll
                for (int s = 0; s < 4; ++s)
                    if (4 * g + s < EK) dst[base + s] = val[s];
            }
        };
        if (a.mode == MODE_NORMS) { if (a.net_out) st4(a.net_out, nt); }
        else {
            st4(a.out, o);
            if (a.mode == MODE_PRED) {
                if (a.apply) st4(a.f1, w1);
                if (a.mean) st4(a.mean, mu);
            }
        }
    }
    if (a.mode == MODE_NORMS) {
        const float tn = block_sum(s_net, red);
        const float tz = block_sum(s_z, red);
        if (threadIdx.x == 0) {
            a.part[((size_t)b * gridDim.x + blockIdx.x) * 2 + 0] = tn;
            a.part[((size_t)b * gridDim.x + blockIdx.x) * 2 + 1] = tz;
        }
    }
}

struct S4Args {
    LangArgs a;
    float m1[3], s1[3], d[3], m2[3], s2[3];
    float* mx; float* madj; float* mr;
};
CCSD_DEV float s4_chain(float v, float net, float z1, float z2, float z3, float c1, float c2, const S4Args& q, int t, float* mean) {
    const float v1 = corr_apply(c1, c2, net, v, z1);
    const float v2 = fmaf(q.s1[t], z2, q.m1[t] * v1);
    const float v3 = fmaf(q.d[t], net, v2);
    const float mu = q.m2[t] * v3;
    *mean = mu;
    return fmaf(q.s2[t], z3, mu);
}
__global__ void k_s4_apply(S4Args q, NoiseArgs n1, NoiseArgs n2, NoiseArgs n3, const unsigned long long* __restrict__ offbits,
                           const unsigned char* __restrict__ edges, const unsigned long long* __restrict__ cells) {
    const LangArgs& a = q.a;
    const long long nxe = (long long)a.B * a.N * a.F, nae = (long long)a.B * a.N * a.N;
    const long long nre = a.is_cc ? (long long)a.B * ((a.E + 3) / 4) * a.K : 0;
    const long long total = nxe + nae + nre;
    float c1x, c2x, c1a, c2a, c1r = 0.f, c2r = 0.f;
    langevin_coef(a.lc, 0, &c1x, &c2x);
    langevin_coef(a.lc, 1, &c1a, &c2a);
    if (a.is_cc) langevin_coef(a.lc, 2, &c1r, &c2r);
    for (long long t = (long long)blockIdx.x * blockDim.x + threadIdx.x; t < total; t += (long long)gridDim.x * blockDim.x) {
        float mu;
        if (t < nxe) {
            const int per = a.N * a.F, b = (int)(t / per), idx = (int)(t % per), i = idx / a.F;
            const float fl = a.flags[(size_t)b * a.N + i];
            a.ox[t] = s4_chain(a.x[t], a.nx[t], raw_noise_x(n1, b, idx, per) * fl, raw_noise_x(n2, b, idx, per) * fl,
                               raw_noise_x(n3, b, idx, per) * fl, c1x, c2x, q, 0, &mu);
            if (q.mx) q.mx[t] = mu;
        } else if (t < nxe + nae) {
            const long long u = t - nxe;
            const int per = a.N * a.N, b = (int)(u / per), ij = (int)(u % per), i = ij / a.N, j = ij % a.N;
            const float fl = a.flags[(size_t)b * a.N + i] * a.flags[(size_t)b * a.N + j];
            a.oadj[u] = s4_chain(a.adj[u], a.nadj[u], raw_noise_adj(n1, b, i, j, a.N) * fl, raw_noise_adj(n2, b, i, j, a.N) * fl,
                                 raw_noise_adj(n3, b, i, j, a.N) * fl, c1a, c2a, q, 1, &mu);
            if (q.madj) q.madj[u] = mu;
        } else {
            const long long u = t - nxe - nae;
            const int eg_n = (a.E + 3) / 4;
            const int k = (int)(u % a.K), eg = (int)((u / a.K) % eg_n), b = (int)(u / ((long long)a.K * eg_n));
            float z1[4], z2[4], z3[4];
            raw_noise_r4(n1, b, eg, k, a.E, a.K, z1);
            raw_noise_r4(n2, b, eg, k, a.E, a.K, z2);
            raw_noise_r4(n3, b, eg, k, a.E, a.K, z3);
            const unsigned long long off = offbits[b];
            const float fr = cell_on(off, cells, k);
#pragma unroll
            for (int s = 0; s < 4; ++s) {
                const int e = 4 * eg + s;
                if (e >= a.E) continue;
                const size_t gi = ((size_t)b * a.E + e) * a.K + k;
                const float m = edge_on(off, edges, e) * fr;
                a.orr[gi] = s4_chain(a.r[gi], a.nr[gi], z1[s] * m, z2[s] * m, z3[s] * m, c1r, c2r, q, 2, &mu);
                if (q.mr) q.mr[gi] = mu;
            }
        }
    }
}

__global__ void k_init_state(float* x, float* adj, float* r, const float* __restrict__ flags, NoiseArgs na,
                             const unsigned long long* __restrict__ offbits, const unsigned char* __restrict__ edges,
                             const unsigned long long* __restrict__ cells, int B, int N, int F, int E, int K, int is_cc) {
    const long long nxe = (long long)B * N * F, nae = (long long)B * N * N;
    const int eg_n = (E + 3) / 4, EK = E * K, ng = (EK + 3) >> 2;
    const long long nre = is_cc ? (na.flat_r ? (long long)B * ng : (long long)B * eg_n * K) : 0;
    const long long total = nxe + nae + nre;
    for (long long t = (long long)blockIdx.x * blockDim.x + threadIdx.x; t < total; t += (long long)gridDim.x * blockDim.x) {
        if (t >= nxe + nae && na.flat_r) {
            const long long u = t - nxe - nae;
            const int b = (int)(u / ng), g = (int)(u - (long long)b * ng);
            float z[4];
            raw_noise_rflat4(na, b, g, EK, z);
            const unsigned long long off = offbits[b];
            int e = (4 * g) / K, k = (4 * g) % K;
#pragma unroll
            for (int s = 0; s < 4; ++s) {
                if (4 * g + s < EK) r[(size_t)b * EK + 4 * g + s] = edge_on(off, edges, e) * z[s] * cell_on(off, cells, k);
                if (++k == K) { k = 0; ++e; }
            }
        } else if (t < nxe) {
            const int per = N * F, b = (int)(t / per), idx = (int)(t % per);
            x[t] = raw_noise_x(na, b, idx, per) * flags[(size_t)b * N + idx / F];
        } else if (t < nxe + nae) {
            const long long u = t - nxe;
            const int per = N * N, b = (int)(u / per), ij = (int)(u % per), i = ij / N, j = ij % N;
            adj[u] = raw_noise_adj(na, b, i, j, N) * flags[(size_t)b * N + i] * flags[(size_t)b * N + j];
        } else {
            const long long u = t - nxe - nae;
            const int k = (int)(u % K), eg = (int)((u / K) % eg_n), b = (int)(u / ((long long)K * eg_n));
            float z[4];
            raw_noise_r4(na, b, eg, k, E, K, z);
            const unsigned long long off = offbits[b];
            const float fr = cell_on(off, cells, k);
#pragma unroll
            for (int s = 0; s < 4; ++s) {
                const int e = 4 * eg + s;
                if (e < E) r[((size_t)b * E + e) * K + k] = edge_on(off, edges, e) * z[s] * fr;
            }
        }
    }
}

__global__ void k_quantize(const float* __restrict__ in, long long n, float thr, long long* __restrict__ out) {
    for (long long t = (long long)blockIdx.x * blockDim.x + threadIdx.x; t < n; t += (long long)gridDim.x * blockDim.x) {
        const float v = in[t];
// ... 45 lines not shown
```

### ccsd_amd/csrc/ccsd_rank2_common.h

```cpp
#pragma once
#include "ccsd_dev.h"

CCSD_DEV float edge_on(unsigned long long off, const unsigned char* __restrict__ edges, int e) {
    return ((off >> edges[2 * e]) | (off >> edges[2 * e + 1])) & 1ull ? 0.f : 1.f;
}
CCSD_DEV float cell_on(unsigned long long off, const unsigned long long* __restrict__ cells, int k) {
    return (cells[k] & off) ? 0.f : 1.f;
}

static inline __host__ __device__ int h_ld(int E) { return (E + 3) & ~3; }
struct MaskTab { const unsigned char* mfr; const unsigned char* mfl; int Kp, Ep; };
CCSD_DEV void group_masks(const MaskTab& mt, int b, int E, int K, int e, int k, float* m) {
    const unsigned char* fr = mt.mfr + (size_t)b * mt.Kp;
    const unsigned char* fl = mt.mfl + (size_t)b * mt.Ep;
    if ((K & 3) == 0) {
        const unsigned f4 = *reinterpret_cast<const unsigned*>(fr + k);
        const float l = (float)fl[e < E ? e : E - 1];
        m[0] = l * (float)(f4 & 0xffu); m[1] = l * (float)((f4 >> 8) & 0xffu); m[2] = l * (float)((f4 >> 16) & 0xffu); m[3] = l * (float)(f4 >> 24);
    } else {
#pragma unroll
        for (int s = 0; s < 4; ++s) {
            m[s] = (float)fl[e < E ? e : E - 1] * (float)fr[k];
            if (++k == K) { k = 0; ++e; }
        }
    }
}

enum { MODE_SCORE = 0, MODE_NORMS = 1, MODE_PRED = 2 };

struct RankEpi {
    int mode;
    float sscale;
    float pa, pb, pc;
    float* out;
    float* mean;
    float* part;
};

template <bool AFFINE, int FW = CCSD_FW>
CCSD_DEV float fnet_element(const PlanD& p, const float* __restrict__ w, float f, const float* hf, float m) {
    if (AFFINE) {
        float t = fmaf(p.f_alpha, f, p.f_gamma);
#pragma unroll
        for (int j = 1; j < CCSD_MAXCN; ++j)
            if (j < p.f_cnum) t = fmaf(p.f_betas[j], hf[j - 1], t);
        return m * t;
    }
    if (p.f_blk >= 0) {
        const float* fb = w + p.f_blk;
        const float* hd = fb + CCSD_FBLK_HEAD;
        float prev[8] = {f, p.f_cnum > 1 ? hf[0] : 0.f, p.f_cnum > 2 ? hf[1] : 0.f, p.f_cnum > 3 ? hf[2] : 0.f, 0.f, 0.f, 0.f, 0.f};
        float acc = 0.f;
#pragma unroll
        for (int i = 0; i < 8; ++i) acc = fmaf(prev[i], hd[i], acc);
#pragma unroll
        for (int l = 0; l < CCSD_MAXFL; ++l)
            if (l < p.f_L) {
                float o8[8];
                small_mlp_lds<8>(fb + l * CCSD_MAXLIN * CCSD_HWBLK, p.fl[l].n, prev, o8);
#pragma unroll
                for (int i = 0; i < 8; ++i) {
                    prev[i] = m * o8[i];
                    acc = fmaf(prev[i], hd[(l + 1) * 8 + i], acc);
                }
            }
        return m * (acc + hd[(CCSD_MAXFL + 1) * 8]);
    }
    float ch[FW];
#pragma unroll
    for (int i = 0; i < FW; ++i) ch[i] = 0.f;
    ch[0] = f;
#pragma unroll
    for (int j = 1; j < CCSD_MAXCN; ++j)
        if (j < p.f_cnum) ch[j] = hf[j - 1];
    int ci0 = 0, co0 = p.f_cnum;
    for (int l = 0; l < p.f_L; ++l) {
        float in[FW], out[FW];
#pragma unroll
        for (int i = 0; i < FW; ++i) {
            float v = 0.f;
#pragma unroll
            for (int j = 0; j < FW; ++j)
                if (j == ci0 + i) v = ch[j];
            in[i] = v;
        }
        small_mlp<FW>(p.fl[l], w, in, out);
        const int no = p.fl[l].out;
#pragma unroll
        for (int j = 0; j < FW; ++j)
#pragma unroll
            for (int i = 0; i < FW; ++i)
                if (i < no && j == co0 + i) ch[j] = m * out[i];
        ci0 = co0; co0 += no;
    }
    float out[FW];
    small_mlp<FW>(p.f_fin, w, ch, out);
    return m * out[0];
}

template <int D = 4, class LA, class LB, class EP>
CCSD_DEV void wave_tile(int m0, int n0, int ks, LA la, LB lb, EP ep) {
#ifdef CCSD_EMU
    for (int i = 0; i < 16; ++i)
        for (int j = 0; j < 16; ++j) {
            float acc = 0.f;
            for (int k = 0; k < 4 * ks; ++k) acc = fmaf(la(m0 + i, k), lb(k, n0 + j), acc);
            ep(m0 + i, n0 + j, acc);
        }
#else
    typedef float f32x4 __attribute__((ext_vector_type(4)));
    const int lane = threadIdx.x & 63, l15 = lane & 15, kq = lane >> 4;
    f32x4 acc = {0.f, 0.f, 0.f, 0.f};
    for (int s = 0; s < ks; s += D) {
        float a[D], bv[D];
#pragma unroll
        for (int u = 0; u < D; ++u) {
            const int sc = s + u < ks ? s + u : ks - 1;
            a[u] = la(m0 + l15, 4 * sc + kq);
            bv[u] = lb(4 * sc + kq, n0 + l15);
        }
#pragma unroll
        for (int u = 0; u < D; ++u)
            if (s + u < ks) acc = __builtin_amdgcn_mfma_f32_16x16x4f32(a[u], bv[u], acc, 0, 0, 0);
    }
#pragma unroll
    for (int r = 0; r < 4; ++r) ep(m0 + 4 * kq + r, n0 + l15, acc[r]);
#endif
}

template <class LA, class LB, class EP>
CCSD_DEV void wave_coltile(int n0, int mt, int ks, LA la, LB lb, EP ep4) {
#ifdef CCSD_EMU
    float acc[64][16];
    for (int i = 0; i < 16 * mt; ++i)
        for (int j = 0; j < 16; ++j) {
            float a = 0.f;
            for (int k = 0; k < 4 * ks; ++k) a = fmaf(la(i, k), lb(k, n0 + j), a);
            acc[i][j] = a;
        }
    for (int i = 0; i < 16 * mt; i += 4)
        for (int j = 0; j < 16; ++j) {
            const float v[4] = {acc[i][j], acc[i + 1][j], acc[i + 2][j], acc[i + 3][j]};
            ep4(i, n0 + j, v);
        }
#else
    typedef float f32x4 __attribute__((ext_vector_type(4)));
    const int lane = threadIdx.x & 63, l15 = lane & 15, kq = lane >> 4;
    f32x4 acc[4];
#pragma unroll
    for (int t = 0; t < 4; ++t) acc[t] = (f32x4){0.f, 0.f, 0.f, 0.f};
    int s = 0;
    for (; s + 4 <= ks; s += 4) {
        float bv[4], a[4][4];
#pragma unroll
        for (int u = 0; u < 4; ++u) bv[u] = lb(4 * (s + u) + kq, n0 + l15);
#pragma unroll
        for (int u = 0; u < 4; ++u)
#pragma unroll
            for (int t = 0; t < 4; ++t) a[u][t] = t < mt ? la(16 * t + l15, 4 * (s + u) + kq) : 0.f;
#pragma unroll
        for (int u = 0; u < 4; ++u)
#pragma unroll
            for (int t = 0; t < 4; ++t)
                if (t < mt) acc[t] = __builtin_amdgcn_mfma_f32_16x16x4f32(a[u][t], bv[u], acc[t], 0, 0, 0);
    }
    for (; s < ks; ++s) {
        const float bv = lb(4 * s + kq, n0 + l15);
#pragma unroll
        for (int t = 0; t < 4; ++t)
            if (t < mt) acc[t] = __builtin_amdgcn_mfma_f32_16x16x4f32(la(16 * t + l15, 4 * s + kq), bv, acc[t], 0, 0, 0);
    }
#pragma unroll
    for (int t = 0; t < 4; ++t)
        if (t < mt) {
            const float v[4] = {acc[t][0], acc[t][1], acc[t][2], acc[t][3]};
            ep4(16 * t + 4 * kq, n0 + l15, v);
        }
#endif
}

#ifndef CCSD_EMU
typedef float f32x4 __attribute__((ext_vector_type(4)));
CCSD_DEV void frag_mma(f32x4& acc, const float4& a, const float4& b) {
    const float av[4] = {a.x, a.y, a.z, a.w}, bv[4] = {b.x, b.y, b.z, b.w};
#pragma unroll
    for (int q = 0; q < 4; ++q) acc = __builtin_amdgcn_mfma_f32_16x16x4f32(av[q], bv[q], acc, 0, 0, 0);
}
CCSD_DEV void row_load4(float4& v, const float* src, int k, int K, bool vec) {
    if (vec && k + 3 < K) v = *reinterpret_cast<const float4*>(src + k);
    else {
        v.x = k < K ? src[k] : 0.f; v.y = k + 1 < K ? src[k + 1] : 0.f;
        v.z = k + 2 < K ? src[k + 2] : 0.f; v.w = k + 3 < K ? src[k + 3] : 0.f;
    }
}
#endif

CCSD_DEV float raw_noise_r1(const NoiseArgs& na, int b, int e, int k, int E, int K) {
    if (na.zr) return na.zr[((size_t)b * E + e) * K + k];
    float n[4];
    philox_normal4(na.seed, na.draw_r, na.b_off + b, (unsigned)((e >> 2) * K + k), n);
    const int s = e & 3;
    return s == 0 ? n[0] : s == 1 ? n[1] : s == 2 ? n[2] : n[3];
}

struct LangCoef { const float* sums; float ss[3], alpha[3]; float snr, seps; };
CCSD_DEV void langevin_coef(const LangCoef& lc, int t, float* c1, float* c2) {
    const float gn = fabsf(lc.ss[t]) * lc.sums[t], zn = lc.sums[3 + t];
    const float q = lc.snr * zn / gn;
    const float step = q * q * 2.f * lc.alpha[t];
    *c1 = step * lc.ss[t];
    *c2 = sqrtf(step * 2.f) * lc.seps;
}
CCSD_DEV float corr_apply(float c1, float c2, float net, float v, float zz) { return fmaf(c2, zz, fmaf(c1, net, v)); }
CCSD_DEV float pred_update(float pa, float pb, float pc, float v, float net, float zz, float* mean) {
    *mean = fmaf(pa, v, pb * net);
    return fmaf(pc, zz, *mean);
}
CCSD_DEV float ew1_net(float alpha, float gamma, float m, float f) { return m * fmaf(alpha, f, gamma); }
struct CorrFuse {
    int on;
    const float* net_x; const float* net_adj; const float* net_r;
    LangCoef lc;
    unsigned int draw_x, draw_adj, draw_r;
};
```

### include/ccsd_hip.h

```cpp
#ifndef CCSD_HIP_H
#define CCSD_HIP_H

#include <stddef.h>
#include <stdint.h>

#ifdef __cplusplus
extern "C" {
#endif

#define CCSD_ABI_VERSION 5

enum {
    CCSD_OK = 0,
    CCSD_ERR_INVALID = 1,
    CCSD_ERR_UNSUPPORTED = 2,
    CCSD_ERR_WEIGHTS = 3,
    CCSD_ERR_RUNTIME = 4,
    CCSD_ERR_WORKSPACE = 5,
    CCSD_ERR_CALLBACK = 6
};

enum { CCSD_SDE_VP = 0, CCSD_SDE_VE = 1, CCSD_SDE_SUBVP = 2 };
enum { CCSD_PRED_EULER = 0, CCSD_PRED_REVERSE = 1, CCSD_PRED_S4 = 2 };
enum { CCSD_CORR_NONE = 0, CCSD_CORR_LANGEVIN = 1 };
enum { CCSD_TARGET_X = 0, CCSD_TARGET_ADJ = 1, CCSD_TARGET_RANK2 = 2 };

typedef struct {
    float sscale, alpha, pa, pb, pc;
    float m1, s1, d, m2, s2;
} ccsd_step_coef_t;

typedef struct {
    int32_t abi_version;
    int32_t N, F, is_cc, d_min, d_max;
    int32_t x_depth, x_nhid;
    int32_t a_num_layers, a_num_linears, a_c_init, a_c_hid, a_c_final, a_nhid, a_adim, a_num_heads;
    int32_t a_is_cc_net, h_num_layers, h_num_linears, h_nhid, h_adim, h_c_hid, h_c_final, h_num_heads;
    int32_t f_num_layers, f_num_linears, f_nhid, f_c_hid, f_c_final, f_cnum, f_num_layers_mlp, f_use_hodge_mask;
    int32_t predictor, corrector, n_corr_steps, probability_flow, denoise;
    float snr, scale_eps;
    int32_t diff_steps;
    int32_t batch_hint;
    int32_t x_gmh, x_num_linears, x_c_init, x_c_hid, x_c_final, x_adim, x_num_heads;
    int32_t a_conv_mlp, x_conv_mlp;
} ccsd_config_t;

typedef struct ccsd_plan ccsd_plan_t;

int ccsd_plan_create(const ccsd_config_t* cfg, const float* weights, size_t n_weights,
                     const ccsd_step_coef_t* step_coef, ccsd_plan_t** out);
void ccsd_plan_destroy(ccsd_plan_t* plan);

size_t ccsd_weight_count(const ccsd_config_t* cfg);
void ccsd_rank2_dims(const ccsd_config_t* cfg, int32_t* E, int64_t* K);
size_t ccsd_workspace_bytes(const ccsd_plan_t* plan, int32_t B);

const char* ccsd_last_error(void);

typedef struct {
    float* x;
    float* adj;
    float* rank2;
} ccsd_state_t;

typedef struct {
    const float* zx;
    const float* zadj;
    const float* zrank2;
} ccsd_noise_t;

int ccsd_score(ccsd_plan_t* plan, int32_t target, int32_t B, const ccsd_state_t* in, const float* flags_dev,
               float sscale, float* out_dev, void* workspace, size_t workspace_bytes, void* stream);

int ccsd_init_state(ccsd_plan_t* plan, int32_t B, const float* flags_dev, const ccsd_noise_t* prior,
                    uint64_t seed, int64_t sample_offset, ccsd_state_t* state, void* stream);

int ccsd_noise_draws(ccsd_plan_t* plan, int32_t B, const float* flags_dev, uint64_t seed, int64_t sample_offset,
                     int32_t step, int32_t phase, ccsd_state_t* out, void* stream);

int ccsd_noise_draws_at(ccsd_plan_t* plan, int32_t B, const float* flags_dev, uint64_t seed, int64_t sample_offset,
                        uint32_t draw, int32_t flat_rank2, ccsd_state_t* out, void* stream);

enum {
    CCSD_QUERY_FUSED_R2 = 0,
    CCSD_QUERY_XA_VARIANT = 1,
    CCSD_QUERY_R2_LDS_BYTES = 2,
    CCSD_QUERY_XA_LDS_BYTES = 3,
    CCSD_QUERY_FUSED_LOOP = 4,
    CCSD_QUERY_MERGED_R2 = 5,
    CCSD_QUERY_EW1 = 6,
    CCSD_QUERY_LARGE_GRAPH = 7,
    CCSD_QUERY_R2_FAMILY = 8,
    CCSD_QUERY_R2_INSTANCE = 9,
    CCSD_QUERY_LOOP_FORM = 10,
    CCSD_QUERY_H_FULL = 11,
    CCSD_QUERY_HP_FULL = 12,
    CCSD_QUERY_P0_NARROW = 13,
    CCSD_QUERY_TILED_FUSE = 14,
    CCSD_QUERY_EW1_FUSE = 15,
    CCSD_QUERY_H_GENERAL = 16,
    CCSD_QUERY_GEO_EK = 17,
    CCSD_QUERY_H_WIDE = 18,
    CCSD_QUERY_MLP_FORMS = 19
};
int ccsd_plan_query(const ccsd_plan_t* plan, int32_t what, int64_t* value);

int ccsd_corrector_norms(ccsd_plan_t* plan, int32_t B, int32_t step, int32_t corr_iter,
                         const ccsd_state_t* base, const ccsd_state_t* cur, const float* flags_dev, const ccsd_noise_t* noise,
                         uint64_t seed, int64_t sample_offset, float* norm_sums_dev,
                         void* workspace, size_t workspace_bytes, void* stream);
int ccsd_corrector_apply(ccsd_plan_t* plan, int32_t B, int32_t step, int32_t corr_iter,
                         const ccsd_state_t* cur, const float* flags_dev, const ccsd_noise_t* noise,
                         uint64_t seed, int64_t sample_offset, const float* norm_sums_dev,
                         ccsd_state_t* out, void* workspace, size_t workspace_bytes, void* stream);

int ccsd_predictor(ccsd_plan_t* plan, int32_t B, int32_t step, const ccsd_state_t* in, const float* flags_dev,
                   const ccsd_noise_t* noise, uint64_t seed, int64_t sample_offset,
                   ccsd_state_t* out, ccsd_state_t* mean, void* workspace, size_t workspace_bytes, void* stream);

int ccsd_s4_apply(ccsd_plan_t* plan, int32_t B, int32_t step, const ccsd_state_t* cur, const float* flags_dev,
                  const ccsd_noise_t* noise1, const ccsd_noise_t* noise2, const ccsd_noise_t* noise3, uint64_t seed,
                  int64_t sample_offset, const float* norm_sums_dev, ccsd_state_t* out, ccsd_state_t* mean,
                  void* workspace, size_t workspace_bytes, void* stream);

int ccsd_sampler_run(ccsd_plan_t* plan, int32_t B, const float* flags_dev, uint64_t seed, int64_t sample_offset,
                     int32_t first_step, int32_t last_step, ccsd_state_t* state, ccsd_state_t* scratch,
                     ccsd_state_t* result, float* traj_dev, void* workspace, size_t workspace_bytes, void* stream);

typedef int (*ccsd_reduce_fn)(float* sums_dev, int32_t n, void* stream, void* user);
typedef struct {
    ccsd_reduce_fn reduce;
    void* user;
} ccsd_run_options_t;
int ccsd_sampler_run_ex(ccsd_plan_t* plan, int32_t B, const float* flags_dev, uint64_t seed, int64_t sample_offset,
                        int32_t first_step, int32_t last_step, ccsd_state_t* state, ccsd_state_t* scratch,
                        ccsd_state_t* result, float* traj_dev, void* workspace, size_t workspace_bytes, void* stream,
                        const ccsd_run_options_t* options);

int ccsd_quantize(const float* in_dev, int64_t n, float thr, int64_t* out_dev, void* stream);

int ccsd_rank2_cells(const float* rank2_dev, int32_t B, int32_t E, int64_t K, float thr, uint64_t* bits_dev,
                     int32_t* counts_dev, void* stream);

enum { CCSD_FINISH_ADJ_QUANTIZE = 0,
       CCSD_FINISH_ADJ_MOL = 1 };
typedef struct {
    int32_t B, N, F, E;
    int64_t K;
    int32_t d_min, d_max;
    int32_t adj_mode;
    float thr;
} ccsd_finish_dims_t;
typedef struct {
    int64_t* adj_int;
    int32_t* degree;
    int32_t* degree_hist;
    int32_t* edge_hist;
    int32_t* n_nodes;
    int32_t* x_hist;
    uint8_t* rank2_u8;
    uint64_t* rank2_cell_bits;
    int32_t* rank2_cell_count;
    int32_t* rank2_cell_hist;
    int32_t* rank2_nnz;
} ccsd_finish_out_t;
int ccsd_finish(const ccsd_finish_dims_t* dims, const ccsd_state_t* in, const float* flags_dev,
                const ccsd_finish_out_t* out, void* stream);

#define CCSD_CLUSTER_MAX_BINS 1024
int ccsd_cluster_hist(const float* adj_dev, int32_t B, int32_t N, int32_t adj_mode, float thr, const double* edges_dev, int32_t bins,
                      int32_t* tri2_dev, int32_t* cluster_hist_dev, void* stream);

#define CCSD_ORBITS 15
int ccsd_orbit_counts(const float* adj_dev, int32_t B, int32_t N, int32_t adj_mode, float thr, int64_t* node_orbits_dev,
                      int64_t* graph_orbits_dev, int32_t* orbit_nodes_dev, void* stream);

#define CCSD_NSPDK_MAX_NODES 64
#define CCSD_NSPDK_FEATURES 65537
int32_t ccsd_nspdk_row_capacity(int32_t N);
size_t ccsd_nspdk_workspace_bytes(int32_t B, int32_t N);
int ccsd_nspdk_features(const float* adj_dev, const int32_t* labels_dev, int32_t B, int32_t N, int32_t adj_mode, float thr,
                        int32_t* nnz_dev, int32_t* indices_dev, double* values_dev, void* workspace, size_t ws_bytes, void* stream);

size_t ccsd_nspdk_mmd_workspace_bytes(int32_t n1, int32_t n2);
int ccsd_nspdk_mmd(const int64_t* indptr1_dev, const int32_t* indices1_dev, const double* values1_dev, int32_t n1,
                   const int64_t* indptr2_dev, const int32_t* indices2_dev, const double* values2_dev, int32_t n2, void* workspace,
                   size_t ws_bytes, double* out_dev, void* stream);

enum { CCSD_MMD_EMD = 0,
       CCSD_MMD_TV = 1,
       CCSD_MMD_L2 = 2 };
enum { CCSD_MMD_INT32 = 0, CCSD_MMD_FP64 = 1 };
enum { CCSD_MMD_IS_HIST = 1,
       CCSD_MMD_DEGREE = 2,
       CCSD_MMD_F32_PMF = 4 };
#define CCSD_MMD_MAX_ROWS (1 << 20)
#define CCSD_MMD_MAX_BINS (1 << 16)
size_t ccsd_mmd_workspace_bytes(int32_t n1, int32_t n2, int32_t L);
int ccsd_mmd(const void* h1_dev, int32_t n1, const int32_t* lens1_dev, const void* h2_dev, int32_t n2, const int32_t* lens2_dev, int32_t L,
             int32_t dtype, int32_t kind, int32_t flags, double sigma, double distance_scaling, void* workspace_dev, size_t ws_bytes,
             double* out_dev, void* stream);

#define CCSD_EIG_MAXN 512
size_t ccsd_eig_workspace_bytes(int32_t B, int32_t n);
int ccsd_eigvalsh(const double* a_dev, int32_t B, int32_t n, double* w_dev, int32_t* sweeps_dev, void* workspace_dev, size_t ws_bytes,
                  void* stream);

size_t ccsd_spectral_workspace_bytes(int32_t B, int32_t N);
int ccsd_spectral_hist(const float* adj_dev, int32_t B, int32_t N, int32_t adj_mode, float thr, const double* edges_dev, int32_t bins,
                       int32_t* hist_dev, double* eig_dev, int32_t* n_eff_dev, void* workspace_dev, size_t ws_bytes, void* stream);

size_t ccsd_hodge_workspace_bytes(int32_t B, int32_t N);
int ccsd_hodge_spectrum(const float* adj_dev, const uint64_t* cell_bits_dev, int32_t B, int32_t N, int32_t d_min, int32_t d_max,
                        int32_t adj_mode, float thr, float* spectrum_dev, int32_t* sweeps_dev, void* workspace_dev, size_t ws_bytes,
                        void* stream);

int ccsd_profile_kernel(ccsd_plan_t* plan, int32_t kernel_id);
int ccsd_profile_stride(ccsd_plan_t* plan, int32_t stride);
int ccsd_profile_read(ccsd_plan_t* plan, int32_t kernel_id, int64_t* launches, double* total_ms);
int ccsd_profile_launches(ccsd_plan_t* plan, int32_t kernel_id, int64_t* launches);
int ccsd_debug_stamps(ccsd_plan_t* plan, void* dev_buffer);

#ifdef __cplusplus
}
#endif
#endif
```

Before: 4346 complexes/s.

## Fold per-step Langevin norm reduction into the rank-2 kernel, dropping k_normsum launch

In the fused Langevin loop, the separate single-block k_normsum reduction is removed. Each k_r2 block now reduces the rank-2 partial norms itself to compute its Langevin coefficients, and block 0 writes the global sums for the other passes. Partial buffers are double-buffered across steps so each step reads what the previous merged pass wrote. This saves one serial launch and grid-wide dependency per step, at the cost of every block redundantly reading and reducing B partials.

```diff
diff --git a/ccsd_amd/_lib.py b/ccsd_amd/_lib.py
--- a/ccsd_amd/_lib.py
+++ b/ccsd_amd/_lib.py
@@ -26,7 +26,7 @@
 ]
 QUERIES = {"fused_r2": 0, "xa_variant": 1, "r2_lds_bytes": 2, "xa_lds_bytes": 3, "fused_loop": 4, "merged_r2": 5, "ew1": 6, "large_graph": 7,
            "r2_family": 8, "r2_instance": 9, "loop_form": 10, "h_full": 11, "hp_full": 12, "p0_narrow": 13, "tiled_fuse": 14, "ew1_fuse": 15,
-           "h_general": 16, "geo_ek": 17, "h_wide": 18, "mlp_forms": 19}
+           "h_general": 16, "geo_ek": 17, "h_wide": 18, "mlp_forms": 19, "fold_sums": 20, "fold_last_run": 21}
 KERNEL_IDS = {"k_xa": 0, "k_gemm_p": 1, "k_hf_score": 2, "k_gemm_h": 3, "k_langevin_apply": 4, "k_r2": 5, "k_s4_apply": 6, "k_ew1": 7}
 
 
diff --git a/ccsd_amd/csrc/ccsd_api.h b/ccsd_amd/csrc/ccsd_api.h
--- a/ccsd_amd/csrc/ccsd_api.h
+++ b/ccsd_amd/csrc/ccsd_api.h
@@ -23,7 +23,7 @@
 }
 
 struct Knobs {
-    int no_fused_r2 = 0, hodge_general = 0, geo_off = 0, no_fused_apply = 0, no_h_full = 0, no_hp_full = 0, hp_full_norms = 0, split_bf16 = 0;
+    int no_fused_r2 = 0, hodge_general = 0, geo_off = 0, no_fused_apply = 0, no_h_full = 0, no_hp_full = 0, hp_full_norms = 0, split_bf16 = 0, no_sum_fold = 0;
     int xa_threads = 0, xa_prio = 0, lg_force = 0, xa_pass = -1, xa_gch = 0, no_mlp_wt = 0, verbose = 0;
     const char *dump_plan = nullptr, *dump_plan_name = nullptr;
 };
@@ -33,7 +33,7 @@
     k.no_fused_r2 = on("CCSD_NO_FUSED_R2"); k.hodge_general = on("CCSD_HODGE_GENERAL");
     k.geo_off = on("CCSD_NO_GEO") ? 1 : on("CCSD_NO_BAKE") ? 2 : 0;
     k.no_fused_apply = on("CCSD_NO_FUSED_APPLY"); k.no_h_full = on("CCSD_NO_H_FULL"); k.no_hp_full = on("CCSD_NO_HP_FULL");
-    k.hp_full_norms = on("CCSD_HP_FULL_NORMS");
+    k.hp_full_norms = on("CCSD_HP_FULL_NORMS"); k.no_sum_fold = on("CCSD_NO_SUM_FOLD");
     if (const char* v = getenv("CCSD_SPLIT_BF16")) k.split_bf16 = atoi(v) == 3 ? 3 : 0;
     if (const char* v = getenv("CCSD_XA_THREADS")) { const int t = atoi(v); if (t >= 64 && t <= 1024 && t % 64 == 0) k.xa_threads = t; }
     if (const char* v = getenv("CCSD_XA_PRIO")) k.xa_prio = atoi(v);
@@ -64,6 +64,7 @@
     unsigned hp_full_modes = 0;
     int loop = LOOP_PRED_ONLY;
     int merged = 0;
+    int fold_sums = 0;
     int tiled_fuse = 0;
     int ew1_fuse = 0;
     int corrector_flat = 0, predictor_flat = 0;
@@ -89,6 +90,7 @@
     size_t init_off_cap = 0;
     Knobs knobs;
     Route rt;
+    int last_run_folded = 0;
     mutable unsigned prof_mask = 0;
     mutable size_t prof_used[8] = {0, 0, 0, 0, 0, 0, 0, 0};
     mutable int prof_stride = 1;
@@ -207,6 +209,7 @@
     if (full_geo && r.tiled_fuse && p.hl[0].wc <= 16 && p.f_cnum == 2 && !k.no_hp_full)
         r.hp_full_modes = (r.loop == LOOP_LANGEVIN_FUSED ? 1u << 2 : 0u) | (k.hp_full_norms ? 1u << 1 : 0u);
     r.merged = r.loop == LOOP_LANGEVIN_FUSED && fused && mt == 3 && rs == 1 && aff && !gen1 && (K & 1) == 0 && ((E * K) & 3) == 0;
+    r.fold_sums = r.loop == LOOP_LANGEVIN_FUSED && fused && !gen1 && !k.no_sum_fold;
     r.corrector_flat = !s4;
     r.predictor_flat = ew1;
     return CCSD_OK;
@@ -224,7 +227,6 @@
     *threads = t > e->max_threads ? e->max_threads : t;
     return e;
 }
-static inline int normsum_threads(int B) { return B > 512 ? 1024 : B > 256 ? 512 : 256; }
 
 extern "C" const char* ccsd_last_error(void) { return g_last_error.c_str(); }
 
@@ -460,6 +462,7 @@
     unsigned char *mfr, *mfl;
     int Kp, Ep;
     float *H, *P0, *P1, *U1, *acoef, *net_x, *net_adj, *net_r, *norm2, *part, *sums, *chan, *zpart, *part2;
+    float* partb;
     float* psplit; size_t psplit_floats;
     float *P0b, *P1b, *U1b;
     int ntiles, nchunk;
@@ -520,6 +523,7 @@
       w.part = (float*)take((size_t)B * (np ? np : 1) * 2 * 4); }
     w.zpart = (float*)take((size_t)B * ((size_t)w.nchunk > E ? (size_t)w.nchunk : E ? E : 1) * 4);
     w.part2 = (float*)take((size_t)B * 2 * 4);
+    w.partb = w.part2;
     w.sums = (float*)take(64);
     w.chan = (float*)take(p.chan_global ? (size_t)B * p.chan_rows * p.N * p.N * 4 : 0);
     if (pl->rt.lg) {
@@ -668,8 +672,10 @@
     LAUNCH_CHECK();
     return CCSD_OK;
 }
+struct SumFold { const float* part_in = nullptr; float* part_next = nullptr; };
 static int launch_r2(const ccsd_plan* pl, int B, const float* rank2, const float* adj, const float* flags, int want_p,
-                     RankEpi& ep, NoiseArgs& na, Pass& ps, Workspace& w, void* stream, const CorrFuse* cf, int merge_draw);
+                     RankEpi& ep, NoiseArgs& na, Pass& ps, Workspace& w, void* stream, const CorrFuse* cf, int merge_draw,
+                     const SumFold* fold = nullptr);
 static int launch_p(const ccsd_plan* pl, int B, const float* adj, const float* rank2, Pass& ps, Workspace& w, void* stream, const P0Fuse* fuse = nullptr) {
     const PlanD& p = pl->h;
     const Route& rt = pl->rt;
@@ -973,15 +979,18 @@
 }
 
 static int launch_r2(const ccsd_plan* pl, int B, const float* rank2, const float* adj, const float* flags, int want_p,
-                     RankEpi& ep, NoiseArgs& na, Pass& ps, Workspace& w, void* stream, const CorrFuse* cf = nullptr, int merge_draw = -1) {
+                     RankEpi& ep, NoiseArgs& na, Pass& ps, Workspace& w, void* stream, const CorrFuse* cf = nullptr, int merge_draw = -1,
+                     const SumFold* fold) {
     const Route& rt = pl->rt;
     R2Args ra{};
     if (cf) ra.cf = *cf;
     ra.masked = (cf && cf->on) ? 1 : 0;
+    const bool folded = fold && fold->part_in && cf && cf->on;
     if (merge_draw >= 0) {
         ra.merge = 1; ra.draw_r2 = (unsigned)merge_draw;
-        ra.P0b = w.P0b; ra.P1b = w.P1b; ra.U1b = w.U1b; ra.net2 = w.net_r; ra.part2 = w.part;
-    }
+        ra.P0b = w.P0b; ra.P1b = w.P1b; ra.U1b = w.U1b; ra.net2 = w.net_r; ra.part2 = folded ? fold->part_next : w.part;
+    }
+    if (folded) { ra.fold = 1; ra.part_in = fold->part_in; ra.norm2 = w.norm2; ra.sums_out = w.sums; }
     ra.rank2 = rank2; ra.adj = adj; ra.flags = flags; ra.offbits = w.offbits; ra.P0 = w.P0; ra.P1 = w.P1; ra.U1 = w.U1; ra.want_p = want_p;
     ra.ldk = rt.r2_ldk; ra.ldh = rt.r2_ldh; ra.dbg = pl->dbg; ra.wp = pl->wp;
     if (want_p && pl->h.h_L > 1) ps.p1_raw = r2_p1_raw(pl->h);
@@ -1142,6 +1151,8 @@
         case CCSD_QUERY_XA_LDS_BYTES: *value = (int64_t)pl->h.xa_lds_floats * 4; break;
         case CCSD_QUERY_FUSED_LOOP: *value = r.loop == LOOP_LANGEVIN_FUSED; break;
         case CCSD_QUERY_MERGED_R2: *value = r.merged; break;
+        case CCSD_QUERY_FOLD_SUMS: *value = r.fold_sums; break;
+        case CCSD_QUERY_FOLD_LAST_RUN: *value = pl->last_run_folded; break;
         case CCSD_QUERY_EW1: *value = r.r2_family == R2_EW1; break;
         case CCSD_QUERY_LARGE_GRAPH: *value = r.lg; break;
         case CCSD_QUERY_R2_FAMILY: *value = r.r2_family; break;
@@ -1169,7 +1180,7 @@
 
 static int corrector_norms(ccsd_plan* pl, int B, int step, int it, const ccsd_state_t* base, const ccsd_state_t* cur,
                            const float* flags, const ccsd_noise_t* noise, uint64_t seed, int64_t off, float* sums,
-                           Workspace& w, void* stream, bool keep_net = true, bool r2_done = false) {
+                           Workspace& w, void* stream, bool keep_net = true, bool r2_done = false, const SumFold* fold = nullptr) {
     const PlanD& p = pl->h;
     int st = CCSD_OK;
     NoiseArgs na = make_noise(noise, seed, off, draw_base(pl, step, it), pl->rt.corrector_flat);
@@ -1181,6 +1192,8 @@
                    : rt.ew1_fuse && own_draw && same_r2 ? NR_EW1_RIDE : NR_EW1;
     const bool z_rides = form == NR_TILED && rt.tiled_fuse && own_draw;
     RankEpi ep = norms_epi(w);
+    const bool folded = fold && fold->part_in;
+    if (folded) ep.part = const_cast<float*>(fold->part_in);
     P0Fuse pf{};
     int ntiles = w.ntiles;
     switch (form) {
@@ -1230,6 +1243,7 @@
             part = w.part2; ntiles = 1;
         }
     }
+    if (folded) return form == NR_R2 ? CCSD_OK : set_err(CCSD_ERR_RUNTIME, "folded norm sums on a pass k_r2 does not serve");
     CCSD_LAUNCH(k_normsum, dim3(1), dim3(CCSD_NTHREADS == 1 ? 1 : normsum_threads(B)), 0, stream, (const float*)w.norm2, part, B, ntiles,
                 p.is_cc, sums);
     LAUNCH_CHECK();
@@ -1252,7 +1266,7 @@
 }
 static int predictor(ccsd_plan* pl, int B, int step, const ccsd_state_t* in, const float* flags, const ccsd_noise_t* noise,
                      uint64_t seed, int64_t off, ccsd_state_t* out, ccsd_state_t* mean, Workspace& w, void* stream,
-                     const float* fuse_sums = nullptr, bool merge_next = false) {
+                     const float* fuse_sums = nullptr, bool merge_next = false, const SumFold* fold = nullptr) {
     const PlanD& p = pl->h;
     int st = CCSD_OK;
     NoiseArgs na = make_noise(noise, seed, off, draw_base(pl, step, pl->cfg.n_corr_steps), pl->rt.predictor_flat);
@@ -1276,7 +1290,7 @@
     const int md = merge_next ? (int)draw_base(pl, step + 1, 0) + 2 : -1;
     switch (form) {
     case PR_R2:
-        if ((st = launch_r2(pl, B, in->rank2, in->adj, flags, 1, ep, na, ps, w, stream, &cf, md))) return st;
+        if ((st = launch_r2(pl, B, in->rank2, in->adj, flags, 1, ep, na, ps, w, stream, &cf, md, fold))) return st;
         break;
     case PR_EW1_ONEPASS:
         pf = p0_fuse(pl, 4, na, cf.draw_r, w);
@@ -1401,6 +1415,8 @@
     const PlanD& p = pl->h;
     if ((st = launch_flagbits(pl, B, flags, w, stream))) return st;
     const size_t nx = (size_t)p.N * p.F, na = (size_t)p.N * p.N, nr = p.is_cc ? (size_t)p.E * p.K : 0;
+    const bool folded = rt.fold_sums && !(options && options->reduce);
+    pl->last_run_folded = folded;
     ccsd_state_t a = *state, b = *scratch;
 #define REDUCE_SUMS() do { if (options && options->reduce && options->reduce(w.sums, 6, stream, options->user)) \
                                return set_err(CCSD_ERR_CALLBACK, "the reduce hook of ccsd_sampler_run_ex failed"); } while (0)
@@ -1416,11 +1432,13 @@
         } else if (rt.loop == LOOP_LANGEVIN_FUSED) {
             const bool r2_done = rt.merged && step > first_step;
             const bool merge_next = rt.merged && !lastone;
-            if ((st = corrector_norms(pl, B, step, 0, &a, &a, flags, nullptr, seed, sample_offset, w.sums, w, stream, rt.r2_family == R2_FUSED, r2_done))) return st;
+            SumFold sf;
+            if (folded) { const int par = (step - first_step) & 1; sf.part_in = par ? w.partb : w.part; sf.part_next = par ? w.part : w.partb; }
+            if ((st = corrector_norms(pl, B, step, 0, &a, &a, flags, nullptr, seed, sample_offset, w.sums, w, stream, rt.r2_family == R2_FUSED, r2_done, &sf))) return st;
             REDUCE_SUMS();
             if (rt.merged && !r2_done && r2_p1_raw(p))
                 RT_CHECK(rt_d2d_async(w.U1b, w.U1, (size_t)B * p.h_pw * 4, stream));
-            if ((st = predictor(pl, B, step, &a, flags, nullptr, seed, sample_offset, &b, want_mean ? result : nullptr, w, stream, w.sums, merge_next))) return st;
+            if ((st = predictor(pl, B, step, &a, flags, nullptr, seed, sample_offset, &b, want_mean ? result : nullptr, w, stream, w.sums, merge_next, &sf))) return st;
             ccsd_state_t t = a; a = b; b = t;
         } else if (rt.loop == LOOP_LANGEVIN || (rt.loop == LOOP_LANGEVIN_MULTI && pl->cfg.n_corr_steps > 0)) {
             const ccsd_state_t* cur = &a;
diff --git a/ccsd_amd/csrc/ccsd_k_r2.h b/ccsd_amd/csrc/ccsd_k_r2.h
--- a/ccsd_amd/csrc/ccsd_k_r2.h
+++ b/ccsd_amd/csrc/ccsd_k_r2.h
@@ -16,6 +16,8 @@
     unsigned int draw_r2;
     float* P0b; float* P1b; float* U1b;
     float* net2; float* part2;
+    int fold;
+    const float* part_in; const float* norm2; float* sums_out;
     int ldk, ldh;
     long long* dbg;
     const float* wp;
@@ -58,13 +60,19 @@
     const unsigned long long off = ra.offbits[b];
     const int hodge2 = (p.h_L > 1) && ra.want_p;
     const bool adjpow = hodge2 && p.hl[0].mval.n > 1;
+    const bool fold = ra.cf.on && ra.fold, fold_xa = fold && b == 0;
+    const int fB = (int)gridDim.x, fnv = normsum_threads(fB);
+    float c1f = 0.f, c2f = 0.f;
     auto build_tables = [&](auto&& between) {
         unsigned long long cw[2];
         unsigned int ew = 0;
+        NormsumPre fpre[2];
+        if (fold) normsum_request<2>(fpre, nullptr, ra.part_in, fB, 1, false, true);
 #pragma unroll
         for (int u = 0; u < 2; ++u) { const int k = tid + u * nth; cw[u] = cells[k < K ? k : K - 1]; }
         if (tid < 64) ew = *reinterpret_cast<const unsigned short*>(edges + 2 * (tid < E ? tid : E - 1));
         between();
+        if (fold) normsum_waves<2>(fpre, nullptr, ra.part_in, fB, 1, fnv, false, true, nullptr, sRed);
 #pragma unroll
         for (int u = 0; u < 2; ++u) { const int k = tid + u * nth; if (k < Kp4) sFrb[k] = (k < K && !(cw[u] & off)) ? 1 : 0; }
         for (int k = tid + 2 * nth; k < Kp4; k += nth) sFrb[k] = (k < K && !(cells[k] & off)) ? 1 : 0;
@@ -87,12 +95,17 @@
             }
         }
         __syncthreads();
+        if (fold) {
+            const float fs[6] = {0.f, 0.f, normsum_total(sRed, fnv), 0.f, 0.f, normsum_total(sRed + 16, fnv)};
+            LangCoef lf = ra.cf.lc;
+            lf.sums = fs;
+            langevin_coef(lf, 2, &c1f, &c2f);
+        }
         stamp(ra.dbg, 8);
     };
     float s_net = 0.f, s_z = 0.f;
     {
-        float c1f = 0.f, c2f = 0.f;
-        if (ra.cf.on) langevin_coef(ra.cf.lc, 2, &c1f, &c2f);
+        if (ra.cf.on && !fold) langevin_coef(ra.cf.lc, 2, &c1f, &c2f);
         NoiseArgs nc = na;
         if (ra.cf.on) { nc.zr = nullptr; nc.draw_r = ra.cf.draw_r; }
         const bool znorm = ep.mode == MODE_NORMS && na.flat_r, zuse = znorm || ra.cf.on;
@@ -212,7 +225,10 @@
             __syncthreads();
         }
     }
+    if (fold_xa) normsum_waves<0>(nullptr, ra.norm2, nullptr, fB, 1, fnv, true, false, sRow, nullptr);
     __syncthreads();
+    if (fold_xa)
+        for (int i = tid; i < 6; i += nth) ra.sums_out[i] = normsum_sum_of(sRow, sRed, i, fnv, true);
     const int npass = ra.merge ? 2 : 1;
     for (int pass = 0; pass < npass; ++pass) {
     const bool wb = ra.merge && pass == 0;
diff --git a/ccsd_amd/csrc/ccsd_k_update.h b/ccsd_amd/csrc/ccsd_k_update.h
--- a/ccsd_amd/csrc/ccsd_k_update.h
+++ b/ccsd_amd/csrc/ccsd_k_update.h
@@ -3,43 +3,11 @@
 
 __global__ void k_normsum(const float* __restrict__ norm2, const float* __restrict__ part, int B, int ntiles,
                           int is_cc, float* __restrict__ sums) {
-    __shared__ float red[16 * 6];
-    float acc[6] = {0.f, 0.f, 0.f, 0.f, 0.f, 0.f};
-    for (int b = threadIdx.x; b < B; b += blockDim.x) {
-        const float4 n4 = *reinterpret_cast<const float4*>(norm2 + (size_t)b * 4);
-        acc[0] += sqrtf(n4.x);
-        acc[1] += sqrtf(n4.y);
-        acc[3] += sqrtf(n4.z);
-        acc[4] += sqrtf(n4.w);
-        if (is_cc) {
-            float sn = 0.f, sz = 0.f;
-            for (int t = 0; t < ntiles; ++t) {
-                const float* p2 = part + ((size_t)b * ntiles + t) * 2;
-                sn += p2[0];
-                sz += p2[1];
-            }
-            acc[2] += sqrtf(sn);
-            acc[5] += sqrtf(sz);
-        }
-    }
-#ifdef CCSD_EMU
-    for (int i = 0; i < 6; ++i) sums[i] = acc[i];
-#else
-    const int wave = wave_index(), lane = threadIdx.x & 63, nw = (blockDim.x + 63) >> 6;
-#pragma unroll
-    for (int i = 0; i < 6; ++i) {
-        float v = acc[i];
-#pragma unroll
-        for (int o = 32; o > 0; o >>= 1) v += __shfl_xor(v, o, 64);
-        if (lane == 0) red[wave * 6 + i] = v;
-    }
+    __shared__ float red[6 * 16];
+    const int nv = blockDim.x;
+    normsum_waves<0>(nullptr, norm2, part, B, ntiles, nv, true, is_cc != 0, red, red + 64);
     __syncthreads();
-    if (threadIdx.x < 6) {
-        float t = 0.f;
-        for (int w = 0; w < nw; ++w) t += red[w * 6 + threadIdx.x];
-        sums[threadIdx.x] = t;
-    }
-#endif
+    for (int i = threadIdx.x; i < 6; i += blockDim.x) sums[i] = normsum_sum_of(red, red + 64, i, nv, is_cc != 0);
 }
 
 __global__ void k_normpart(const float* __restrict__ part, int ntiles, const float* __restrict__ zpart, int nchunk,
diff --git a/ccsd_amd/csrc/ccsd_rank2_common.h b/ccsd_amd/csrc/ccsd_rank2_common.h
--- a/ccsd_amd/csrc/ccsd_rank2_common.h
+++ b/ccsd_amd/csrc/ccsd_rank2_common.h
@@ -211,6 +211,103 @@
     *c1 = step * lc.ss[t];
     *c2 = sqrtf(step * 2.f) * lc.seps;
 }
+
+static inline __host__ __device__ int normsum_threads(int B) { return B > 512 ? 1024 : B > 256 ? 512 : 256; }
+struct NormsumPre { float4 n4; float2 p2; };
+template <int NPRE>
+CCSD_DEV void normsum_request(NormsumPre* pre, const float* __restrict__ norm2, const float* __restrict__ part, int B, int ntiles,
+                              bool xa, bool r2) {
+#ifdef CCSD_EMU
+    (void)pre; (void)norm2; (void)part; (void)B; (void)ntiles; (void)xa; (void)r2;
+#else
+    const int wave = wave_index(), lane = threadIdx.x & 63, nw = blockDim.x >> 6;
+#pragma unroll
+    for (int u = 0; u < NPRE; ++u) {
+        const int v = (wave + u * nw) * 64 + lane, b = v < B ? v : B - 1;
+        pre[u].n4 = make_float4(0.f, 0.f, 0.f, 0.f);
+        pre[u].p2 = make_float2(0.f, 0.f);
+        if (xa) pre[u].n4 = *reinterpret_cast<const float4*>(norm2 + (size_t)b * 4);
+        if (r2) pre[u].p2 = *reinterpret_cast<const float2*>(part + (size_t)b * ntiles * 2);
+    }
+#endif
+}
+template <int NPRE>
+CCSD_DEV void normsum_waves(const NormsumPre* pre, const float* __restrict__ norm2, const float* __restrict__ part, int B, int ntiles,
+                            int nv, bool xa, bool r2, float* red_xa, float* red_r2) {
+    float acc[6] = {0.f, 0.f, 0.f, 0.f, 0.f, 0.f};
+    auto add = [&](const float4& n4, const float2& p2, int b) {
+        if (xa) {
+            acc[0] += sqrtf(n4.x);
+            acc[1] += sqrtf(n4.y);
+            acc[3] += sqrtf(n4.z);
+            acc[4] += sqrtf(n4.w);
+        }
+        if (r2) {
+            float sn = 0.f, sz = 0.f;
+            sn += p2.x;
+            sz += p2.y;
+            for (int t = 1; t < ntiles; ++t) {
+                const float* q2 = part + ((size_t)b * ntiles + t) * 2;
+                sn += q2[0];
+                sz += q2[1];
+            }
+            acc[2] += sqrtf(sn);
+            acc[5] += sqrtf(sz);
+        }
+    };
+    auto fetch = [&](int b) {
+        NormsumPre s;
+        s.n4 = make_float4(0.f, 0.f, 0.f, 0.f);
+        s.p2 = make_float2(0.f, 0.f);
+        if (xa) s.n4 = *reinterpret_cast<const float4*>(norm2 + (size_t)b * 4);
+        if (r2) s.p2 = *reinterpret_cast<const float2*>(part + (size_t)b * ntiles * 2);
+        return s;
+    };
+#ifdef CCSD_EMU
+    (void)pre; (void)nv;
+    for (int b = 0; b < B; ++b) { const NormsumPre s = fetch(b); add(s.n4, s.p2, b); }
+    if (xa) { red_xa[0] = acc[0]; red_xa[16] = acc[1]; red_xa[32] = acc[3]; red_xa[48] = acc[4]; }
+    if (r2) { red_r2[0] = acc[2]; red_r2[16] = acc[5]; }
+#else
+    const int wave = wave_index(), lane = threadIdx.x & 63, nw = blockDim.x >> 6, nvw = nv >> 6;
+    auto one_wave = [&](int vw, const NormsumPre* first) {
+#pragma unroll
+        for (int i = 0; i < 6; ++i) acc[i] = 0.f;
+        int b = vw * 64 + lane;
+        NormsumPre s = first ? *first : fetch(b < B ? b : B - 1);
+        while (b < B) {
+            add(s.n4, s.p2, b);
+            b += nv;
+            if (b < B) s = fetch(b);
+        }
+        auto wave_sum = [&](float v, float* dst) {
+#pragma unroll
+            for (int o = 32; o > 0; o >>= 1) v += __shfl_xor(v, o, 64);
+            if (lane == 0) dst[vw] = v;
+        };
+        if (xa) { wave_sum(acc[0], red_xa); wave_sum(acc[1], red_xa + 16); wave_sum(acc[3], red_xa + 32); wave_sum(acc[4], red_xa + 48); }
+        if (r2) { wave_sum(acc[2], red_r2); wave_sum(acc[5], red_r2 + 16); }
+    };
+#pragma unroll
+    for (int u = 0; u < NPRE; ++u)
+        if (wave + u * nw < nvw) one_wave(wave + u * nw, pre + u);
+    for (int vw = wave + NPRE * nw; vw < nvw; vw += nw) one_wave(vw, nullptr);
+#endif
+}
+CCSD_DEV float normsum_total(const float* red16, int nv) {
+#ifdef CCSD_EMU
+    (void)nv;
+    return red16[0];
+#else
+    float t = 0.f;
+    for (int w = 0; w < (nv >> 6); ++w) t += red16[w];
+    return t;
+#endif
+}
+CCSD_DEV float normsum_sum_of(const float* red_xa, const float* red_r2, int i, int nv, bool r2) {
+    if (i == 2 || i == 5) return r2 ? normsum_total(red_r2 + (i == 5 ? 16 : 0), nv) : 0.f;
+    return normsum_total(red_xa + 16 * (i - (i > 2 ? 1 : 0)), nv);
+}
 CCSD_DEV float corr_apply(float c1, float c2, float net, float v, float zz) { return fmaf(c2, zz, fmaf(c1, net, v)); }
 CCSD_DEV float pred_update(float pa, float pb, float pc, float v, float net, float zz, float* mean) {
     *mean = fmaf(pa, v, pb * net);
diff --git a/include/ccsd_hip.h b/include/ccsd_hip.h
--- a/include/ccsd_hip.h
+++ b/include/ccsd_hip.h
@@ -101,6 +101,8 @@
     CCSD_QUERY_H_GENERAL = 16,
     CCSD_QUERY_GEO_EK = 17,
     CCSD_QUERY_H_WIDE = 18,
+    CCSD_QUERY_FOLD_SUMS = 20,
+    CCSD_QUERY_FOLD_LAST_RUN = 21,
     CCSD_QUERY_MLP_FORMS = 19
 };
 int ccsd_plan_query(const ccsd_plan_t* plan, int32_t what, int64_t* value);
```

New measurement: 4402 complexes/s, median of 6. +1.3%, better.
